# jackBonadies/Guided-Attention

Hardware: AMD Instinct MI355X
Metric: guided images/sec (50-step SD-1.5 512^2) (higher is better)
Workload: dtype f16

## Files before the change

guided-attention_amd/_lib.py:

```python
import ctypes
import os
from pathlib import Path

import torch

_HERE = Path(__file__).resolve().parent
LIB_PATH = Path(os.environ.get("GA_HIP_LIB", _HERE / "libga_hip.so"))

GA_VERSION = 183
GA_F16, GA_BF16, GA_F32 = 0, 1, 2
GA_LINEAR_STREAM = 8
GA_TOK_COOR, GA_TOK_BOX = 0, 1
GA_TERMS = 8
GA_MAX_IMAGES = 64
GA_IMAGE_MAX_TOKENS = 32
DTYPE_CODE = {torch.float16: GA_F16, torch.bfloat16: GA_BF16, torch.float32: GA_F32}


class GaError(RuntimeError):
    pass


class ga_token_t(ctypes.Structure):
    _fields_ = [("token", ctypes.c_int32), ("kind", ctypes.c_int32), ("geom", ctypes.c_double * 4),
# ... 30 lines not shown
    "ga_attn_capture_bwd": [_vp, _vp, _vp, _vp, _vp, _i64, _i64, _vp, _vp, _vp, _i, _i, _i, _i, _i, _f, _i, _vp],
    "ga_attn_capture_bwd_strided": [_vp, _vp, _vp, _vp, _vp, _i64, _i64, _i64, _vp, _vp, _vp, _i, _i, _i, _i, _i, _f, _i,
                                    _vp],
    "ga_attn_scores_max": [_vp, _vp, _i, _i, _i, _i, _i, _f, _i, _vp, _vp],
    "ga_attn_capture_fwd_biased": [_vp, _vp, _vp, _vp, _vp, _vp, _vp, _i, _i, _i, _i, _i, _f, _i, _vp],
    "ga_attn_capture_bwd_biased": [_vp, _vp, _vp, _vp, _vp, _i64, _i64, _vp, _vp, _vp, _vp, _i, _i, _i, _i, _i, _f, _i, _vp],
    "ga_attn_scores_max_grouped": [_vp, _vp, _i, _i, _i, _i, _i, _f, _i, _i, _vp, _vp],
    "ga_attn_capture_fwd_biased_grouped": [_vp, _vp, _vp, _vp, _vp, _vp, _i64, _vp, _vp, _i, _i, _i, _i, _i, _f, _i, _i, _vp],
    "ga_attn_capture_bwd_biased_grouped": [_vp, _vp, _vp, _vp, _vp, _i64, _i64, _i64, _vp, _vp, _i64, _vp, _vp, _vp, _i, _i, _i,
                                           _i, _i, _f, _i, _i, _vp],
    "ga_attn_pww_max_grad": [_vp, _vp, _vp, _vp, _vp, _i, _i, _i, _i, _i, _f, _i, _i, _vp],
    "ga_aggregate_maps": [ctypes.POINTER(_vp), ctypes.POINTER(_i), _i, _i, _i, _vp, _i, _vp],
    "ga_smooth_loss_fwd": [_vp, _i, _i, _i, _i, ctypes.POINTER(ga_token_t), _i, ctypes.POINTER(ga_loss_params_t), _vp,
                           _vp, _vp],
    "ga_smooth_loss_bwd": [_vp, _i, _i, _i, _i, ctypes.POINTER(ga_token_t), _i, ctypes.POINTER(ga_loss_params_t), _vp,
                           _vp, _vp, _f, _i, _vp],
    "ga_aggregate_loss_fwd": [ctypes.POINTER(_vp), ctypes.POINTER(_i), _i, _i, _i, _i, _i, ctypes.POINTER(ga_token_t), _i,
                              ctypes.POINTER(ga_loss_params_t), _vp, _vp, _vp, _vp, _i, _vp],
    "ga_aggregate_loss_fwd_batched": [ctypes.POINTER(_vp), ctypes.POINTER(_i), _i, _i, _i, _i, _i, _i,
                                      ctypes.POINTER(ga_token_t), _i, ctypes.POINTER(ga_loss_params_t), _vp, _vp, _vp, _vp,
                                      _i, _vp],
    "ga_smooth_loss_bwd_batched": [_vp, _i, _i, _i, _i, _i, ctypes.POINTER(ga_token_t), _i, ctypes.POINTER(ga_loss_params_t),
                                   _vp, _vp, _vp, _f, _i, _vp],
    "ga_aggregate_loss_fwd_images": [ctypes.POINTER(_vp), ctypes.POINTER(_i), _i, _i, _i, _i, _vp, _i,
                                     ctypes.POINTER(ga_loss_params_t), _vp, _vp, _vp, _vp, _i, _vp],
    "ga_smooth_loss_bwd_images": [_vp, _i, _i, _i, _vp, _i, ctypes.POINTER(ga_loss_params_t), _vp, _vp, _vp, _f, _i, _vp],
    "ga_gaussian_weights": [_i, _f, ctypes.POINTER(_f)],
    "ga_latent_axpy": [_vp, _vp, _f, _vp, _vp, _i64, _i, _vp],
    "ga_latent_sgd_momentum": [_vp, _vp, _vp, _f, _f, _i, _vp, _i64, _i, _vp],
    "ga_latent_axpby": [_vp, _vp, _f, _f, _vp, _i64, _i, _vp],
    "ga_cfg_ddim_step": [_vp, _vp, _f, _vp, _f, _f, _vp, _vp, _i64, _i, _vp],
    "ga_latent_axpy_batched": [_vp, _vp, _vp, _vp, _vp, _vp, _i, _i64, _i, _vp],
    "ga_latent_axpby_masked": [_vp, _vp, _f, _f, _vp, _vp, _i, _i64, _i, _vp],
    "ga_cfg_ddim_step_masked": [_vp, _vp, _f, _vp, _f, _f, _vp, _vp, _vp, _i, _i64, _i, _vp],
    "ga_self_attn_fwd": [_vp, _vp, _vp, _vp, _vp, _i, _i, _i, _i, _i, _f, _i, _vp],
    "ga_self_attn_bwd": [_vp, _vp, _vp, _vp, _vp, _vp, _vp, _vp, _vp, _vp, _i, _i, _i, _i, _i, _f, _i, _vp],
    "ga_group_norm_fwd": [_vp, _vp, _vp, _vp, _vp, _vp, _vp, _i, _i, _i, _i, _f, _i, _i, _vp],
    "ga_group_norm_bwd": [_vp, _vp, _vp, _vp, _vp, _vp, _vp, _vp, _vp, _i, _i, _i, _i, _i, _i, _vp],
    "ga_geglu_fwd": [_vp, _vp, _i64, _i, _i, _vp],
    "ga_geglu_bwd": [_vp, _vp, _vp, _i64, _i, _i, _vp],
    "ga_bias_residual_add": [_vp, _vp, _vp, _vp, _i64, _i, _i, _vp],
    "ga_cat_channels": [_vp, _vp, _vp, _i64, _i, _i, _i, _vp],
    "ga_cat_channels_gn_blocks": [_i, _i, _i, _i],
    "ga_linear_gn_blocks": [_i, _i, _i, _i, _i],
    "ga_group_norm_one_launch": [_i, _i, _i, _i],
    "ga_cat_group_norm_fwd": [_vp, _vp, _vp, _vp, _vp, _vp, _vp, _i, _i, _i, _i, _i, _f, _i, _i, _vp],
    "ga_cat_channels_gn": [_vp, _vp, _vp, _vp, _i, _i, _i, _i, _i, _i, _vp],
    "ga_conv3x3_packed_elems": [_i, _i],
    "ga_conv3x3_thin_packed_elems": [_i, _i],
    "ga_conv3x3_thin_supported": [_i, _i, _i, _i],
    "ga_conv3x3_thin_pack": [_vp, _vp, _i, _i, _i64, _i64, _i64, _i64, _i, _i, _vp],
    "ga_conv3x3_thin_in": [_vp, _vp, _vp, _vp, _i, _i, _i, _i, _i, _vp],
    "ga_conv3x3_thin_out": [_vp, _vp, _vp, _vp, _i, _i, _i, _i, _i, _vp],
    "ga_conv3x3_pack_weights": [_vp, _vp, _i, _i, _i64, _i64, _i64, _i64, _i, _i, _vp],
    "ga_conv3x3_plan": [_i, _i, _i, _i, _i, _i, ctypes.POINTER(_i), ctypes.POINTER(_i), ctypes.POINTER(_i),
                        ctypes.POINTER(ctypes.c_longlong)],
    "ga_splitk_workspace_floats": [_i64, _i, _i, _i, _i],
    "ga_conv3x3_nhwc": [_vp, _vp, _vp, _vp, _vp, _vp, _vp, _i, _i, _i, _i, _i, _i, _i, _i, _i, _i, _vp],
    "ga_conv3x3_gn_blocks": [_i, _i, _i, _i, _i, _i],
    "ga_conv3x3_nhwc_gn": [_vp, _vp, _vp, _vp, _vp, _vp, _vp, _i, _i, _i, _i, _i, _i, _i, _i, _i, _vp, _vp, _vp, _i],
    "ga_group_norm_apply": [_vp, _vp, _vp, _vp, _vp, _vp, _vp, _i, _i, _i, _i, _i, _f, _i, _i, _vp],
    "ga_group_norm_two_launch": [_i, _i, _i, _i],
    "ga_conv3x3_up2x_nhwc": [_vp, _vp, _vp, _vp, _vp, _vp, _vp, _i, _i, _i, _i, _i, _i, _i, _i, _i, _vp],
    "ga_gemm_nt": [_vp, _vp, _vp, _vp, _vp, _vp, _vp, _i64, _i, _i, _i, _i, _i, _i, _vp],
    "ga_linear_workspace": [_i64, _i, _i, _i, _i, _i, ctypes.POINTER(ctypes.c_longlong), ctypes.POINTER(_i)],
    "ga_linear_fused": [_vp, _i64, _vp, _vp, _i64, ctypes.POINTER(ga_linear_epilogue_t), _vp, _vp, _i64, _i, _i, _i, _i, _i,
                        _i, _i, _vp],
    "ga_add_layer_norm_fwd": [_vp, _vp, _vp, _vp, _vp, _vp, _vp, _i64, _i, _f, _i, _vp],
    "ga_add_layer_norm_bwd": [_vp, _vp, _vp, _vp, _vp, _vp, _i64, _i, _i, _vp],
}

_lib = None


def load():
    global _lib
    if _lib is None:
        if not LIB_PATH.exists():
            raise GaError(f"{LIB_PATH} not found: build it with `make` (or __graft_entry__.build()); "
                          "the guided-attention path has no CPU fallback")
        lib = ctypes.CDLL(str(LIB_PATH))
        lib.ga_version.argtypes, lib.ga_version.restype = [], ctypes.c_int
        built = lib.ga_version()
        if built != GA_VERSION:
            raise GaError(f"{LIB_PATH} is ABI version {built}, this binding is written for {GA_VERSION}: rebuild with `make`")
        for name, argtypes in PROTOTYPES.items():
            try:
                fn = getattr(lib, name)
            except AttributeError:
                raise GaError(f"{LIB_PATH} does not export {name}: rebuild with `make`") from None
            fn.argtypes = argtypes
            fn.restype = (ctypes.c_char_p if name == "ga_strerror" else
                          ctypes.c_longlong if name in ("ga_splitk_workspace_floats", "ga_conv3x3_packed_elems", "ga_conv3x3_thin_packed_elems") else ctypes.c_int)
        _lib = lib
    return _lib


def check(rc, what):
    if rc != 0:
        raise GaError(f"{what} failed: {load().ga_strerror(rc).decode()} ({rc})")


def stream_ptr():
    return ctypes.c_void_p(torch.cuda.current_stream().cuda_stream)


def dtype_code(t):
    try:
        return DTYPE_CODE[t.dtype]
    except KeyError:
        raise GaError(f"unsupported dtype {t.dtype}") from None


def require_cuda(*tensors):
    for t in tensors:
        if t is not None and not t.is_cuda:
            raise GaError("guided-attention kernels run on the GPU only (got a CPU tensor); there is no CPU fallback")
```

guided-attention_amd/csrc/group_norm.hip:

```cpp
#include "attn_common.h"

using namespace ga;

namespace {

constexpr int kThreads = 256;
constexpr int kMaxNPT = 5;
constexpr int kU = 8;

template <typename T, int W>
struct Item {
  T v[W];
};

template <typename T>
__device__ __forceinline__ Item<T, 2> load_pair(const T* p) {
  if constexpr (sizeof(T) == 2) return __builtin_bit_cast(Item<T, 2>, *reinterpret_cast<const unsigned*>(p));
  else return __builtin_bit_cast(Item<T, 2>, *reinterpret_cast<const unsigned long long*>(p));
}

__device__ __forceinline__ float sigmoidf_(float z) { return __builtin_amdgcn_rcpf(1.0f + __expf(-z)); }

template <typename T, int W>
__device__ __forceinline__ void load_chan_bias(const T* __restrict__ cbias, int b, int CP, int cp, float (&cb)[W]) {
#pragma unroll
  for (int j = 0; j < W; ++j) cb[j] = 0.f;
  if (cbias != nullptr) {
    const Item<T, W> it = reinterpret_cast<const Item<T, W>*>(cbias)[(size_t)b * CP + cp];
#pragma unroll
    for (int j = 0; j < W; ++j) cb[j] = Traits<T>::to_f32(it.v[j]);
  }
}

template <int NPT>
__device__ __forceinline__ void fold_to_groups(const float (&s0)[NPT], const float (&s1)[NPT], int CP, int cpg, int G,
                                               float* lds, float* out) {
#pragma unroll
  for (int k = 0; k < NPT; ++k) {
    const int cp = threadIdx.x + k * kThreads;
    if (cp < CP) {
      lds[2 * cp] = s0[k];
      lds[2 * cp + 1] = s1[k];
    }
  }
  __syncthreads();
  for (int g = threadIdx.x; g < G; g += kThreads) {
    float a = 0.f, b = 0.f;
    for (int cp = g * cpg; cp < (g + 1) * cpg; ++cp) {
      a += lds[2 * cp];
      b += lds[2 * cp + 1];
    }
    out[2 * g] = a;
    out[2 * g + 1] = b;
  }
}

template <typename T, int NPT, int W>
__global__ __launch_bounds__(kThreads) void gn_stats_kernel(const T* __restrict__ x, const T* __restrict__ cbias,
                                                            float* __restrict__ partial, int HW, int C, int G, int PB) {
  extern __shared__ __attribute__((aligned(16))) float lds[];
  const int b = blockIdx.y, nb = blockIdx.x, CP = C / W, cpg = (C / G) / W;
  const int p0 = nb * PB, p1 = min(HW, p0 + PB);
  float s0[NPT], s1[NPT];
#pragma unroll
  for (int k = 0; k < NPT; ++k) s0[k] = s1[k] = 0.f;
  const Item<T, W>* xb = reinterpret_cast<const Item<T, W>*>(x) + (size_t)b * HW * CP;
#pragma unroll
  for (int k = 0; k < NPT; ++k) {
    const int cp = threadIdx.x + k * kThreads;
    if (cp >= CP) continue;
    float cb[W];
    load_chan_bias<T, W>(cbias, b, CP, cp, cb);
    for (int p = p0; p < p1; p += kU) {
      Item<T, W> v[kU];
#pragma unroll
      for (int u = 0; u < kU; ++u)
        if (p + u < p1) v[u] = xb[(size_t)(p + u) * CP + cp];
#pragma unroll
      for (int u = 0; u < kU; ++u)
        if (p + u < p1) {
#pragma unroll
          for (int j = 0; j < W; ++j) {
            const float a = Traits<T>::to_f32(v[u].v[j]) + cb[j];
            s0[k] += a;
            s1[k] += a * a;
          }
        }
    }
  }
  fold_to_groups<NPT>(s0, s1, CP, cpg, G, lds, partial + ((size_t)b * gridDim.x + nb) * G * 2);
}

constexpr int kMaxStatsNB = 128;

struct NoHook {
  __device__ __forceinline__ void operator()() const {}
};
template <bool FWD, typename Hook = NoHook>
__device__ __forceinline__ void fold_partials(const float* __restrict__ partial, int b, int NB, int G, float inv_n,
                                              float eps, float2* res, float* keep, Hook after_loads = Hook()) {
  const float2* pp = reinterpret_cast<const float2*>(partial) + (size_t)b * NB * G;
  for (int g0 = 0; g0 < G; g0 += kThreads / 8) {
    const int g = g0 + (threadIdx.x >> 3), part = threadIdx.x & 7;
    float2 v[kMaxStatsNB / 8];
#pragma unroll
    for (int i = 0; i < kMaxStatsNB / 8; ++i) {
      const int nb = part + 8 * i;
      v[i] = pp[(size_t)min(nb, NB - 1) * G + min(g, G - 1)];
    }
    if (g0 == 0) after_loads();
    float sa = 0.f, sc = 0.f;
#pragma unroll
    for (int i = 0; i < kMaxStatsNB / 8; ++i) {
      const bool in = g < G && part + 8 * i < NB;
      sa += in ? v[i].x : 0.f;
      sc += in ? v[i].y : 0.f;
    }
    sa = group_sum<8>(sa);
    sc = group_sum<8>(sc);
    if (part == 0 && g < G) {
      float o0, o1;
      if (FWD) {
        const double mean = (double)sa * inv_n;
        const double var = fmax((double)sc * inv_n - mean * mean, 0.0);
        o0 = (float)mean;
        o1 = rsqrtf((float)var + eps);
      } else {
        o0 = sa * inv_n;
        o1 = sc * inv_n;
      }
      res[g] = float2{o0, o1};
      if (keep != nullptr) {
        keep[((size_t)b * G + g) * 2] = o0;
        keep[((size_t)b * G + g) * 2 + 1] = o1;
      }
    }
  }
  __syncthreads();
}

template <typename T, bool ACT, int NPT, int W>
__global__ __launch_bounds__(kThreads) void gn_apply_kernel(const T* __restrict__ x, const T* __restrict__ cbias,
                                                            const T* __restrict__ gamma,
                                                            const T* __restrict__ beta, T* __restrict__ y,
                                                            const float* __restrict__ partial, int NB, float inv_n,
                                                            float eps, float* __restrict__ stats, int HW, int C, int G,
                                                            int PB) {
  __shared__ float2 res[64];
  const int b = blockIdx.y, CP = C / W, cpg = (C / G) / W;
  fold_partials<true>(partial, b, NB, G, inv_n, eps, res, blockIdx.x == 0 ? stats : nullptr);
  const float* mu_rs = reinterpret_cast<const float*>(res);
  float sc[NPT][W], sh[NPT][W];
#pragma unroll
  for (int k = 0; k < NPT; ++k) {
    const int cp = threadIdx.x + k * kThreads;
    if (cp < CP) {
      const int g = cp / cpg;
      const Item<T, W> ga_ = reinterpret_cast<const Item<T, W>*>(gamma)[cp];
      const Item<T, W> be = reinterpret_cast<const Item<T, W>*>(beta)[cp];
      float cb[W];
      load_chan_bias<T, W>(cbias, b, CP, cp, cb);
#pragma unroll
      for (int j = 0; j < W; ++j) {
        sc[k][j] = Traits<T>::to_f32(ga_.v[j]) * mu_rs[2 * g + 1];
        sh[k][j] = Traits<T>::to_f32(be.v[j]) - (mu_rs[2 * g] - cb[j]) * sc[k][j];
      }
    }
  }
  const int p0 = blockIdx.x * PB, p1 = min(HW, p0 + PB);
  const Item<T, W>* xb = reinterpret_cast<const Item<T, W>*>(x) + (size_t)b * HW * CP;
  Item<T, W>* yb = reinterpret_cast<Item<T, W>*>(y) + (size_t)b * HW * CP;
#pragma unroll
  for (int k = 0; k < NPT; ++k) {
    const int cp = threadIdx.x + k * kThreads;
    if (cp >= CP) continue;
    for (int p = p0; p < p1; p += kU) {
      Item<T, W> v[kU];
#pragma unroll
      for (int u = 0; u < kU; ++u)
        if (p + u < p1) v[u] = xb[(size_t)(p + u) * CP + cp];
#pragma unroll
      for (int u = 0; u < kU; ++u)
        if (p + u < p1) {
          Item<T, W> o;
#pragma unroll
          for (int j = 0; j < W; ++j) {
            float z = Traits<T>::to_f32(v[u].v[j]) * sc[k][j] + sh[k][j];
            if (ACT) z *= sigmoidf_(z);
            o.v[j] = Traits<T>::from_f32(z);
          }
          yb[(size_t)(p + u) * CP + cp] = o;
        }
// ... 740 lines not shown
}

template <typename T>
int small_bwd(const void* x, const void* cb, const void* dy, const void* gamma, const void* beta, const float* stats,
              const void* gres, void* dx, int B, int HW, int C, int G, int act, hipStream_t s) {
  if (small_wide(HW, C, G))
    return act ? small_bwd_launch<T, true, 1024>(x, cb, dy, gamma, beta, stats, gres, dx, B, HW, C, G, s)
               : small_bwd_launch<T, false, 1024>(x, cb, dy, gamma, beta, stats, gres, dx, B, HW, C, G, s);
  return act ? small_bwd_launch<T, true, 256>(x, cb, dy, gamma, beta, stats, gres, dx, B, HW, C, G, s)
             : small_bwd_launch<T, false, 256>(x, cb, dy, gamma, beta, stats, gres, dx, B, HW, C, G, s);
}

bool small_path(int HW, int C, int G, size_t slab_bytes_per_elem) {
  const int Cg = C / G;
  return HW <= 1024 && (Cg & 1) == 0 && Cg <= 2048 && HW * Cg <= kSmallMaxElems &&
         kSmallHeader + slab_bytes_per_elem * (size_t)HW * Cg <= kMaxLdsBytes;
}

inline size_t elem_bytes(int dtype) { return dtype == GA_F32 ? 4 : 2; }

struct Geom {
  int NB, PBs, NBa, PBa, NPT, W;
  size_t lds;
};

int geometry(int B, int HW, int C, int G, Geom& g) {
  if (B < 1 || HW < 1 || C < 1 || G < 1 || G > 64 || C % G != 0) return GA_ERR_SHAPE;
  const int cg = C / G;
  g.W = (cg % 4 == 0) ? 4 : ((cg & 1) ? 1 : 2);
  const int CP = C / g.W;
  g.NPT = (CP + kThreads - 1) / kThreads;
  if (g.NPT > kMaxNPT) return GA_ERR_SHAPE;
  g.PBs = (HW + kMaxStatsNB - 1) / kMaxStatsNB < 8 ? 8 : (HW + kMaxStatsNB - 1) / kMaxStatsNB;
  g.NB = (HW + g.PBs - 1) / g.PBs;
  g.PBa = HW >= 4096 ? 16 : (HW >= 1024 ? 8 : 4);
  g.NBa = (HW + g.PBa - 1) / g.PBa;
  g.lds = sizeof(float) * 2 * CP;
  return GA_OK;
}

template <typename T, bool ACT, int NPT, int W>
int launch_fwd_t(const void* x, const void* cbias, const void* gamma, const void* beta, void* y, float* stats, float* ws,
                 int B, int HW, int C, int G, float eps, const Geom& g, hipStream_t s) {
  const float inv_n = 1.0f / ((float)HW * (float)(C / G));
  hipLaunchKernelGGL((gn_stats_kernel<T, NPT, W>), dim3(g.NB, B), dim3(kThreads), g.lds, s, (const T*)x,
                     (const T*)cbias, ws, HW, C, G, g.PBs);
  hipLaunchKernelGGL((gn_apply_kernel<T, ACT, NPT, W>), dim3(g.NBa, B), dim3(kThreads), 0, s, (const T*)x,
                     (const T*)cbias, (const T*)gamma, (const T*)beta, (T*)y, (const float*)ws, g.NB, inv_n, eps, stats,
                     HW, C, G, g.PBa);
  return check_launch();
}

template <typename T, bool ACT, int NPT, int W>
int launch_bwd_t(const void* x, const void* cbias, const void* dy, const void* gamma, const void* beta,
                 const float* stats, const void* gres, void* dx, float* ws, int B, int HW, int C, int G, const Geom& g,
                 hipStream_t s) {
  const float inv_n = 1.0f / ((float)HW * (float)(C / G));
  hipLaunchKernelGGL((gn_bwd_stats_kernel<T, ACT, NPT, W>), dim3(g.NB, B), dim3(kThreads), g.lds, s, (const T*)x,
                     (const T*)cbias, (const T*)dy, (const T*)gamma, (const T*)beta, stats, ws, HW, C, G, g.PBs);
  hipLaunchKernelGGL((gn_bwd_apply_kernel<T, ACT, NPT, W>), dim3(g.NBa, B), dim3(kThreads), 0, s, (const T*)x,
                     (const T*)cbias, (const T*)dy, (const T*)gamma, (const T*)beta, stats, (const float*)ws, g.NB, inv_n,
                     (const T*)gres, (T*)dx, HW, C, G, g.PBa);
  return check_launch();
}

#define GA_GN_NPT(FN, T, ACT, ...)                                   \
  if (g.W == 1) {                                                    \
    switch (g.NPT) {                                                 \
      case 1: return FN<T, ACT, 1, 1>(__VA_ARGS__);                  \
      case 2: return FN<T, ACT, 2, 1>(__VA_ARGS__);                  \
      default: return FN<T, ACT, 5, 1>(__VA_ARGS__);                 \
    }                                                                \
  }                                                                  \
  if (g.W == 4) {                                                    \
    switch (g.NPT) {                                                 \
      case 1: return FN<T, ACT, 1, 4>(__VA_ARGS__);                  \
      case 2: return FN<T, ACT, 2, 4>(__VA_ARGS__);                  \
      default: return FN<T, ACT, 3, 4>(__VA_ARGS__);                 \
    }                                                                \
  }                                                                  \
  switch (g.NPT) {                                                   \
    case 1: return FN<T, ACT, 1, 2>(__VA_ARGS__);                    \
    case 2: return FN<T, ACT, 2, 2>(__VA_ARGS__);                    \
    case 3: return FN<T, ACT, 3, 2>(__VA_ARGS__);                    \
    case 4: return FN<T, ACT, 4, 2>(__VA_ARGS__);                    \
    default: return FN<T, ACT, 5, 2>(__VA_ARGS__);                   \
  }

inline bool wide_ok(int C, int G, size_t elem) { return elem == 2 && C % 8 == 0 && C / G >= 8 && C <= 8 * kThreads; }

struct WideGeom {
  int PBs, NB, PBa, NBa;
  WideGeom(int HW, int C) {
    const int RP = kThreads / (C / 8);
    const int fill = (HW + kMaxStatsNB - 1) / kMaxStatsNB;
    PBs = fill > 8 * RP ? fill : 8 * RP;
    NB = (HW + PBs - 1) / PBs;
    PBa = 4 * RP;
    NBa = (HW + PBa - 1) / PBa;
  }
};

template <typename T>
int wide_fwd(const void* x, const void* cbias, const void* gamma, const void* beta, void* y, float* stats, float* ws,
             int B, int HW, int C, int G, float eps, int act, hipStream_t s) {
  const WideGeom g(HW, C);
  const float inv_n = 1.0f / ((float)HW * (float)(C / G));
  hipLaunchKernelGGL(gn_wide_stats_kernel<T>, dim3(g.NB, B), dim3(kThreads), 0, s, (const T*)x, (const T*)cbias, ws, HW,
                     C, G, g.PBs);
  if (act)
    hipLaunchKernelGGL((gn_wide_apply_kernel<T, true>), dim3(g.NBa, B), dim3(kThreads), 0, s, (const T*)x,
                       (const T*)cbias, (const T*)gamma, (const T*)beta, (T*)y, (const float*)ws, g.NB, inv_n, eps, stats,
                       HW, C, G, g.PBa);
  else
    hipLaunchKernelGGL((gn_wide_apply_kernel<T, false>), dim3(g.NBa, B), dim3(kThreads), 0, s, (const T*)x,
                       (const T*)cbias, (const T*)gamma, (const T*)beta, (T*)y, (const float*)ws, g.NB, inv_n, eps, stats,
                       HW, C, G, g.PBa);
  return check_launch();
}

template <typename T>
int wide_bwd(const void* x, const void* cbias, const void* dy, const void* gamma, const void* beta, const float* stats,
             const void* gres, void* dx, float* ws, int B, int HW, int C, int G, int act, hipStream_t s) {
  const WideGeom g(HW, C);
  const float inv_n = 1.0f / ((float)HW * (float)(C / G));
  if (act)
    hipLaunchKernelGGL((gn_wide_bwd_stats_kernel<T, true>), dim3(g.NB, B), dim3(kThreads), 0, s, (const T*)x,
                       (const T*)cbias, (const T*)dy, (const T*)gamma, (const T*)beta, stats, ws, HW, C, G, g.PBs);
  else
    hipLaunchKernelGGL((gn_wide_bwd_stats_kernel<T, false>), dim3(g.NB, B), dim3(kThreads), 0, s, (const T*)x,
                       (const T*)cbias, (const T*)dy, (const T*)gamma, (const T*)beta, stats, ws, HW, C, G, g.PBs);
  if (act)
    hipLaunchKernelGGL((gn_wide_bwd_apply_kernel<T, true>), dim3(g.NBa, B), dim3(kThreads), 0, s, (const T*)x,
                       (const T*)cbias, (const T*)dy, (const T*)gamma, (const T*)beta, stats, (const float*)ws, g.NB,
                       inv_n, (const T*)gres, (T*)dx, HW, C, G, g.PBa);
  else
    hipLaunchKernelGGL((gn_wide_bwd_apply_kernel<T, false>), dim3(g.NBa, B), dim3(kThreads), 0, s, (const T*)x,
                       (const T*)cbias, (const T*)dy, (const T*)gamma, (const T*)beta, stats, (const float*)ws, g.NB,
                       inv_n, (const T*)gres, (T*)dx, HW, C, G, g.PBa);
  return check_launch();
}

template <typename T>
int fwd_dtype(const void* x, const void* cbias, const void* gamma, const void* beta, void* y, float* stats, float* ws, int B,
              int HW, int C, int G, float eps, int act, const Geom& g, hipStream_t s) {
  if constexpr (sizeof(T) == 2) {
    if (wide_ok(C, G, sizeof(T))) return wide_fwd<T>(x, cbias, gamma, beta, y, stats, ws, B, HW, C, G, eps, act, s);
  }
  if (act) {
    GA_GN_NPT(launch_fwd_t, T, true, x, cbias, gamma, beta, y, stats, ws, B, HW, C, G, eps, g, s)
  }
  GA_GN_NPT(launch_fwd_t, T, false, x, cbias, gamma, beta, y, stats, ws, B, HW, C, G, eps, g, s)
}

template <typename T>
int bwd_dtype(const void* x, const void* cbias, const void* dy, const void* gamma, const void* beta, const float* stats,
              const void* gres, void* dx, float* ws, int B, int HW, int C, int G, int act, const Geom& g, hipStream_t s) {
  if constexpr (sizeof(T) == 2) {
    if (wide_ok(C, G, sizeof(T))) return wide_bwd<T>(x, cbias, dy, gamma, beta, stats, gres, dx, ws, B, HW, C, G, act, s);
  }
  if (act) {
    GA_GN_NPT(launch_bwd_t, T, true, x, cbias, dy, gamma, beta, stats, gres, dx, ws, B, HW, C, G, g, s)
  }
  GA_GN_NPT(launch_bwd_t, T, false, x, cbias, dy, gamma, beta, stats, gres, dx, ws, B, HW, C, G, g, s)
}

}

extern "C" int ga_group_norm_fwd(const void* x, const void* chan_bias, const void* gamma, const void* beta, void* y,
                                 float* stats, float* workspace, int B, int HW, int C, int G, float eps, int act_silu,
                                 int dtype, ga_stream_t stream) {
  if (!x || !gamma || !beta || !y || !stats || !workspace) return GA_ERR_NULL;
  Geom g;
  int rc = geometry(B, HW, C, G, g);
  if (rc != GA_OK) return rc;
  hipStream_t s = static_cast<hipStream_t>(stream);
  if (small_path(HW, C, G, sizeof(float))) {
    switch (dtype) {
      case GA_F16: return small_fwd<_Float16>(x, chan_bias, gamma, beta, y, stats, B, HW, C, G, eps, act_silu, s);
      case GA_BF16: return small_fwd<bf16_t>(x, chan_bias, gamma, beta, y, stats, B, HW, C, G, eps, act_silu, s);
      case GA_F32: return small_fwd<float>(x, chan_bias, gamma, beta, y, stats, B, HW, C, G, eps, act_silu, s);
      default: return GA_ERR_DTYPE;
    }
  }
  switch (dtype) {
    case GA_F16: return fwd_dtype<_Float16>(x, chan_bias, gamma, beta, y, stats, workspace, B, HW, C, G, eps, act_silu, g, s);
    case GA_BF16: return fwd_dtype<bf16_t>(x, chan_bias, gamma, beta, y, stats, workspace, B, HW, C, G, eps, act_silu, g, s);
    case GA_F32: return fwd_dtype<float>(x, chan_bias, gamma, beta, y, stats, workspace, B, HW, C, G, eps, act_silu, g, s);
    default: return GA_ERR_DTYPE;
  }
}

extern "C" int ga_group_norm_apply(const void* x, const void* chan_bias, const void* gamma, const void* beta, void* y,
                                   float* stats, const float* partials, int blocks, int B, int HW, int C, int G, float eps,
                                   int act_silu, int dtype, ga_stream_t stream) {
  if (!x || !gamma || !beta || !y || !stats || !partials) return GA_ERR_NULL;
  Geom g;
  int rc = geometry(B, HW, C, G, g);
  if (rc != GA_OK) return rc;
  if (blocks < 1 || blocks > kMaxStatsNB) return GA_ERR_SHAPE;
  if (dtype == GA_F32 || !wide_ok(C, G, 2)) return GA_ERR_UNSUPPORTED;
  hipStream_t s = static_cast<hipStream_t>(stream);
  const WideGeom wg(HW, C);
  const float inv_n = 1.0f / ((float)HW * (float)(C / G));
#define GA_GN_APPLY(T, ACT)                                                                                                   \
  hipLaunchKernelGGL((gn_wide_apply_kernel<T, ACT>), dim3(wg.NBa, B), dim3(kThreads), 0, s, (const T*)x, (const T*)chan_bias, \
                     (const T*)gamma, (const T*)beta, (T*)y, partials, blocks, inv_n, eps, stats, HW, C, G, wg.PBa)
  if (dtype == GA_F16) {
    if (act_silu) GA_GN_APPLY(_Float16, true);
    else GA_GN_APPLY(_Float16, false);
  } else if (dtype == GA_BF16) {
    if (act_silu) GA_GN_APPLY(bf16_t, true);
    else GA_GN_APPLY(bf16_t, false);
  } else {
    return GA_ERR_DTYPE;
  }
#undef GA_GN_APPLY
  return check_launch();
}

extern "C" int ga_group_norm_one_launch(int HW, int C, int G, int dtype) {
  if (HW < 1 || C < 1 || G < 1 || G > 64 || C % G != 0 || dtype < GA_F16 || dtype > GA_F32) return 0;
  return small_path(HW, C, G, sizeof(float)) ? 1 : 0;
}

extern "C" int ga_cat_group_norm_fwd(const void* a, const void* b, void* cat, const void* gamma, const void* beta, void* y,
                                     float* stats, int B, int HW, int C1, int C2, int G, float eps, int act_silu, int dtype,
                                     ga_stream_t stream) {
  if (!a || !b || !cat || !gamma || !beta || !y || !stats) return GA_ERR_NULL;
  if (C1 < 2 || C2 < 2 || C1 % 2 != 0 || C2 % 2 != 0) return GA_ERR_SHAPE;
  const int C = C1 + C2;
  Geom g;
  int rc = geometry(B, HW, C, G, g);
  if (rc != GA_OK) return rc;
  if ((C / G) % 2 != 0) return GA_ERR_SHAPE;
  if (!small_path(HW, C, G, sizeof(float))) return GA_ERR_UNSUPPORTED;
  hipStream_t s = static_cast<hipStream_t>(stream);
  const SmallCat sc{b, C1, cat};
  switch (dtype) {
    case GA_F16: return small_fwd<_Float16>(a, nullptr, gamma, beta, y, stats, B, HW, C, G, eps, act_silu, s, sc);
    case GA_BF16: return small_fwd<bf16_t>(a, nullptr, gamma, beta, y, stats, B, HW, C, G, eps, act_silu, s, sc);
    case GA_F32: return small_fwd<float>(a, nullptr, gamma, beta, y, stats, B, HW, C, G, eps, act_silu, s, sc);
    default: return GA_ERR_DTYPE;
  }
}

extern "C" int ga_cat_channels_gn_blocks(int HW, int C, int G, int dtype) {
  if (dtype == GA_F32 || HW < 1 || C < 1 || G < 1 || C % G != 0) return 0;
  if (small_path(HW, C, G, sizeof(float)) || !wide_ok(C, G, 2)) return 0;
  return WideGeom(HW, C).NB;
}

extern "C" int ga_cat_channels_gn(const void* a, const void* b, void* out, float* partials, int B, int HW, int C1, int C2, int G,
                                  int dtype, ga_stream_t stream) {
  if (!a || !b || !out || !partials) return GA_ERR_NULL;
// ... 47 lines not shown
```

guided-attention_amd/csrc/linear.hip:

```cpp
#include "attn_common.h"

using namespace ga;

namespace {

typedef float f32x16 __attribute__((ext_vector_type(16)));
typedef unsigned int u32x4 __attribute__((ext_vector_type(4)));

constexpr int kBK = 64;
constexpr int kThreads = 256;
#define GA_LDS_PTR(p) ((__attribute__((address_space(3))) void*)(p))

template <typename T>
struct Mma32L;
template <>
struct Mma32L<_Float16> {
  __device__ static __forceinline__ f32x16 run(uint4 a, uint4 b, f32x16 c) {
    return __builtin_amdgcn_mfma_f32_32x32x16_f16(__builtin_bit_cast(f16x8, a), __builtin_bit_cast(f16x8, b), c, 0, 0, 0);
  }
};
template <>
struct Mma32L<bf16_t> {
  __device__ static __forceinline__ f32x16 run(uint4 a, uint4 b, f32x16 c) {
    return __builtin_amdgcn_mfma_f32_32x32x16_bf16(__builtin_bit_cast(bf16x8, a), __builtin_bit_cast(bf16x8, b), c, 0, 0, 0);
  }
};

struct LinArgs {
  int M, N, K;
  int ldx, ldy, ld_res, ld_pre;
  int tm, tn, splits, steps, steps_per, n_fastest;
  FastDiv d_tm, d_tn;
  int F;
  int ln_parts;
  float ln_eps, ln_inv_k;
  unsigned x_bytes, w_bytes;
};

struct LinHead {
  int M, ldx;
  unsigned kn;
  int tm;
  unsigned tn_splits;
  unsigned steps;
  unsigned dtm_m, dtn_m;
};

struct LinPtrs {
  const void* bias;
  const void* residual;
  void* preact;
  const float* ln_partials;
  const float* ln_colsum;
  const float* ln_shift;
  float* ln_stats_out;
  float* row_partials_out;
  float* slabs;
  unsigned* tickets;
  float* gn_partials;
  int gn_cg, gn_G, gn_hw, gn_tpi;
};

template <int BM, int BN>
__device__ __forceinline__ void lin_tile(const LinArgs& a, int& mt, int& nt, int& split) {
  const int total = a.tm * a.tn * a.splits, q = total >> 3, r = total & 7;
  const int xcd = blockIdx.x & 7, slot = blockIdx.x >> 3;
  const int logical = (xcd < r ? xcd * (q + 1) : r * (q + 1) + (xcd - r) * q) + slot;
  const bool nf = a.n_fastest != 0;
  const FastDiv d1 = nf ? a.d_tn : a.d_tm, d2 = nf ? a.d_tm : a.d_tn;
  const int t1 = nf ? a.tn : a.tm, t2 = nf ? a.tm : a.tn;
  const int rest = fdiv(logical, d1), i1 = logical - rest * t1;
  split = fdiv(rest, d2);
  const int i2 = rest - split * t2;
  mt = nf ? i2 : i1;
  nt = nf ? i1 : i2;
}

__device__ __forceinline__ void lds_read128(u32x4& dst, unsigned byte_address) {
#if defined(__HIP_DEVICE_COMPILE__)
  asm volatile("ds_read_b128 %0, %1" : "=v"(dst) : "v"(byte_address) : "memory");
#else
  dst = u32x4{byte_address, 0u, 0u, 0u};
#endif
}
__device__ __forceinline__ void opaque(u32x4& v) {
#if defined(__HIP_DEVICE_COMPILE__)
  asm volatile("" : "+v"(v));
#endif
}
template <int N>
__device__ __forceinline__ void wait_vmcnt() {
#if defined(__HIP_DEVICE_COMPILE__)
  asm volatile("s_waitcnt vmcnt(%0)" ::"n"(N) : "memory");
#endif
}
template <int N>
__device__ __forceinline__ void wait_lgkmcnt() {
#if defined(__HIP_DEVICE_COMPILE__)
  asm volatile("s_waitcnt lgkmcnt(%0)" ::"n"(N) : "memory");
#endif
}

#if defined(GA_LIN_STAMPS)
__device__ unsigned long long* g_lin_stamps = nullptr;
struct LinStamps {
  unsigned long long t[10];
  __device__ __forceinline__ void at(int i) {
#if defined(__HIP_DEVICE_COMPILE__)
    __builtin_amdgcn_sched_barrier(0);
    unsigned long long v;
    asm volatile("s_memtime %0\n\ts_waitcnt lgkmcnt(0)" : "=s"(v)::"memory");
    __builtin_amdgcn_sched_barrier(0);
    t[i] = v;
#endif
  }
  __device__ __forceinline__ void real(int i) {
#if defined(__HIP_DEVICE_COMPILE__)
    __builtin_amdgcn_sched_barrier(0);
    unsigned long long v;
    asm volatile("s_memrealtime %0\n\ts_waitcnt lgkmcnt(0)" : "=s"(v)::"memory");
    __builtin_amdgcn_sched_barrier(0);
    t[i] = v;
#endif
  }
  __device__ __forceinline__ void flush() {
    if (threadIdx.x == 0 && g_lin_stamps != nullptr)
      for (int i = 0; i < 10; ++i) g_lin_stamps[(size_t)blockIdx.x * 10 + i] = t[i];
  }
};
#define GA_STAMP(st, i) (st).at(i)
#else
struct LinStamps {};
#define GA_STAMP(st, i) ((void)0)
#endif

// ... 179 lines not shown
      s1 = group_sum<VPR>(s1);
      s2 = group_sum<VPR>(s2);
      if ((v & (VPR - 1)) == 0 && m < a.M)
        *reinterpret_cast<float2*>(p.row_partials_out + ((size_t)m * a.tn + nt) * 2) = float2{s1, s2};
    }
  }
  if constexpr (!GEGLU) {
    if (gn) {
      const int cv = (tid & (VPR - 1)) * 8;
      const int c_abs = n0 + cv, gA = c_abs / p.gn_cg, split = min(8, (gA + 1) * p.gn_cg - c_abs);
      float4 r = {0.f, 0.f, 0.f, 0.f};
#pragma unroll
      for (int q = 0; q < 8; ++q) {
        if (q < split) {
          r.x += gsum[q];
          r.y += gsq[q];
        } else {
          r.z += gsum[q];
          r.w += gsq[q];
        }
      }
      __syncthreads();
      float4* lds4 = reinterpret_cast<float4*>(Cs);
      lds4[tid] = r;
      __syncthreads();
      const int n_end = min(n0 + BN, a.N);
      const int g_first = n0 / p.gn_cg, g_last = (n_end - 1) / p.gn_cg;
      const int g = g_first + tid;
      if (g <= g_last) {
        const int c_lo = max(g * p.gn_cg, n0), c_hi = min((g + 1) * p.gn_cg, n_end);
        float sa = 0.f, sq = 0.f;
        for (int vv = (c_lo - n0) >> 3; vv <= (c_hi - 1 - n0) >> 3; ++vv) {
          const bool first = (n0 + 8 * vv) / p.gn_cg == g;
          for (int pr = 0; pr < kThreads / VPR; ++pr) {
            const float4 e4 = lds4[pr * VPR + vv];
            sa += first ? e4.x : e4.z;
            sq += first ? e4.y : e4.w;
          }
        }
        const int b = m0 / p.gn_hw, t = (m0 - b * p.gn_hw) / BM;
        float2* out = reinterpret_cast<float2*>(p.gn_partials) + ((size_t)b * 2 * p.gn_tpi + 2 * t) * p.gn_G + g;
        const bool starts = g * p.gn_cg >= n0, ends = (g + 1) * p.gn_cg <= n_end;
        if (starts) {
          out[0] = float2{sa, sq};
          if (ends) out[p.gn_G] = float2{0.f, 0.f};
        } else {
          out[p.gn_G] = float2{sa, sq};
        }
      }
    }
  }
}

template <typename T, int BM, int BN, int NSTAGE, bool GEGLU, bool LN>
__global__ __launch_bounds__(kThreads, (BM + BN) * 128 * NSTAGE <= 80 * 1024 ? 2 : 1) void linear_kernel(
    const T* __restrict__ X, const T* __restrict__ W, T* __restrict__ Y, int h_M, int h_ldx, unsigned h_kn, int h_tm,
    unsigned h_tn_splits, unsigned h_steps, unsigned h_dtm_m, unsigned h_dtn_m, LinArgs a_in, LinPtrs p) {
  const LinHead h{h_M, h_ldx, h_kn, h_tm, h_tn_splits, h_steps, h_dtm_m, h_dtn_m};
  LinStamps st;
#if defined(GA_LIN_STAMPS)
  st.real(8);
#endif
  GA_STAMP(st, 0);
  LinArgs a;
  a.M = h.M; a.ldx = h.ldx; a.K = (int)(h.kn & 0xffffu); a.N = (int)(h.kn >> 16);
  a.tm = h.tm; a.tn = (int)(h.tn_splits & 0xffffu); a.splits = (int)(h.tn_splits >> 16);
  a.steps = (int)(h.steps & 0xffffu); a.steps_per = (int)((h.steps >> 16) & 0x7fffu); a.n_fastest = (int)(h.steps >> 31);
  a.d_tm = FastDiv{(unsigned)a.tm, h.dtm_m}; a.d_tn = FastDiv{(unsigned)a.tn, h.dtn_m};
  a.F = GEGLU ? a.N / 2 : 0;
  a.x_bytes = (unsigned)(((a.M - 1) * a.ldx + a.K) * 2); a.w_bytes = (unsigned)(a.N * a.K * 2);
  a.ldy = a_in.ldy; a.ld_res = a_in.ld_res; a.ld_pre = a_in.ld_pre;
  a.ln_parts = a_in.ln_parts; a.ln_eps = a_in.ln_eps; a.ln_inv_k = a_in.ln_inv_k;
  constexpr int WM = BM / 2, WN = BN / 2, IM = WM / 32, JN = WN / 32;
  constexpr int kStage = (BM + BN) * kBK;
  constexpr int IPS = (BM + BN) / 32;
  constexpr int LDC = BN + 8;
  constexpr int kLds = NSTAGE * kStage > BM * LDC ? NSTAGE * kStage : BM * LDC;
  __shared__ __attribute__((aligned(1024))) T lds[kLds];

  const int tid = threadIdx.x, lane = tid & 63, wave = tid >> 6;
  const int wm = wave >> 1, wn = wave & 1, fr = lane & 31, fh = lane >> 5;
  int mt, nt, split;
  lin_tile<BM, BN>(a, mt, nt, split);
  const int m0 = mt * BM;
  const int n0 = GEGLU ? nt * (BN / 2) : nt * BN;
  const int it0 = split * a.steps_per, it1 = min(a.steps, it0 + a.steps_per);
  const int nsteps = it1 - it0;

  const __amdgpu_buffer_rsrc_t xrsrc = __builtin_amdgcn_make_buffer_rsrc(const_cast<T*>(X), 0, a.x_bytes, 0x00020000);
  const __amdgpu_buffer_rsrc_t wrsrc = __builtin_amdgcn_make_buffer_rsrc(const_cast<T*>(W), 0, a.w_bytes, 0x00020000);
  unsigned voff[IPS];
#pragma unroll
  for (int q = 0; q < IPS; ++q) {
    const int row = 8 * (wave + 4 * q) + (lane >> 3);
    const int col = (lane & 7) ^ ((row >> 1) & 7);
    if (row < BM) {
      const int m = min(m0 + row, a.M - 1);
      voff[q] = (unsigned)((m * a.ldx + 8 * col) * (int)sizeof(T));
    } else {
      const int r = row - BM;
      int n;
      if (GEGLU) n = r < BN / 2 ? min(n0 + r, a.F - 1) : a.F + min(n0 + r - BN / 2, a.F - 1);
      else n = min(n0 + r, a.N - 1);
      voff[q] = (unsigned)((n * a.K + 8 * col) * (int)sizeof(T));
    }
  }
  const int wave_u = __builtin_amdgcn_readfirstlane(wave);
  auto issue = [&](int step, int slot) {
    const unsigned koff = (unsigned)((it0 + step) * kBK * (int)sizeof(T));
#pragma unroll
    for (int q = 0; q < IPS; ++q) {
      T* dst = lds + slot * kStage + (wave_u + 4 * q) * 8 * kBK;
      if (8 * (wave_u + 4 * q) < BM)
        __builtin_amdgcn_raw_ptr_buffer_load_lds(xrsrc, GA_LDS_PTR(dst), 16, (int)voff[q], (int)koff, 0, 0);
      else
        __builtin_amdgcn_raw_ptr_buffer_load_lds(wrsrc, GA_LDS_PTR(dst), 16, (int)voff[q], (int)koff, 0, 0);
    }
  };

  unsigned a_adr[IM], a_sw[IM], b_adr[JN], b_sw[JN];
  const unsigned lds0 = (unsigned)(uintptr_t)GA_LDS_PTR(lds);
#pragma unroll
  for (int i = 0; i < IM; ++i) {
    const int row = wm * WM + i * 32 + fr;
    a_adr[i] = lds0 + row * (kBK * (int)sizeof(T));
    a_sw[i] = (unsigned)(((row >> 1) & 7) ^ fh);
  }
#pragma unroll
  for (int j = 0; j < JN; ++j) {
    const int row = BM + wn * WN + j * 32 + fr;
    b_adr[j] = lds0 + row * (kBK * (int)sizeof(T));
    b_sw[j] = (unsigned)(((row >> 1) & 7) ^ fh);
  }

  f32x16 acc[JN][IM];
#pragma unroll
  for (int j = 0; j < JN; ++j)
#pragma unroll
    for (int i = 0; i < IM; ++i)
#pragma unroll
      for (int r = 0; r < 16; ++r) acc[j][i][r] = 0.f;

  constexpr int PRE = NSTAGE - 1;
#pragma unroll
  for (int s = 0; s < PRE; ++s)
    if (s < nsteps) issue(s, s);
  LinPrefetch<T, BM, BN, GEGLU, LN> pre;
  pre.load(a, p, m0, n0);
  float ln_mean[IM], ln_rstd[IM];
  if constexpr (LN) {
    const float2* part[IM];
    float s1[IM], s2[IM];
#pragma unroll
    for (int i = 0; i < IM; ++i) {
      const int m = min(m0 + wm * WM + i * 32 + fr, a.M - 1);
      part[i] = reinterpret_cast<const float2*>(p.ln_partials) + (size_t)m * a.ln_parts;
      s1[i] = s2[i] = 0.f;
    }
    for (int q0 = 0; q0 < a.ln_parts; q0 += 4) {
      float2 v[IM][4];
#pragma unroll
      for (int i = 0; i < IM; ++i)
#pragma unroll
        for (int u = 0; u < 4; ++u) v[i][u] = part[i][min(q0 + u, a.ln_parts - 1)];
#pragma unroll
      for (int i = 0; i < IM; ++i)
#pragma unroll
        for (int u = 0; u < 4; ++u)
          if (q0 + u < a.ln_parts) {
            s1[i] += v[i][u].x;
            s2[i] += v[i][u].y;
          }
    }
#pragma unroll
    for (int i = 0; i < IM; ++i) {
      const float mean = s1[i] * a.ln_inv_k;
      ln_mean[i] = mean;
      ln_rstd[i] = rsqrtf(fmaxf(s2[i] * a.ln_inv_k - mean * mean, 0.f) + a.ln_eps);
    }
  }

  GA_STAMP(st, 1);
  for (int it = 0; it < nsteps; ++it) {
    const int younger = min(nsteps - 1 - it, PRE - 1);
    if (younger >= 3) wait_vmcnt<3 * IPS>();
    else if (younger == 2) wait_vmcnt<2 * IPS>();
    else if (younger == 1) wait_vmcnt<IPS>();
    else wait_vmcnt<0>();
    __builtin_amdgcn_s_barrier();
#if defined(GA_LIN_STAMPS)
    if (it == 0) st.at(2);
#endif
    if (it + PRE < nsteps) issue(it + PRE, (it + PRE) % NSTAGE);
    const unsigned slot_off = (unsigned)((it % NSTAGE) * kStage * (int)sizeof(T));
    u32x4 fa[2][IM], fb[2][JN];
    auto request = [&](int kk, int set) {
#pragma unroll
      for (int i = 0; i < IM; ++i)
        lds_read128(fa[set][i], a_adr[i] + slot_off + 16u * ((2u * kk) ^ a_sw[i]));
#pragma unroll
      for (int j = 0; j < JN; ++j)
        lds_read128(fb[set][j], b_adr[j] + slot_off + 16u * ((2u * kk) ^ b_sw[j]));
    };
    request(0, 0);
#pragma unroll
    for (int kk = 0; kk < kBK / 16; ++kk) {
      if (kk + 1 < kBK / 16) {
        request(kk + 1, (kk + 1) & 1);
        wait_lgkmcnt<IM + JN>();
      } else {
        wait_lgkmcnt<0>();
      }
      __builtin_amdgcn_sched_barrier(0);
#pragma unroll
      for (int j = 0; j < JN; ++j)
#pragma unroll
        for (int i = 0; i < IM; ++i)
          acc[j][i] = Mma32L<T>::run(__builtin_bit_cast(uint4, fb[kk & 1][j]), __builtin_bit_cast(uint4, fa[kk & 1][i]), acc[j][i]);
    }
  }
  static_assert(NSTAGE >= 2 && NSTAGE <= 5, "the counted waits above cover up to four k-steps in flight");
  wait_lgkmcnt<0>();
  __builtin_amdgcn_s_barrier();
  GA_STAMP(st, 3);

  if (a.splits > 1) {
    const int tile = nt * a.tm + mt;
    const __amdgpu_buffer_rsrc_t srsrc =
        __builtin_amdgcn_make_buffer_rsrc(p.slabs, 0, 0x7ffffff0, 0x00020000);
    constexpr int QUADS = JN * IM * 4;
    const unsigned per_slice = (unsigned)(a.tm * a.tn) * (BM * BN * 4u);
    const unsigned tbase = (unsigned)tile * (BM * BN * 4u) + (unsigned)tid * 16u;
#pragma unroll
    for (int j = 0; j < JN; ++j)
#pragma unroll
      for (int i = 0; i < IM; ++i)
#pragma unroll
        for (int qd = 0; qd < 4; ++qd) {
          const int q = (j * IM + i) * 4 + qd;
          const u32x4 v = {__float_as_uint(acc[j][i][4 * qd]), __float_as_uint(acc[j][i][4 * qd + 1]),
                           __float_as_uint(acc[j][i][4 * qd + 2]), __float_as_uint(acc[j][i][4 * qd + 3])};
          __builtin_amdgcn_raw_buffer_store_b128(v, srsrc, tbase + q * (kThreads * 16u), split * per_slice, 16);
        }
    asm volatile("s_waitcnt vmcnt(0)" ::: "memory");
#pragma unroll
    for (int j = 0; j < JN; ++j)
#pragma unroll
      for (int i = 0; i < IM; ++i) keep_live(acc[j][i]);
    __syncthreads();
    int* flag = reinterpret_cast<int*>(lds);
    if (tid == 0) {
      const unsigned old = __hip_atomic_fetch_add(p.tickets + tile, 1u, __ATOMIC_RELAXED, __HIP_MEMORY_SCOPE_AGENT);
      flag[0] = old == (unsigned)a.splits - 1;
      if (old == (unsigned)a.splits - 1) __hip_atomic_store(p.tickets + tile, 0u, __ATOMIC_RELAXED, __HIP_MEMORY_SCOPE_AGENT);
    }
    __syncthreads();
    const int last = flag[0];
    __syncthreads();
    if (!last) return;
#pragma unroll
    for (int j = 0; j < JN; ++j)
#pragma unroll
      for (int i = 0; i < IM; ++i)
#pragma unroll
        for (int r = 0; r < 16; ++r) acc[j][i][r] = 0.f;
    constexpr int SB = QUADS <= 4 ? 4 : (QUADS <= 8 ? 2 : 1);
    for (int s0 = 0; s0 < a.splits; s0 += SB) {
      u32x4 v[SB][QUADS];
#pragma unroll
      for (int sb = 0; sb < SB; ++sb) {
        const unsigned soff = (unsigned)min(s0 + sb, a.splits - 1) * per_slice;
#pragma unroll
        for (int q = 0; q < QUADS; ++q)
          v[sb][q] = __builtin_amdgcn_raw_buffer_load_b128(srsrc, tbase + q * (kThreads * 16u), soff, 16);
      }
#pragma unroll
      for (int sb = 0; sb < SB; ++sb) {
        const bool in = s0 + sb < a.splits;
#pragma unroll
        for (int j = 0; j < JN; ++j)
#pragma unroll
          for (int i = 0; i < IM; ++i)
#pragma unroll
            for (int qd = 0; qd < 4; ++qd)
#pragma unroll
              for (int r = 0; r < 4; ++r)
                acc[j][i][4 * qd + r] += in ? __uint_as_float(v[sb][(j * IM + i) * 4 + qd][r]) : 0.f;
      }
    }
  }

  float ln_m[IM], ln_r[IM];
#pragma unroll
  for (int i = 0; i < IM; ++i) {
    ln_m[i] = LN ? ln_mean[i] : 0.f;
    ln_r[i] = LN ? ln_rstd[i] : 1.f;
  }
  GA_STAMP(st, 4);
  lin_epilogue<T, BM, BN, GEGLU, LN>(acc, lds, Y, a, p, m0, n0, nt, ln_m, ln_r, pre, st);
#if defined(GA_LIN_STAMPS)
  st.at(6);
  asm volatile("s_waitcnt vmcnt(0)" ::: "memory");
  st.at(7);
  st.real(9);
  st.flush();
#endif
}

template <typename T, int BM, int BN, int NSTAGE>
int launch_lin(const T* X, const T* W, T* Y, LinArgs a, const LinPtrs& p, hipStream_t s) {
  const int outc = a.F ? BN / 2 : BN, n_out = a.F ? a.F : a.N;
  a.tm = (a.M + BM - 1) / BM;
  a.tn = (n_out + outc - 1) / outc;
  a.steps = a.K / kBK;
  a.steps_per = (a.steps + a.splits - 1) / a.splits;
  {
    const double xb = (double)a.M * a.K, wb = (double)a.N * a.K;
    const double m_first = wb + xb * (a.tn * a.splits < 8 ? a.tn * a.splits : 8), n_first = xb + wb * (a.tm < 8 ? a.tm : 8);
    a.n_fastest = n_first < m_first ? 1 : 0;
  }
  {
    bool ok = true;
    const unsigned long long wgs = (unsigned long long)a.tm * a.tn * a.splits;
    a.d_tm = make_fastdiv(a.tm, wgs, ok);
    a.d_tn = make_fastdiv(a.tn, wgs, ok);
    if (!ok) return GA_ERR_SHAPE;
  }
  const dim3 grid((unsigned)(a.tm * a.tn * a.splits));
  const bool ln = a.ln_parts > 0;
  if (a.K > 0xffff || a.N > 0xffff || a.tn > 0xffff || a.splits > 0xffff || a.steps > 0xffff || a.steps_per > 0x7fff) return GA_ERR_SHAPE;
  const LinHead h{a.M, a.ldx, (unsigned)a.K | ((unsigned)a.N << 16), a.tm, (unsigned)a.tn | ((unsigned)a.splits << 16),
                  (unsigned)a.steps | ((unsigned)a.steps_per << 16) | ((unsigned)(a.n_fastest != 0) << 31), a.d_tm.m, a.d_tn.m};
#define GA_LIN_LAUNCH(G, L)                                                                                                \
  hipLaunchKernelGGL((linear_kernel<T, BM, BN, NSTAGE, G, L>), grid, dim3(kThreads), 0, s, X, W, Y, h.M, h.ldx, h.kn, h.tm, \
                     h.tn_splits, h.steps, h.dtm_m, h.dtn_m, a, p)
  if (a.F) {
    if (ln) GA_LIN_LAUNCH(true, true);
    else GA_LIN_LAUNCH(true, false);
  } else {
    if (ln) GA_LIN_LAUNCH(false, true);
    else GA_LIN_LAUNCH(false, false);
  }
#undef GA_LIN_LAUNCH
  return check_launch();
}

template <typename T>
int lin_t(const void* X, const void* W, void* Y, const LinArgs& a, const LinPtrs& p, int bm, int bn, int stages, hipStream_t s) {
  const T* x = (const T*)X;
  const T* w = (const T*)W;
  if (bm == 128 && bn == 128) {
    if (stages == 2) return launch_lin<T, 128, 128, 2>(x, w, (T*)Y, a, p, s);
    if (stages == 0 || stages == 3) return launch_lin<T, 128, 128, 3>(x, w, (T*)Y, a, p, s);
  } else if ((bm == 128 && bn == 64) || (bm == 64 && bn == 128)) {
    const bool tall = bm == 128;
    if (stages == 3) return tall ? launch_lin<T, 128, 64, 3>(x, w, (T*)Y, a, p, s) : launch_lin<T, 64, 128, 3>(x, w, (T*)Y, a, p, s);
    if (stages == 0 || stages == 4)
      return tall ? launch_lin<T, 128, 64, 4>(x, w, (T*)Y, a, p, s) : launch_lin<T, 64, 128, 4>(x, w, (T*)Y, a, p, s);
  } else if (bm == 64 && bn == 64) {
    if (stages == 5) return launch_lin<T, 64, 64, 5>(x, w, (T*)Y, a, p, s);
    if (stages == 0 || stages == 4) return launch_lin<T, 64, 64, 4>(x, w, (T*)Y, a, p, s);
  }
  return GA_ERR_SHAPE;
}

constexpr int kSThreads = 512;
constexpr int kSStage = 256 * kBK * 2;
constexpr int kSNst = 4, kSPre = kSNst - 1;
constexpr int kSOutStride = 144;
constexpr int kSPartsMax = 20;
constexpr int kSStageOff = kSNst * kSStage;
constexpr int kSStageBytes = 128 * 16 * (kSPartsMax / 2);
constexpr int kSCstOff = kSStageOff + kSStageBytes;
constexpr int kSStatOff = kSCstOff + 1024;
constexpr int kSLds = kSStatOff + 1024;
static_assert(128 * kSOutStride <= kSStageBytes && kSLds <= 160 * 1024, "LDS map of linear_stream_kernel");

__device__ __forceinline__ void lds_read64(f32x2& dst, unsigned byte_address) {
#if defined(__HIP_DEVICE_COMPILE__)
  asm volatile("ds_read_b64 %0, %1" : "=v"(dst) : "v"(byte_address) : "memory");
#else
  dst = f32x2{(float)byte_address, 0.f};
#endif
}
__device__ __forceinline__ void lds_read128f(f32x4& dst, unsigned byte_address) {
#if defined(__HIP_DEVICE_COMPILE__)
  asm volatile("ds_read_b128 %0, %1" : "=v"(dst) : "v"(byte_address) : "memory");
#else
  dst = f32x4{(float)byte_address, 0.f, 0.f, 0.f};
#endif
}
__device__ __forceinline__ void lds_write64(unsigned byte_address, f32x2 v) {
#if defined(__HIP_DEVICE_COMPILE__)
  asm volatile("ds_write_b64 %0, %1" ::"v"(byte_address), "v"(v) : "memory");
#endif
}

template <typename T>
__device__ __forceinline__ f32x2 pack4(float a, float b, float c, float d) {
  typename Traits<T>::frag f;
  f[0] = Traits<T>::from_f32(a);
  f[1] = Traits<T>::from_f32(b);
  f[2] = Traits<T>::from_f32(c);
  f[3] = Traits<T>::from_f32(d);
  return __builtin_bit_cast(f32x2, f);
}

template <typename T, bool GEGLU>
__global__ __launch_bounds__(kSThreads, 2) void linear_stream_kernel(
    const T* __restrict__ X, const T* __restrict__ W, T* __restrict__ Y, int h_M, int h_ldx, unsigned h_kn, int h_tm,
    unsigned h_tn_splits, unsigned h_steps, unsigned h_dtm_m, unsigned h_dtn_m, LinArgs a_in, LinPtrs p) {
  const int M = h_M, ldx = h_ldx, K = (int)(h_kn & 0xffffu), N = (int)(h_kn >> 16);
  const int tm = h_tm, tn = (int)(h_tn_splits & 0xffffu), G = (int)(h_tn_splits >> 16);
  const int steps = (int)(h_steps & 0xffffu);
// ... 269 lines not shown
  const long long tiles = (long long)a.tm * a.tn;
  if (tiles > 0x7fffffffLL / 256 || a.K > 0xffff || a.N > 0xffff || a.tn > 0xffff || a.steps > 0xffff) return GA_ERR_SHAPE;
  const int G = tiles < cus ? (int)tiles : cus;
  {
    const double xb = (double)a.M * a.K, wb = (double)a.N * a.K;
    const double m_first = wb + xb * (a.tn < 8 ? a.tn : 8), n_first = xb + wb * (a.tm < 8 ? a.tm : 8);
    a.n_fastest = n_first < m_first ? 1 : 0;
  }
  bool ok = true;
  const unsigned long long span = (unsigned long long)tiles + (unsigned long long)G;
  a.d_tm = make_fastdiv(a.tm, span, ok);
  a.d_tn = make_fastdiv(a.tn, span, ok);
  if (!ok) return GA_ERR_SHAPE;
  const LinHead h{a.M, a.ldx, (unsigned)a.K | ((unsigned)a.N << 16), a.tm, (unsigned)a.tn | ((unsigned)G << 16),
                  (unsigned)a.steps | ((unsigned)(a.n_fastest != 0) << 31), a.d_tm.m, a.d_tn.m};
  if (a.F)
    hipLaunchKernelGGL((linear_stream_kernel<T, true>), dim3((unsigned)G), dim3(kSThreads), 0, s, X, W, Y, h.M, h.ldx, h.kn, h.tm,
                       h.tn_splits, h.steps, h.dtm_m, h.dtn_m, a, p);
  else
    hipLaunchKernelGGL((linear_stream_kernel<T, false>), dim3((unsigned)G), dim3(kSThreads), 0, s, X, W, Y, h.M, h.ldx, h.kn, h.tm,
                       h.tn_splits, h.steps, h.dtm_m, h.dtn_m, a, p);
  return check_launch();
}

bool al16(const void* p) { return (reinterpret_cast<uintptr_t>(p) & 15) == 0; }

}

#if defined(GA_LIN_STAMPS)
extern "C" int ga_lin_set_stamps(void* buffer) {
  unsigned long long* p = static_cast<unsigned long long*>(buffer);
  return hipMemcpyToSymbol(HIP_SYMBOL(g_lin_stamps), &p, sizeof(p)) == hipSuccess ? GA_OK : GA_ERR_LAUNCH;
}
#endif

extern "C" int ga_linear_workspace(int64_t M, int N, int bm, int bn, int splits, int geglu, long long* slab_floats, int* tiles) {
  if (!slab_floats || !tiles) return GA_ERR_NULL;
  if (M < 1 || N < 8 || splits < 1 || (bm != 64 && bm != 128) || (bn != 64 && bn != 128)) return GA_ERR_SHAPE;
  const int outc = geglu ? bn / 2 : bn, n_out = geglu ? N / 2 : N;
  const long long tm = (M + bm - 1) / bm, tn = (n_out + outc - 1) / outc;
  *tiles = (int)(tm * tn);
  *slab_floats = splits > 1 ? (long long)splits * tm * tn * bm * bn : 0;
  return GA_OK;
}

extern "C" int ga_linear_gn_blocks(int hw, int N, int groups, int bm, int bn) {
  if (hw < 1 || N < 8 || groups < 1 || N % groups != 0 || (bm != 64 && bm != 128) || (bn != 64 && bn != 128)) return 0;
  const int cg = N / groups;
  if (hw % bm != 0 || cg < 8 || cg > bn || groups > 64) return 0;
  const int blocks = 2 * (hw / bm);
  return blocks <= 128 ? blocks : 0;
}

extern "C" int ga_linear_fused(const void* X, int64_t ldx, const void* W, void* Y, int64_t ldy, const ga_linear_epilogue_t* ep,
                               float* slabs, unsigned* tickets, int64_t M, int K, int N, int bm, int bn, int splits,
                               int stages, int dtype, ga_stream_t stream) {
  if (!X || !W || !Y || !ep) return GA_ERR_NULL;
  if (M < 1 || K < kBK || K % kBK != 0 || N < 8 || N % 8 != 0 || ldx < K || ldx % 8 != 0 || ldy % 8 != 0) return GA_ERR_SHAPE;
  if (splits < 1 || splits > 64 || K / kBK < splits || (splits > 1 && (!slabs || !tickets))) return GA_ERR_SHAPE;
  const int n_out = ep->geglu ? N / 2 : N;
  if (ep->geglu && (N % 16 != 0 || ep->residual)) return GA_ERR_SHAPE;
  if (ldy < n_out || (ep->residual && (ep->ld_res < n_out || ep->ld_res % 8 != 0))) return GA_ERR_SHAPE;
  if (ep->preact && (!ep->geglu || ep->ld_pre < N || ep->ld_pre % 8 != 0)) return GA_ERR_SHAPE;
  if (ep->ln_partials && (ep->ln_parts < 1 || !ep->ln_colsum || !ep->ln_shift)) return GA_ERR_NULL;
  if (!al16(X) || !al16(W) || !al16(Y) || (ep->bias && !al16(ep->bias)) || (ep->residual && !al16(ep->residual)) ||
      (ep->preact && !al16(ep->preact)) || (ep->ln_colsum && !al16(ep->ln_colsum)) || (ep->ln_shift && !al16(ep->ln_shift)))
    return GA_ERR_ALIGN;
  const long long xb = ((long long)(M - 1) * ldx + K) * 2, wb = (long long)N * K * 2;
  if (xb >= (1LL << 31) || wb >= (1LL << 31)) return GA_ERR_SHAPE;
  LinArgs a;
  a.M = (int)M; a.N = N; a.K = K;
  a.ldx = (int)ldx; a.ldy = (int)ldy; a.ld_res = (int)ep->ld_res; a.ld_pre = (int)ep->ld_pre;
  a.splits = splits;
  a.F = ep->geglu ? N / 2 : 0;
  a.ln_parts = ep->ln_partials ? ep->ln_parts : 0;
  a.ln_eps = ep->ln_eps;
  a.ln_inv_k = 1.0f / (float)K;
  a.x_bytes = (unsigned)xb;
  a.w_bytes = (unsigned)wb;
  if (splits > 1) {
    long long need; int tiles;
    if (ga_linear_workspace(M, N, bm, bn, splits, ep->geglu, &need, &tiles) != GA_OK) return GA_ERR_SHAPE;
    if (need * 4 >= (1LL << 31)) return GA_ERR_SHAPE;
  }
  LinPtrs p;
  p.bias = ep->bias; p.residual = ep->residual; p.preact = ep->preact;
  p.ln_partials = ep->ln_partials; p.ln_colsum = ep->ln_colsum; p.ln_shift = ep->ln_shift;
  p.ln_stats_out = ep->ln_stats_out; p.row_partials_out = ep->row_partials_out;
  p.slabs = slabs; p.tickets = tickets;
  p.gn_partials = nullptr; p.gn_cg = p.gn_G = p.gn_hw = p.gn_tpi = 0;
  if (ep->gn_partials) {
    if (ep->geglu || stages == GA_LINEAR_STREAM) return GA_ERR_UNSUPPORTED;
    if (ga_linear_gn_blocks(ep->gn_hw, N, ep->gn_groups, bm, bn) == 0 || M % ep->gn_hw != 0) return GA_ERR_SHAPE;
    p.gn_partials = ep->gn_partials; p.gn_G = ep->gn_groups; p.gn_cg = N / ep->gn_groups; p.gn_hw = ep->gn_hw;
    p.gn_tpi = ep->gn_hw / bm;
  }
  hipStream_t s = static_cast<hipStream_t>(stream);
  if (stages == GA_LINEAR_STREAM) {
    if (bm != 128 || bn != 128 || splits != 1 || !ep->ln_partials || ep->bias || ep->residual || ep->preact || ep->ln_stats_out ||
        ep->row_partials_out || K / kBK < 5 || ep->ln_parts < 2 || ep->ln_parts > kSPartsMax || ldy > 0x7fffffff)
      return GA_ERR_UNSUPPORTED;
    if ((long long)M * ep->ln_parts * 8 >= (1LL << 31)) return GA_ERR_SHAPE;
    switch (dtype) {
      case GA_F16: return launch_stream<_Float16>((const _Float16*)X, (const _Float16*)W, (_Float16*)Y, a, p, s);
      case GA_BF16: return launch_stream<bf16_t>((const bf16_t*)X, (const bf16_t*)W, (bf16_t*)Y, a, p, s);
      default: return GA_ERR_DTYPE;
    }
  }
  switch (dtype) {
    case GA_F16: return lin_t<_Float16>(X, W, Y, a, p, bm, bn, stages, s);
    case GA_BF16: return lin_t<bf16_t>(X, W, Y, a, p, bm, bn, stages, s);
    default: return GA_ERR_DTYPE;
  }
}
```

guided-attention_amd/csrc/thin_conv.hip:

```cpp
#include "ga_common.h"

namespace {
using namespace ga;

constexpr int kSeg = 16;
constexpr int kPatchW = kSeg + 2;
constexpr int kTaps = 9;

template <typename T>
struct Dot2;
template <>
struct Dot2<_Float16> {
  typedef _Float16 v2 __attribute__((ext_vector_type(2)));
  __device__ static __forceinline__ float acc(uint32_t a, uint32_t b, float c) {
    return __builtin_amdgcn_fdot2(__builtin_bit_cast(v2, a), __builtin_bit_cast(v2, b), c, false);
  }
};
template <>
struct Dot2<bf16_t> {
  typedef __bf16 v2 __attribute__((ext_vector_type(2)));
  __device__ static __forceinline__ float acc(uint32_t a, uint32_t b, float c) {
    return __builtin_amdgcn_fdot2_f32_bf16(__builtin_bit_cast(v2, a), __builtin_bit_cast(v2, b), c, false);
  }
};

template <typename T>
__device__ __forceinline__ uint16_t bits_of(T x) {
  return __builtin_bit_cast(uint16_t, x);
}

__global__ void thin_pack_kernel(const uint16_t* __restrict__ w, uint32_t* __restrict__ out, int N, int C, long long so,
                                 long long si, long long sy, long long sx, int flip) {
  const int total = kTaps * (C / 2) * N;
  const int i = blockIdx.x * blockDim.x + threadIdx.x;
  if (i >= total) return;
  int n, q, t;
  if (C == 4) {
    n = i % N;
    q = (i / N) % 2;
    t = i / (2 * N);
  } else {
    n = i % 4;
    q = (i / 4) % (C / 2);
    t = i / (4 * (C / 2));
  }
  const int ty = t / 3, tx = t % 3;
  uint32_t v[2];
#pragma unroll
  for (int e = 0; e < 2; ++e) {
    const int c = 2 * q + e;
    const long long off = flip ? c * so + n * si + (2 - ty) * sy + (2 - tx) * sx : n * so + c * si + ty * sy + tx * sx;
    v[e] = w[off];
  }
// ... 13 lines not shown

  uint4 wv[2 * kTaps];
#pragma unroll
  for (int i = 0; i < 2 * kTaps; ++i) wv[i] = wp[(size_t)i * G + g];
  float bv[4] = {0.f, 0.f, 0.f, 0.f};
  if (bias) {
    const typename Traits<T>::frag bf = load_frag<T>(bias + 4 * g);
#pragma unroll
    for (int j = 0; j < 4; ++j) bv[j] = Traits<T>::to_f32(bf[j]);
  }

  const int pc = tid % kPatchW, pr = (tid / kPatchW) % 3, pci = tid / (3 * kPatchW);
  auto fetch = [&](int sg) -> uint16_t {
    const int seg = sg % segs, row = (sg / segs) % H, b = sg / (segs * H);
    const int yy = row + pr - 1, xx = seg * kSeg + pc - 1;
    if (tid < kInPatch && yy >= 0 && yy < H && xx >= 0 && xx < W) return bits_of(x[(((size_t)b * 4 + pci) * H + yy) * W + xx]);
    return 0;
  };
  uint16_t* pl = reinterpret_cast<uint16_t*>(patch);
  const int first = blockIdx.x * segs_per_wg;
  const int last = min(first + segs_per_wg, total_segs);
  uint16_t nxt = fetch(first);
  for (int sg = first; sg < last; ++sg) {
    const int seg = sg % segs, row = (sg / segs) % H, b = sg / (segs * H);
    if (sg != first) __syncthreads();
    if (tid < kInPatch) pl[(pr * kPatchW + pc) * 4 + pci] = nxt;
    __syncthreads();
    if (sg + 1 < last) nxt = fetch(sg + 1);
    for (int s = slot; s < kSeg; s += PP) {
      float acc[4] = {bv[0], bv[1], bv[2], bv[3]};
#pragma unroll
      for (int t = 0; t < kTaps; ++t) {
        const uint2 xv = patch[(t / 3) * kPatchW + s + (t % 3)];
        const uint4 w0 = wv[2 * t], w1 = wv[2 * t + 1];
        acc[0] = Dot2<T>::acc(xv.x, w0.x, acc[0]);
        acc[1] = Dot2<T>::acc(xv.x, w0.y, acc[1]);
        acc[2] = Dot2<T>::acc(xv.x, w0.z, acc[2]);
        acc[3] = Dot2<T>::acc(xv.x, w0.w, acc[3]);
        acc[0] = Dot2<T>::acc(xv.y, w1.x, acc[0]);
        acc[1] = Dot2<T>::acc(xv.y, w1.y, acc[1]);
        acc[2] = Dot2<T>::acc(xv.y, w1.z, acc[2]);
        acc[3] = Dot2<T>::acc(xv.y, w1.w, acc[3]);
      }
      typename Traits<T>::frag o;
#pragma unroll
      for (int j = 0; j < 4; ++j) o[j] = Traits<T>::from_f32(acc[j]);
      store_frag<T>(y + (((size_t)b * H + row) * W + seg * kSeg + s) * N + 4 * g, o);
    }
  }
}

constexpr int kOutThreads = 256;
constexpr int kOutSlices = 32;

template <typename T, int PAIRS>
__global__ void __launch_bounds__(kOutThreads)
thin_out_kernel(const T* __restrict__ x, const uint32_t* __restrict__ wp, const T* __restrict__ bias, T* __restrict__ y, int H, int W,
                int total_segs, int segs_per_wg) {
  constexpr int C = PAIRS * 64;
  constexpr int kVecPx = C / 8;
  constexpr int kPatchVecs = 3 * kPatchW * kVecPx;
  constexpr int kLoads = (kPatchVecs + kOutThreads - 1) / kOutThreads;
  __shared__ uint4 patch[kPatchVecs];
  const int tid = threadIdx.x;
  const int sl = tid & (kOutSlices - 1), slot = tid >> 5;
  const int segs = W / kSeg;

  uint4 wr[kTaps][PAIRS];
#pragma unroll
  for (int t = 0; t < kTaps; ++t)
#pragma unroll
    for (int q = 0; q < PAIRS; ++q) wr[t][q] = reinterpret_cast<const uint4*>(wp)[t * (C / 2) + sl * PAIRS + q];
  float bv = 0.f;
  if (bias && sl < 4) bv = Traits<T>::to_f32(bias[sl]);

  auto fetch = [&](int sg, uint4 (&val)[kLoads]) {
    const int seg = sg % segs, row = (sg / segs) % H, b = sg / (segs * H);
#pragma unroll
    for (int j = 0; j < kLoads; ++j) {
      const int i = tid + j * kOutThreads;
      const int v = i % kVecPx, c = (i / kVecPx) % kPatchW, r = i / (kVecPx * kPatchW);
      const int yy = row + r - 1, xx = seg * kSeg + c - 1;
      const bool in = i < kPatchVecs && yy >= 0 && yy < H && xx >= 0 && xx < W;
      const size_t pix = in ? ((size_t)b * H + yy) * W + xx : (size_t)b * H * W;
      const uint4 t = reinterpret_cast<const uint4*>(x + pix * C)[in ? v : 0];
      val[j] = in ? t : uint4{0u, 0u, 0u, 0u};
    }
  };
  const int first = blockIdx.x * segs_per_wg;
  const int last = min(first + segs_per_wg, total_segs);
  uint4 val[kLoads];
  fetch(first, val);
  for (int sg = first; sg < last; ++sg) {
    const int seg = sg % segs, row = (sg / segs) % H, b = sg / (segs * H);
    if (sg != first) __syncthreads();
#pragma unroll
    for (int j = 0; j < kLoads; ++j) {
      const int i = tid + j * kOutThreads;
      if (i < kPatchVecs) patch[i] = val[j];
    }
    __syncthreads();
    if (sg + 1 < last) fetch(sg + 1, val);

    const uint32_t* pw = reinterpret_cast<const uint32_t*>(patch);
#pragma unroll
    for (int h = 0; h < kSeg / 8; ++h) {
      const int p = slot + 8 * h;
      float acc[4] = {0.f, 0.f, 0.f, 0.f};
#pragma unroll
      for (int t = 0; t < kTaps; ++t) {
        const uint32_t* xp = pw + ((t / 3) * kPatchW + p + (t % 3)) * (C / 2) + sl * PAIRS;
#pragma unroll
        for (int q = 0; q < PAIRS; ++q) {
          const uint32_t xv = xp[q];
          acc[0] = Dot2<T>::acc(xv, wr[t][q].x, acc[0]);
          acc[1] = Dot2<T>::acc(xv, wr[t][q].y, acc[1]);
          acc[2] = Dot2<T>::acc(xv, wr[t][q].z, acc[2]);
          acc[3] = Dot2<T>::acc(xv, wr[t][q].w, acc[3]);
        }
      }
#pragma unroll
      for (int j = 0; j < 4; ++j) {
        acc[j] = group_sum<16>(acc[j]);
        acc[j] += __shfl_xor(acc[j], 16, 64);
      }
      if (sl < 4) {
        const float v = (sl == 0 ? acc[0] : sl == 1 ? acc[1] : sl == 2 ? acc[2] : acc[3]) + bv;
        y[(((size_t)b * 4 + sl) * H + row) * W + seg * kSeg + p] = Traits<T>::from_f32(v);
      }
    }
  }
}

inline bool aligned16(const void* p) { return (reinterpret_cast<uintptr_t>(p) & 15u) == 0; }

inline void seg_grid(long long total, int& per, unsigned& grid) {
  per = (int)((total + 1023) / 1024);
  grid = (unsigned)((total + per - 1) / per);
}

template <typename T>
int launch_in(const void* x, const void* wp, const void* bias, void* y, int B, int H, int W, int N, hipStream_t s) {
  const int G = N / 4;
  int PP = (256 + G - 1) / G;
  PP = PP < 1 ? 1 : PP > kSeg ? kSeg : PP;
  if (G * PP < kInPatch || G * PP > 1024) return GA_ERR_SHAPE;
  const long long total = (long long)B * H * (W / kSeg);
  int per;
  unsigned grid;
  seg_grid(total, per, grid);
  hipLaunchKernelGGL(thin_in_kernel<T>, dim3(grid), dim3((unsigned)(G * PP)), 0, s, (const T*)x, (const uint4*)wp, (const T*)bias,
                     (T*)y, H, W, N, G, PP, (int)total, per);
  return check_launch();
}

template <typename T>
int launch_out(const void* x, const void* wp, const void* bias, void* y, int B, int H, int W, int C, hipStream_t s) {
  const long long total = (long long)B * H * (W / kSeg);
  const int per = total <= 1024 ? (int)((total + 255) / 256) : (int)((total + 1023) / 1024);
  const unsigned grid = (unsigned)((total + per - 1) / per);
#define GA_THIN_OUT(P)                                                                                                   \
  case P:                                                                                                                \
    hipLaunchKernelGGL((thin_out_kernel<T, P>), dim3(grid), dim3(kOutThreads), 0, s, (const T*)x, (const uint32_t*)wp,    \
                       (const T*)bias, (T*)y, H, W, (int)total, per);                                                    \
    break;
  switch (C / 64) {
    GA_THIN_OUT(1)
    GA_THIN_OUT(2)
    GA_THIN_OUT(3)
    GA_THIN_OUT(4)
    GA_THIN_OUT(5)
    default: return GA_ERR_SHAPE;
  }
#undef GA_THIN_OUT
  return check_launch();
}

}

extern "C" long long ga_conv3x3_thin_packed_elems(int Cout, int Cin) {
  if (Cin == 4 && Cout >= 4) return 36LL * Cout;
  if (Cout == 4 && Cin >= 4) return 36LL * Cin;
  return 0;
}

extern "C" int ga_conv3x3_thin_supported(int H, int W, int Cin, int Cout) {
  if (H < 1 || W < kSeg || W % kSeg != 0) return 0;
  if (Cin == 4) return Cout % 4 == 0 && Cout >= 64 && Cout <= 4096 ? 1 : 0;
  if (Cout == 4) return Cin % 64 == 0 && Cin >= 64 && Cin <= 320 ? 1 : 0;
  return 0;
}

extern "C" int ga_conv3x3_thin_pack(const void* weight, void* packed, int Cout, int Cin, long long so, long long si, long long sy,
                                    long long sx, int transpose_flip, int dtype, ga_stream_t stream) {
  if (!weight || !packed) return GA_ERR_NULL;
  if (dtype != GA_F16 && dtype != GA_BF16) return GA_ERR_DTYPE;
  const int N = transpose_flip ? Cin : Cout, C = transpose_flip ? Cout : Cin;
  if (!((C == 4 && N >= 4 && N % 4 == 0) || (N == 4 && C % 2 == 0 && C >= 4))) return GA_ERR_SHAPE;
  if (!aligned16(packed)) return GA_ERR_ALIGN;
  const int total = kTaps * (C / 2) * N;
  hipLaunchKernelGGL(thin_pack_kernel, dim3((unsigned)((total + 255) / 256)), dim3(256), 0, static_cast<hipStream_t>(stream),
                     (const uint16_t*)weight, (uint32_t*)packed, N, C, so, si, sy, sx, transpose_flip ? 1 : 0);
  return check_launch();
}

extern "C" int ga_conv3x3_thin_in(const void* x, const void* packed, const void* bias, void* y, int B, int H, int W, int Cout,
                                  int dtype, ga_stream_t stream) {
  if (!x || !packed || !y) return GA_ERR_NULL;
  if (B < 1 || !ga_conv3x3_thin_supported(H, W, 4, Cout) || Cout / 4 > 1024) return GA_ERR_SHAPE;
  if ((long long)B * H * (W / kSeg) >= (1LL << 31)) return GA_ERR_SHAPE;
  if (!aligned16(packed) || (reinterpret_cast<uintptr_t>(y) & 7u) || (bias && (reinterpret_cast<uintptr_t>(bias) & 7u)))
    return GA_ERR_ALIGN;
  hipStream_t s = static_cast<hipStream_t>(stream);
  switch (dtype) {
    case GA_F16: return launch_in<_Float16>(x, packed, bias, y, B, H, W, Cout, s);
    case GA_BF16: return launch_in<bf16_t>(x, packed, bias, y, B, H, W, Cout, s);
    default: return GA_ERR_DTYPE;
  }
}

extern "C" int ga_conv3x3_thin_out(const void* x, const void* packed, const void* bias, void* y, int B, int H, int W, int Cin,
                                   int dtype, ga_stream_t stream) {
  if (!x || !packed || !y) return GA_ERR_NULL;
  if (B < 1 || !ga_conv3x3_thin_supported(H, W, Cin, 4)) return GA_ERR_SHAPE;
  if ((long long)B * H * (W / kSeg) >= (1LL << 31)) return GA_ERR_SHAPE;
  if (!aligned16(x) || !aligned16(packed)) return GA_ERR_ALIGN;
  hipStream_t s = static_cast<hipStream_t>(stream);
  switch (dtype) {
    case GA_F16: return launch_out<_Float16>(x, packed, bias, y, B, H, W, Cin, s);
    case GA_BF16: return launch_out<bf16_t>(x, packed, bias, y, B, H, W, Cin, s);
    default: return GA_ERR_DTYPE;
  }
}
```

guided-attention_amd/fused_linear.py:

```python
import weakref

import torch
import torch.nn.functional as F

from . import ops
from ._lib import GaError


def supported(x, in_features, out_features):
    return (x.is_cuda and x.dtype in (torch.float16, torch.bfloat16) and in_features % 64 == 0 and out_features % 16 == 0
            and x.stride(-1) == 1)


def block_folds(x):
    return supported(x, x.shape[-1], x.shape[-1]) and not ops.library_block(x.numel() // x.shape[-1], x.shape[-1])


def _transposed(weight):
    key = (weight.data_ptr(), weight._version, tuple(weight.shape), weight.dtype)
    hit = _wt_cache.get(key)
    if hit is None or hit[0]() is None:
        with torch.no_grad():
            wt = weight.t().contiguous()
        if len(_wt_cache) > 2048:
            for dead in [k for k, (ref, _) in _wt_cache.items() if ref() is None]:
                del _wt_cache[dead]
        owner = weight._base if weight._base is not None else weight
        hit = _wt_cache[key] = (weakref.ref(owner), wt)
    return ops.keep_alive(hit[1])


_wt_cache = {}


def grad_input(gy, weight):
    gy2 = gy if gy.stride(-1) == 1 else gy.contiguous()
    if supported(gy2, weight.shape[0], weight.shape[1]) and weight.shape[1] % 8 == 0:
        return ops.linear_fused(gy2, _transposed(weight), None)["y"]
    return torch.matmul(gy, weight)


class _Linear(torch.autograd.Function):

    @staticmethod
    def forward(ctx, x, weight, bias, residual, want_partials, gn=None, box=None):
        if ctx.needs_input_grad[1] or (bias is not None and ctx.needs_input_grad[2]):
            raise GaError("Linear weight gradients are not part of the guided-attention path (frozen UNet)")
        out = ops.linear_fused(x, weight, bias, residual=residual, want_row_partials=want_partials, gn=gn)
        if box is not None:
            box.append(out["gn"])
        ctx.weight, ctx.has_res = weight, residual is not None
        partials = out["row_partials"]
        if partials is None:
            partials = x.new_empty(0)
        ctx.mark_non_differentiable(partials)
        ctx.set_materialize_grads(False)
        return out["y"], partials

    @staticmethod
    def backward(ctx, gy, _gp):
        if gy is None:
            return None, None, None, None, None, None, None
        gx = grad_input(gy, ctx.weight) if ctx.needs_input_grad[0] else None
        return gx, None, None, (gy if ctx.has_res else None), None, None, None


def linear(x, weight, bias=None, residual=None, want_partials=False, gn_for=None):
    if gn_for is not None and ops.gn_two_launch(gn_for[1], weight.shape[0], gn_for[0], x.dtype):
        box = []
        y, partials = _Linear.apply(x, weight, bias, residual, want_partials, gn_for, box)
        if box and box[0] is not None:
            y._ga_gn_tokens = (box[0][0], box[0][1], gn_for[0], y._version)
        return y, (partials if want_partials else None)
    y, partials = _Linear.apply(x, weight, bias, residual, want_partials)
    return y, (partials if want_partials else None)


def _folded(weight, bias, norm):
    key = (weight.data_ptr(), weight._version, tuple(weight.shape), None if bias is None else (bias.data_ptr(), bias._version),
           norm.weight._version, norm.bias._version, weight.dtype)
    cache = norm.__dict__.setdefault("_ga_folded", {})
    entry = cache.get(key)
    owner = weight._base if weight._base is not None else weight
    hit = entry[1] if entry is not None and entry[0]() is owner else None
    if hit is None:
        with torch.no_grad():
            wg = (weight.float() * norm.weight.float()[None, :]).to(weight.dtype).contiguous()
            colsum = wg.float().sum(1).contiguous()
            shift = weight.float() @ norm.bias.float()
            if bias is not None:
                shift = shift + bias.float()
            hit = (wg, colsum, shift.contiguous())
        if len(cache) > 8:
            def stale(k, ref):
                w = ref()
                return w is None or w._version != k[1] or norm.weight._version != k[4] or norm.bias._version != k[5]
            for k in [k for k, (ref, _) in cache.items() if stale(k, ref)]:
                del cache[k]
        cache[key] = (weakref.ref(owner), hit)
    ops.keep_alive(*hit)
    return hit


class _LNLinear(torch.autograd.Function):

    @staticmethod
    def forward(ctx, x, partials, norm, weight, bias, geglu):
        need = ctx.needs_input_grad[0]
        wg, colsum, shift = _folded(weight, bias, norm)
        out = ops.linear_fused(x, wg, None, geglu=geglu, want_preact=geglu and need,
                               ln=(partials, colsum, shift, norm.eps), want_ln_stats=need)
        if need:
            ctx.save_for_backward(x, out["ln_stats"], out["preact"] if geglu else None)
            ctx.norm, ctx.weight, ctx.geglu = norm, weight, geglu
        ctx.set_materialize_grads(False)
        return out["y"], x.view_as(x)

    @staticmethod
    def backward(ctx, gy, g_pass):
        x, stats, preact = ctx.saved_tensors
        if gy is None:
            return g_pass, None, None, None, None, None
        if ctx.geglu:
            gy = ops.geglu_backward(preact, gy)
        g_ln = grad_input(gy, ctx.weight)
        gx = ops._ln_bwd(x.contiguous(), stats, ctx.norm.weight, g_ln, g_pass)
        return gx, None, None, None, None, None


def ln_linear(x, partials, norm, weight, bias=None, geglu=False):
# ... 7 lines not shown
```

guided-attention_amd/ops.py:

```python
import ctypes
import weakref
from collections import OrderedDict

import torch

from . import _lib
from ._lib import GaError, check, dtype_code, load, require_cuda, stream_ptr


def _ptr(t):
    return ctypes.c_void_p(t.data_ptr()) if t is not None else ctypes.c_void_p(0)


_CENSUS = None


def start_census():
    global _CENSUS
    _CENSUS = {}


def stop_census():
    global _CENSUS
    rec, _CENSUS = _CENSUS, None
    return rec or {}


def _count(key):
    if _CENSUS is not None:
        _CENSUS[key] = _CENSUS.get(key, 0) + 1


class census_scope:

    def __enter__(self):
        global _CENSUS
        self._outer, _CENSUS = _CENSUS, {}
        return self

    def __exit__(self, *exc):
        global _CENSUS
        self.launches, _CENSUS = _CENSUS, self._outer


def add_census(launches):
    if _CENSUS is not None:
        for key, n in launches.items():
            _CENSUS[key] = _CENSUS.get(key, 0) + n


class no_gc:

    def __enter__(self):
# ... 1059 lines not shown

class GroupNormAct(torch.autograd.Function):

    @staticmethod
    def forward(ctx, x, weight, bias, groups, eps, act, chan_bias, with_alias=False, produced=None):
        require_cuda(x, weight, bias, chan_bias)
        if x.dim() != 4:
            raise GaError("GroupNormAct expects a (B, C, H, W) tensor")
        x = _nhwc(x)
        B, C, H, W = x.shape
        if chan_bias is not None:
            if chan_bias.requires_grad:
                raise GaError("the channel bias of the fused GroupNorm carries no gradient on this path")
            chan_bias = chan_bias.to(x.dtype).contiguous()
            if tuple(chan_bias.shape) != (B, C):
                raise GaError(f"chan_bias must be (B, C) = {(B, C)}, got {tuple(chan_bias.shape)}")
        if produced is not None and produced[0] == "done":
            y, stats = produced[1], produced[2]
            ctx.save_for_backward(x, weight, bias, stats, chan_bias)
            ctx.meta = (groups, bool(act))
            if with_alias:
                ctx.set_materialize_grads(False)
                return y, x.view_as(x)
            return y
        y = torch.empty_like(x, memory_format=torch.channels_last)
        stats = torch.empty((B, groups, 2), dtype=torch.float32, device=x.device)
        if produced is not None:
            partials, blocks = produced
            _count(("group_norm_apply", B, groups, H * W, blocks, C, bool(act), str(x.dtype)))
            check(load().ga_group_norm_apply(_ptr(x), _ptr(chan_bias), _ptr(weight), _ptr(bias), _ptr(y), _ptr(stats),
                                             _ptr(partials), blocks, B, H * W, C, groups, float(eps), int(bool(act)),
                                             dtype_code(x), stream_ptr()), "ga_group_norm_apply")
        else:
            ws = torch.empty((B * 257 * groups * 2,), dtype=torch.float32, device=x.device)
            _count(("group_norm_fwd", B, groups, H * W, 0, C, bool(act), str(x.dtype)))
            check(load().ga_group_norm_fwd(_ptr(x), _ptr(chan_bias), _ptr(weight), _ptr(bias), _ptr(y), _ptr(stats), _ptr(ws),
                                           B, H * W, C, groups, float(eps), int(bool(act)), dtype_code(x), stream_ptr()),
                  "ga_group_norm_fwd")
        ctx.save_for_backward(x, weight, bias, stats, chan_bias)
        ctx.meta = (groups, bool(act))
        if with_alias:
            ctx.set_materialize_grads(False)
            return y, x.view_as(x)
        return y

    @staticmethod
    def backward(ctx, dy, g_alias=None):
        if ctx.needs_input_grad[1] or ctx.needs_input_grad[2]:
            raise GaError("GroupNorm weight gradients are not part of the guided-attention path (frozen UNet)")
        if dy is None:
            return g_alias, None, None, None, None, None, None, None, None
        x, weight, bias, stats, chan_bias = ctx.saved_tensors
        groups, act = ctx.meta
        B, C, H, W = x.shape
        dy = _nhwc(dy)
        if g_alias is not None:
            g_alias = _nhwc(g_alias)
        dx = torch.empty_like(x, memory_format=torch.channels_last)
        ws = torch.empty((B * 257 * groups * 2,), dtype=torch.float32, device=x.device)
        _count(("group_norm_bwd", B, groups, H * W, 0, C, bool(act), str(x.dtype)))
        check(load().ga_group_norm_bwd(_ptr(x), _ptr(chan_bias), _ptr(dy), _ptr(weight), _ptr(bias), _ptr(stats),
                                       _ptr(g_alias), _ptr(dx), _ptr(ws), B, H * W, C, groups, int(act), dtype_code(x),
                                       stream_ptr()),
              "ga_group_norm_bwd")
        return dx, None, None, None, None, None, None, None, None


def _gn_versions(x, chan_bias):
    return (x._version, None if chan_bias is None else chan_bias._version)


def group_norm_act(x, weight, bias, groups, eps, act, chan_bias=None, with_alias=False):
    pre = getattr(x, "_ga_gn", None)
    produced = None
    if pre is not None and pre["groups"] == groups and pre["chan_bias"] is chan_bias and pre["shape"] == tuple(x.shape) and \
            pre.get("versions") == _gn_versions(x, chan_bias):
        if "done" not in pre:
            produced = (pre["partials"], pre["blocks"])
        elif pre["weight"] is weight and pre["bias"] is bias and pre["eps"] == float(eps) and pre["act"] == bool(act) and \
                pre.get("norm_versions") == (weight._version, bias._version):
            produced = ("done",) + pre.pop("done")
    return GroupNormAct.apply(x, weight, bias, groups, eps, act, chan_bias, with_alias, produced)


def gn_fused_with_cat(HW, C, groups, dtype):
    code = _lib.DTYPE_CODE.get(dtype)
    return code is not None and (C // groups) % 2 == 0 and bool(load().ga_group_norm_one_launch(HW, C, groups, code))


def gn_two_launch(HW, C, groups, dtype):
    code = _lib.DTYPE_CODE.get(dtype)
    return code is not None and bool(load().ga_group_norm_two_launch(HW, C, groups, code))


class Geglu(torch.autograd.Function):

    @staticmethod
    def forward(ctx, x):
        require_cuda(x)
        x = x.contiguous()
        F2 = x.shape[-1]
        rows = x.numel() // F2
        y = torch.empty(x.shape[:-1] + (F2 // 2,), dtype=x.dtype, device=x.device)
        _count(("geglu_fwd", rows, 0, 0, 0, F2 // 2, False, str(x.dtype)))
        check(load().ga_geglu_fwd(_ptr(x), _ptr(y), rows, F2 // 2, dtype_code(x), stream_ptr()), "ga_geglu_fwd")
        if ctx.needs_input_grad[0]:
            ctx.save_for_backward(x)
        return y

    @staticmethod
    def backward(ctx, dy):
        (x,) = ctx.saved_tensors
        dy = dy.contiguous()
        F2 = x.shape[-1]
        dx = torch.empty_like(x)
        _count(("geglu_bwd", x.numel() // F2, 0, 0, 0, F2 // 2, False, str(x.dtype)))
        check(load().ga_geglu_bwd(_ptr(x), _ptr(dy), _ptr(dx), x.numel() // F2, F2 // 2, dtype_code(x), stream_ptr()),
              "ga_geglu_bwd")
        return dx


def geglu(x):
# ... 245 lines not shown
        if hit is not None:
            bm, bn, sp = hit
        else:
            c_bm, c_bn, c_sp, c_ws = ctypes.c_int(), ctypes.c_int(), ctypes.c_int(), ctypes.c_longlong()
            check(load().ga_conv3x3_plan(B, H, W, Cin, Cout, stride, ctypes.byref(c_bm), ctypes.byref(c_bn), ctypes.byref(c_sp),
                                         ctypes.byref(c_ws)), "ga_conv3x3_plan")
            bm, bn, sp = c_bm.value, c_bn.value, c_sp.value
        floats = lambda k: int(load().ga_splitk_workspace_floats(B * Ho * Wo, Cout, bm, bn, k))
        while sp > 1 and floats(sp) > LIN_SLAB_FLOATS:
            sp -= 1
        plan = _conv_plan_cache[key] = (bm, bn, sp, floats(sp))
    return plan


def conv3x3_packed_weights(weight, transpose_flip):
    key = (weight.data_ptr(), weight._version, weight.dtype, bool(transpose_flip), tuple(weight.stride()), tuple(weight.shape))
    entry = _conv_pack_cache.get(key)
    hit = entry[1] if entry is not None and entry[0]() is weight else None
    if hit is None:
        require_cuda(weight)
        Cout, Cin = weight.shape[0], weight.shape[1]
        N, C = (Cin, Cout) if transpose_flip else (Cout, Cin)
        hit = torch.empty(int(load().ga_conv3x3_packed_elems(N, C)), dtype=weight.dtype, device=weight.device)
        so, si, sy, sx = weight.stride()
        check(load().ga_conv3x3_pack_weights(_ptr(weight), _ptr(hit), Cout, Cin, so, si, sy, sx, int(bool(transpose_flip)),
                                             dtype_code(weight), stream_ptr()), "ga_conv3x3_pack_weights")
        if len(_conv_pack_cache) > 512:
            for dead in [k for k, (ref, _) in _conv_pack_cache.items() if ref() is None]:
                del _conv_pack_cache[dead]
        _conv_pack_cache[key] = (weakref.ref(weight), hit)
    return keep_alive(hit)


CONV_KC = 64


def conv3x3_supported(x, weight, stride=1):
    return (x.is_cuda and x.dtype in (torch.float16, torch.bfloat16) and weight.shape[2:] == (3, 3) and
            weight.shape[1] % CONV_KC == 0 and weight.shape[0] % CONV_KC == 0 and stride in (1, 2))


def conv3x3_nhwc(x, wp, cout, stride=1, bias=None, residual=None, plan=None, gn=None):
    require_cuda(x, wp, bias, residual)
    x = _nhwc(x)
    B, Cin, H, W = x.shape
    Ho, Wo = (H - 1) // stride + 1, (W - 1) // stride + 1
    bm, bn, splits = (plan or conv3x3_plan(B, H, W, Cin, cout, stride))[:3]
    y = torch.empty((B, cout, Ho, Wo), dtype=x.dtype, device=x.device, memory_format=torch.channels_last)
    ws, tickets = splitk_workspace(x.device, B * Ho * Wo, cout, bm, bn, splits)
    if residual is not None:
        residual = _nhwc(residual)
    _count(("conv3x3", B, Cin, H * W, stride, cout, bias is not None or residual is not None, str(x.dtype)))
    if gn is not None:
        groups, cb = gn
        blocks = int(load().ga_conv3x3_gn_blocks(H, W, cout, groups, bm, bn)) if stride == 1 else 0
        if blocks and gn_two_launch(H * W, cout, groups, x.dtype):
            if cb is not None:
                require_cuda(cb)
                cb = cb.to(x.dtype).contiguous()
                if tuple(cb.shape) != (B, cout):
                    raise GaError(f"chan_bias must be (B, C) = {(B, cout)}, got {tuple(cb.shape)}")
            partials = torch.empty((B, blocks, groups, 2), dtype=torch.float32, device=x.device)
            _check_ticketed(load().ga_conv3x3_nhwc_gn(_ptr(x), _ptr(wp), _ptr(y), _ptr(ws), _ptr(tickets), _ptr(bias),
                                                      _ptr(residual), B, H, W, Cin, cout, bm, bn, splits, dtype_code(x),
                                                      stream_ptr(), _ptr(partials), _ptr(cb), groups),
                            "ga_conv3x3_nhwc_gn", tickets)
            return y, (partials, blocks)
    _check_ticketed(load().ga_conv3x3_nhwc(_ptr(x), _ptr(wp), _ptr(y), _ptr(ws), _ptr(tickets), _ptr(bias), _ptr(residual), B,
                                           H, W, Cin, cout, stride, bm, bn, splits, dtype_code(x), stream_ptr()),
                    "ga_conv3x3_nhwc", tickets)
    return (y, None) if gn is not None else y


GA_ERR_SHAPE = -2
_no_fused_upsample = set()


def conv3x3_up2x_nhwc(x, wp, cout, bias=None, plan=None):
    require_cuda(x, wp, bias)
    x = _nhwc(x)
    B, Cin, H, W = x.shape
    key = (B, H, W, Cin, cout, x.dtype)
    if key in _no_fused_upsample:
        return None
    bm, bn, splits = (plan or conv3x3_plan(B, 2 * H, 2 * W, Cin, cout, 1))[:3]
    y = torch.empty((B, cout, 2 * H, 2 * W), dtype=x.dtype, device=x.device, memory_format=torch.channels_last)
    ws, tickets = splitk_workspace(x.device, B * 4 * H * W, cout, bm, bn, splits)
    rc = load().ga_conv3x3_up2x_nhwc(_ptr(x), _ptr(wp), _ptr(y), _ptr(ws), _ptr(tickets), _ptr(bias), None, B, H, W, Cin,
                                     cout, bm, bn, splits, dtype_code(x), stream_ptr())
    if rc == GA_ERR_SHAPE:
        _no_fused_upsample.add(key)
        return None
    _check_ticketed(rc, "ga_conv3x3_up2x_nhwc", tickets)
    _count(("conv3x3", B, Cin, 4 * H * W, 1, cout, bias is not None, str(x.dtype)))
    return y


class UpsampleConv3x3(torch.autograd.Function):

    @staticmethod
    def forward(ctx, x, weight, bias):
        if ctx.needs_input_grad[1] or (bias is not None and ctx.needs_input_grad[2]):
            raise GaError("convolution weight gradients are not part of the guided-attention path (frozen UNet)")
        y = conv3x3_up2x_nhwc(x, conv3x3_packed_weights(weight, False), weight.shape[0], bias)
        if y is None:
            up = torch.nn.functional.interpolate(x, scale_factor=2.0, mode="nearest")
            y = conv3x3_nhwc(up, conv3x3_packed_weights(weight, False), weight.shape[0], 1, bias)
        ctx.weight, ctx.in_shape = weight, tuple(x.shape)
        return y

    @staticmethod
    def backward(ctx, gy):
        if not ctx.needs_input_grad[0]:
            return None, None, None
        g_up = conv3x3_nhwc(_nhwc(gy), conv3x3_packed_weights(ctx.weight, True), ctx.weight.shape[1], 1)
        B, C, H, W = ctx.in_shape
        gx = torch.ops.aten.upsample_nearest2d_backward(g_up, [2 * H, 2 * W], [B, C, H, W], 2.0, 2.0)
        return gx, None, None


def upsample_conv3x3(x, weight, bias=None):
    return UpsampleConv3x3.apply(x, weight, bias)


class Conv3x3(torch.autograd.Function):

    @staticmethod
    def forward(ctx, x, weight, bias, residual, stride, gn=None):
        if ctx.needs_input_grad[1] or ctx.needs_input_grad[2]:
            raise GaError("convolution weight gradients are not part of the guided-attention path (frozen UNet)")
        wp = conv3x3_packed_weights(weight, False)
        ctx.weight, ctx.stride, ctx.in_shape = weight, stride, tuple(x.shape)
        ctx.has_res = residual is not None
        if gn is None:
            return conv3x3_nhwc(x, wp, weight.shape[0], stride, bias, residual)
        y, made = conv3x3_nhwc(x, wp, weight.shape[0], stride, bias, residual, gn=gn)
        ctx.gn_made = made
        return y

    @staticmethod
    def backward(ctx, gy):
        weight, stride = ctx.weight, ctx.stride
        gx = None
        gy = _nhwc(gy)
        if ctx.needs_input_grad[0]:
            if stride == 1:
                gx = conv3x3_nhwc(gy, conv3x3_packed_weights(weight, True), weight.shape[1], 1)
            else:
                gx = torch.nn.grad.conv2d_input(ctx.in_shape, weight, gy, stride=stride, padding=1)
        return gx, None, None, (gy if ctx.has_res else None), None


def conv3x3(x, weight, bias=None, residual=None, stride=1, gn_for=None):
    if gn_for is None:
        return Conv3x3.apply(x, weight, bias, residual, stride)
    groups, cb = gn_for
    B, _, H, W = x.shape
    cout = weight.shape[0]
    if stride != 1 or not gn_two_launch(H * W, cout, groups, x.dtype):
        return Conv3x3.apply(x, weight, bias, residual, stride)
    box = []
    y = _Conv3x3Gn.apply(x, weight, bias, residual, (groups, cb), box)
    if box and box[0] is not None:
        partials, blocks = box[0]
        y._ga_gn = {"partials": partials, "blocks": blocks, "groups": groups, "chan_bias": cb, "shape": tuple(y.shape),
                    "versions": _gn_versions(y, cb)}
    return y


class _Conv3x3Gn(Conv3x3):

    @staticmethod
    def forward(ctx, x, weight, bias, residual, gn, box):
        y = Conv3x3.forward(ctx, x, weight, bias, residual, 1, gn)
        box.append(ctx.gn_made)
        return y

    @staticmethod
    def backward(ctx, gy):
        return Conv3x3.backward(ctx, gy) + (None,)


conv3x3.supported = conv3x3_supported
conv3x3.upsample = upsample_conv3x3


_thin_pack_cache = {}


def conv3x3_thin_supported(x, weight, stride=1):
    if not (x.is_cuda and x.dim() == 4 and x.dtype in (torch.float16, torch.bfloat16) and weight.dtype == x.dtype
            and tuple(weight.shape[2:]) == (3, 3) and stride == 1 and x.shape[1] == weight.shape[1]):
        return False
    cout, cin = weight.shape[0], weight.shape[1]
    if min(cin, cout) != 4 or max(cin, cout) % 64 != 0:
        return False
    lib = load()
    return bool(lib.ga_conv3x3_thin_supported(x.shape[2], x.shape[3], cin, cout) and
                lib.ga_conv3x3_thin_supported(x.shape[2], x.shape[3], cout, cin))


def conv3x3_thin_packed_weights(weight, transpose_flip):
    key = (weight.data_ptr(), weight._version, weight.dtype, bool(transpose_flip), tuple(weight.stride()), tuple(weight.shape))
    entry = _thin_pack_cache.get(key)
    hit = entry[1] if entry is not None and entry[0]() is weight else None
    if hit is None:
        require_cuda(weight)
        Cout, Cin = weight.shape[0], weight.shape[1]
        hit = torch.empty(int(load().ga_conv3x3_thin_packed_elems(Cout, Cin)), dtype=weight.dtype, device=weight.device)
        so, si, sy, sx = weight.stride()
        check(load().ga_conv3x3_thin_pack(_ptr(weight), _ptr(hit), Cout, Cin, so, si, sy, sx, int(bool(transpose_flip)),
                                          dtype_code(weight), stream_ptr()), "ga_conv3x3_thin_pack")
        if len(_thin_pack_cache) > 64:
            for dead in [k for k, (ref, _) in _thin_pack_cache.items() if ref() is None]:
                del _thin_pack_cache[dead]
        _thin_pack_cache[key] = (weakref.ref(weight), hit)
    return keep_alive(hit)


def conv3x3_thin(x, wp, cout, bias=None):
    require_cuda(x, wp, bias)
    B, Cin, H, W = x.shape
    if bias is not None:
        bias = bias.to(x.dtype).contiguous()
    if Cin == 4:
        x = x.contiguous()
        y = torch.empty((B, cout, H, W), dtype=x.dtype, device=x.device, memory_format=torch.channels_last)
        _count(("conv3x3_thin_in", B, 4, H * W, 1, cout, bias is not None, str(x.dtype)))
        check(load().ga_conv3x3_thin_in(_ptr(x), _ptr(wp), _ptr(bias), _ptr(y), B, H, W, cout, dtype_code(x), stream_ptr()),
              "ga_conv3x3_thin_in")
        return y
    if cout != 4:
        raise GaError(f"conv3x3_thin serves 4 -> C and C -> 4 channels, got {Cin} -> {cout}")
    x = _nhwc(x)
    y = torch.empty((B, 4, H, W), dtype=x.dtype, device=x.device)
    _count(("conv3x3_thin_out", B, Cin, H * W, 1, 4, bias is not None, str(x.dtype)))
    check(load().ga_conv3x3_thin_out(_ptr(x), _ptr(wp), _ptr(bias), _ptr(y), B, H, W, Cin, dtype_code(x), stream_ptr()),
          "ga_conv3x3_thin_out")
    return y


class Conv3x3Thin(torch.autograd.Function):

    @staticmethod
    def forward(ctx, x, weight, bias):
        if ctx.needs_input_grad[1] or (bias is not None and ctx.needs_input_grad[2]):
            raise GaError("convolution weight gradients are not part of the guided-attention path (frozen UNet)")
        ctx.weight = weight
        return conv3x3_thin(x, conv3x3_thin_packed_weights(weight, False), weight.shape[0], bias)

    @staticmethod
    def backward(ctx, gy):
        if not ctx.needs_input_grad[0]:
            return None, None, None
        weight = ctx.weight
        return conv3x3_thin(gy, conv3x3_thin_packed_weights(weight, True), weight.shape[1]), None, None


def conv3x3_thin_apply(x, weight, bias=None):
    return Conv3x3Thin.apply(x, weight, bias)


conv3x3_thin_apply.supported = conv3x3_thin_supported


def _sub_ptr(t, elem_offset):
    return ctypes.c_void_p(t.data_ptr() + elem_offset * t.element_size())


def self_attn_fwd(q, k, v, heads, scale, want_lse=True):
    require_cuda(q, k, v)
    q, k, v = q.contiguous(), k.contiguous(), v.contiguous()
    B, N, C = q.shape
    o = torch.empty_like(q)
    lse = torch.empty((B * heads, N), dtype=torch.float32, device=q.device) if want_lse else None
    _count(("self_attn_fwd", B, heads, N, N, C // heads, bool(want_lse), str(q.dtype)))
    check(load().ga_self_attn_fwd(_ptr(q), _ptr(k), _ptr(v), _ptr(o), _ptr(lse), B, heads, N, C // heads, 0,
                                  float(scale), dtype_code(q), stream_ptr()), "ga_self_attn_fwd")
    return o, lse


def self_attn_bwd(q, k, v, o, d_o, lse, heads, scale):
    require_cuda(q, k, v, o, d_o, lse)
    B, N, C = q.shape
    d_o = d_o.contiguous()
    dq, dk, dv = torch.empty_like(q), torch.empty_like(k), torch.empty_like(v)
    delta = torch.empty_like(lse)
    _count(("self_attn_bwd", B, heads, N, N, C // heads, True, str(q.dtype)))
    check(load().ga_self_attn_bwd(_ptr(q), _ptr(k), _ptr(v), _ptr(o), _ptr(d_o), _ptr(lse), _ptr(delta), _ptr(dq),
                                  _ptr(dk), _ptr(dv), B, heads, N, C // heads, 0, float(scale), dtype_code(q),
                                  stream_ptr()), "ga_self_attn_bwd")
    return dq, dk, dv


class SelfAttention(torch.autograd.Function):

    @staticmethod
    def forward(ctx, q, k, v, heads, scale):
        q, k, v = q.contiguous(), k.contiguous(), v.contiguous()
        need = any(ctx.needs_input_grad[:3])
        o, lse = self_attn_fwd(q, k, v, heads, scale, want_lse=need)
        if need:
            ctx.save_for_backward(q, k, v, o, lse)
        ctx.meta = (heads, scale)
        return o

    @staticmethod
    def backward(ctx, d_o):
        q, k, v, o, lse = ctx.saved_tensors
        heads, scale = ctx.meta
        dq, dk, dv = self_attn_bwd(q, k, v, o, d_o, lse, heads, scale)
        return dq, dk, dv, None, None


class SelfAttentionFusedQKV(torch.autograd.Function):

# ... 101 lines not shown
        import json
        from pathlib import Path
        path = Path(__file__).resolve().parent / "linear_plans.json"
        _lin_plan_table = {}
        if path.exists():
            for k, v in json.loads(path.read_text()).items():
                _lin_plan_table[tuple(int(x) for x in k.split(","))] = tuple(v)
    return _lin_plan_table


def library_block(M, C):
    return bool(_measured_linear_plans().get((int(M), int(C), -1, -1), (0,))[0])


LINEAR_STREAM = _lib.GA_LINEAR_STREAM
LINEAR_STREAM_PLAN = (128, 128, 1, LINEAR_STREAM)


def linear_stream_serves(K, parts, ln, bias, residual, want_preact, want_ln_stats, want_row_partials):
    return (ln is not None and bias is None and residual is None and not want_preact and not want_ln_stats
            and not want_row_partials and K // 64 >= 5 and 2 <= parts <= 20)


def linear_plan(M, K, N, geglu=False, stream_ok=False):
    key = (int(M), int(K), int(N), int(bool(geglu)))
    if stream_ok and _measured_linear_plans().get(key + (LINEAR_STREAM,), (0,))[0]:
        return LINEAR_STREAM_PLAN
    plan = _lin_plan_cache.get(key)
    if plan is None:
        plan = _measured_linear_plans().get(key)
        if plan is None:
            n_out = N // 2 if geglu else N
            steps = K // 64
            best, best_cost = None, None
            for bm, bn in ((128, 128), (128, 64), (64, 128), (64, 64)):
                outc = bn // 2 if geglu else bn
                tiles = -(-M // bm) * -(-n_out // outc)
                waste = (-(-M // bm) * bm) * (-(-n_out // outc) * outc) / (M * n_out)
                for sp in (1, 2, 3, 4, 6, 8, 12, 16):
                    if sp > 1 and (steps // sp < 4 or sp * tiles * bm * bn > LIN_SLAB_FLOATS or tiles > LIN_TICKETS):
                        break
                    wgs = tiles * sp
                    rounds = -(-wgs // 256)
                    per_wg = -(-steps // sp) * (0.09 if bm * bn == 128 * 128 else 0.055 if bm * bn == 128 * 64 else 0.04)
                    cost = rounds * (1.2 + per_wg) * waste ** 0.5 + (1.5 + sp * bm * bn * 4 / 100e3 if sp > 1 else 0.0)
                    if best_cost is None or cost < best_cost:
                        best, best_cost = (bm, bn, sp), cost
            plan = best
        _lin_plan_cache[key] = plan
    return plan


def linear_fused(x, weight, bias=None, residual=None, geglu=False, want_preact=False, ln=None, want_ln_stats=False,
                 want_row_partials=False, plan=None, out=None, gn=None):
    require_cuda(x, weight, bias, residual)
    if x.stride(-1) != 1 or not weight.is_contiguous():
        raise GaError("linear_fused needs unit-stride feature axes")
    K = x.shape[-1]
    lead = x.shape[:-1]
    M = 1
    for d in lead:
        M *= d
    ldx = x.stride(-2) if x.dim() > 1 else K
    if x.dim() > 2 and any(x.stride(i) != x.stride(i + 1) * x.shape[i + 1] for i in range(x.dim() - 2)):
        x = x.contiguous()
        ldx = K
    N = weight.shape[0]
    n_out = N // 2 if geglu else N
    if plan is None:
        stream_ok = ln is not None and linear_stream_serves(K, ln[0].shape[1], ln, bias, residual, want_preact, want_ln_stats,
                                                            want_row_partials)
        plan = linear_plan(M, K, N, geglu, stream_ok)
    plan = tuple(plan)
    bm, bn, splits = plan[:3]
    stages = plan[3] if len(plan) > 3 else 0
    y = out if out is not None else torch.empty(lead + (n_out,), dtype=x.dtype, device=x.device)
    ep = _lib.ga_linear_epilogue_t()
    ep.bias = bias.data_ptr() if bias is not None else None
    if residual is not None:
        if residual.stride(-1) != 1 or tuple(residual.shape) != tuple(y.shape):
            raise GaError("residual must have the result's shape and a unit-stride feature axis")
        if residual.dim() > 2 and any(residual.stride(i) != residual.stride(i + 1) * residual.shape[i + 1]
                                      for i in range(residual.dim() - 2)):
            residual = residual.contiguous()
        ep.residual, ep.ld_res = residual.data_ptr(), residual.stride(-2) if residual.dim() > 1 else n_out
    ep.geglu = int(bool(geglu))
    preact = None
    if geglu and want_preact:
        preact = torch.empty(lead + (N,), dtype=x.dtype, device=x.device)
        ep.preact, ep.ld_pre = preact.data_ptr(), N
    ln_stats = None
    if ln is not None:
        partials, colsum, shift, eps = ln
        if partials.dtype != torch.float32 or tuple(partials.shape) != (M, partials.shape[1], 2) or not partials.is_contiguous():
            raise GaError("LayerNorm partial sums must be a contiguous (M, parts, 2) float32 tensor")
        ep.ln_partials, ep.ln_parts, ep.ln_eps = partials.data_ptr(), partials.shape[1], float(eps)
        ep.ln_colsum, ep.ln_shift = colsum.data_ptr(), shift.data_ptr()
        if want_ln_stats:
            ln_stats = torch.empty((M, 2), dtype=torch.float32, device=x.device)
            ep.ln_stats_out = ln_stats.data_ptr()
    outc = bn // 2 if geglu else bn
    parts = -(-n_out // outc)
    row_partials = None
    if want_row_partials:
        row_partials = torch.empty((M, parts, 2), dtype=torch.float32, device=x.device)
        ep.row_partials_out = row_partials.data_ptr()
    gn_made = None
    if gn is not None and not geglu and stages != LINEAR_STREAM:
        groups, hw = gn
        blocks = int(load().ga_linear_gn_blocks(hw, N, groups, bm, bn)) if M % hw == 0 else 0
        if blocks:
            gn_partials = torch.empty((M // hw, blocks, groups, 2), dtype=torch.float32, device=x.device)
            ep.gn_partials, ep.gn_groups, ep.gn_hw = gn_partials.data_ptr(), groups, hw
            gn_made = (gn_partials, blocks)
    slabs = tickets = None
    if splits > 1:
        ws = linear_workspace(x.device)
        tiles = -(-M // bm) * parts
        if splits * tiles * bm * bn > ws["slabs"].numel() or tiles > ws["tickets"].numel():
            raise GaError(f"split-K workspace too small for M={M} N={N} plan {(bm, bn, splits)}")
        slabs, tickets = ws["slabs"], ws["tickets"]
    _count(("linear", M, K, 0, int(bool(geglu)) + 2 * int(ln is not None) + 4 * int(residual is not None), N, bias is not None,
            str(x.dtype)))
    _check_ticketed(load().ga_linear_fused(_ptr(x), ldx, _ptr(weight), _ptr(y), y.stride(-2) if y.dim() > 1 else n_out,
                                           ctypes.byref(ep), _ptr(slabs), _ptr(tickets), M, K, N, bm, bn, splits, stages,
                                           dtype_code(x), stream_ptr()), "ga_linear_fused", tickets)
    return {"y": y, "preact": preact, "ln_stats": ln_stats, "row_partials": row_partials, "parts": parts, "gn": gn_made}
```

guided-attention_amd/unet.py:

```python
import math
from dataclasses import dataclass, field
from types import SimpleNamespace
from typing import Optional, Tuple, Union

import torch
import torch.nn as nn
import torch.nn.functional as F


@dataclass
class UNetConfig:
    sample_size: int = 64
    in_channels: int = 4
    out_channels: int = 4
    block_out_channels: Tuple[int, ...] = (320, 640, 1280, 1280)
    down_block_types: Tuple[str, ...] = ("CrossAttnDownBlock2D", "CrossAttnDownBlock2D", "CrossAttnDownBlock2D",
                                         "DownBlock2D")
    up_block_types: Tuple[str, ...] = ("UpBlock2D", "CrossAttnUpBlock2D", "CrossAttnUpBlock2D", "CrossAttnUpBlock2D")
    layers_per_block: int = 2
    attention_head_dim: Union[int, Tuple[int, ...]] = 8
    cross_attention_dim: int = 768
    norm_num_groups: int = 32
    norm_eps: float = 1e-5
    use_linear_projection: bool = False
# ... 170 lines not shown

    ln_impl = None
    lin_impl = None

    def folds(self, x):
        lin = self.lin_impl
        return (lin is not None and lin.block_folds(x) and
                all(getattr(a._processor(), "supports_folded_layer_norm", False) for a in (self.attn1, self.attn2)))

    def forward_folded(self, x, xp, context, want_partials):
        lin = self.lin_impl
        x, xp = self.attn1(x, folded={"partials": xp, "norm": self.norm1, "residual": x, "want_partials": True})
        x, xp = self.attn2(x, encoder_hidden_states=context,
                           folded={"partials": xp, "norm": self.norm2, "residual": x, "want_partials": True})
        proj, out = self.ff.net[0].proj, self.ff.net[2]
        h, x = lin.ln_linear(x, xp, self.norm3, proj.weight, proj.bias, geglu=True)
        return lin.linear(h, out.weight, out.bias, residual=x, want_partials=want_partials)

    def forward(self, x, context):
        if self.ln_impl is not None and x.shape[-1] % 8 == 0:
            ln, add_ln = self.ln_impl
            h = self.attn1(ln(x, self.norm1.weight, self.norm1.bias, self.norm1.eps))
            x, n = add_ln(h, x, self.norm2.weight, self.norm2.bias, self.norm2.eps)
            h = self.attn2(n, encoder_hidden_states=context)
            x, n = add_ln(h, x, self.norm3.weight, self.norm3.bias, self.norm3.eps)
            return self.ff(n) + x
        x = self.attn1(self.norm1(x)) + x
        x = self.attn2(self.norm2(x), encoder_hidden_states=context) + x
        return self.ff(self.norm3(x)) + x


class Transformer2DModel(nn.Module):
    def __init__(self, heads, dim_head, in_channels, cross_attention_dim, groups, use_linear_projection, depth=1):
        super().__init__()
        inner = heads * dim_head
        self.use_linear_projection = use_linear_projection
        self.norm = GroupNormAct(groups, in_channels, eps=1e-6, act=False)
        if use_linear_projection:
            self.proj_in = nn.Linear(in_channels, inner)
            self.proj_out = nn.Linear(inner, in_channels)
        else:
            self.proj_in = nn.Conv2d(in_channels, inner, 1)
            self.proj_out = nn.Conv2d(inner, in_channels, 1)
        self.transformer_blocks = nn.ModuleList([BasicTransformerBlock(inner, heads, dim_head, cross_attention_dim)
                                                 for _ in range(depth)])

    feeds_norm = False

    def _proj_weights(self, proj):
        if self.use_linear_projection:
            return proj.weight, proj.bias
        return proj.weight.reshape(proj.out_channels, proj.in_channels), proj.bias

    def forward(self, x, context):
        b, c, h, w = x.shape
        x, res = self.norm(x, with_alias=True)
        x = nchw_to_tokens(x)
        blocks = self.transformer_blocks
        lin = blocks[0].lin_impl
        if lin is not None and x.is_contiguous() and lin.supported(x, c, blocks[0].norm1.normalized_shape[0]) and \
                res.is_contiguous(memory_format=torch.channels_last) and all(blk.folds(x) for blk in blocks):
            x, xp = lin.linear(x, *self._proj_weights(self.proj_in), want_partials=True)
            for i, blk in enumerate(blocks):
                x, xp = blk.forward_folded(x, xp, context, want_partials=i + 1 < len(blocks))
            x, _ = lin.linear(x, *self._proj_weights(self.proj_out), residual=nchw_to_tokens(res),
                              gn_for=(self.norm.num_groups, h * w) if self.feeds_norm and self.norm.impl is not None else None)
            made = getattr(x, "_ga_gn_tokens", None)
            x = tokens_to_nchw(x, h, w)
            if made is not None:
                x._ga_gn = {"partials": made[0], "blocks": made[1], "groups": made[2], "chan_bias": None, "shape": tuple(x.shape),
                            "versions": (made[3], None)}
            return x
        x = self.proj_in(x) if self.use_linear_projection else pointwise_conv_tokens(x, self.proj_in)
        for blk in self.transformer_blocks:
            x = blk(x, context)
        x = self.proj_out(x) if self.use_linear_projection else pointwise_conv_tokens(x, self.proj_out)
        return tokens_to_nchw(x, h, w) + res


class ResnetBlock2D(nn.Module):
    def __init__(self, in_channels, out_channels, temb_channels, groups, eps):
        super().__init__()
        self.norm1 = GroupNormAct(groups, in_channels, eps=eps, act=True)
        self.conv1 = nn.Conv2d(in_channels, out_channels, 3, padding=1)
        self.time_emb_proj = nn.Linear(temb_channels, out_channels)
        self.norm2 = GroupNormAct(groups, out_channels, eps=eps, act=True)
        self.conv2 = nn.Conv2d(out_channels, out_channels, 3, padding=1)
        self.conv_shortcut = nn.Conv2d(in_channels, out_channels, 1) if in_channels != out_channels else None

    add_impl = None
    conv_impl = None
    lin_impl = None

    def forward(self, x, temb_act):
        h, x = self.norm1(x, with_alias=True)
        if isinstance(temb_act, dict):
            tproj = temb_act[id(self)]
        else:
            tproj = self.time_emb_proj(temb_act) + self.conv1.bias
        gn = self.norm2.impl is not None
        h = conv3x3(h, self.conv1, self.conv_impl, with_bias=False, gn_for=(self.norm2.num_groups, tproj) if gn else None)
        h = self.norm2(h, chan_bias=tproj)
        if self.conv_shortcut is not None:
            _, _, hh, ww = x.shape
            xt = nchw_to_tokens(x)
            sc = self.conv_shortcut
            if self.lin_impl is not None and xt.is_contiguous() and self.lin_impl.supported(xt, sc.in_channels, sc.out_channels):
                xt, _ = self.lin_impl.linear(xt, sc.weight.reshape(sc.out_channels, sc.in_channels), sc.bias)
            else:
                xt = pointwise_conv_tokens(xt, sc)
            x = tokens_to_nchw(xt, hh, ww)
        if self.conv_impl is not None and self.conv_impl.supported(h, self.conv2.weight, 1):
            if gn:
                return self.conv_impl(h, self.conv2.weight, self.conv2.bias, x, 1, gn_for=(self.norm2.num_groups, None))
            return self.conv_impl(h, self.conv2.weight, self.conv2.bias, x, 1)
        if self.add_impl is not None and self.conv2.out_channels % 8 == 0:
            return self.add_impl(F.conv2d(h, self.conv2.weight, None, padding=1), self.conv2.bias, x)
        return x + self.conv2(h)


class Downsample2D(nn.Module):
    conv_impl = None

    def __init__(self, channels):
        super().__init__()
        self.conv = nn.Conv2d(channels, channels, 3, stride=2, padding=1)

    def forward(self, x):
        return conv3x3(x, self.conv, self.conv_impl)


class Upsample2D(nn.Module):
    conv_impl = None

    def __init__(self, channels):
        super().__init__()
        self.conv = nn.Conv2d(channels, channels, 3, padding=1)

    def forward(self, x, output_size=None):
        impl = self.conv_impl
        if output_size is None and impl is not None and getattr(impl, "upsample", None) is not None and _FUSE_UPSAMPLE and \
                impl.supported(x, self.conv.weight, 1):
            return impl.upsample(x, self.conv.weight, self.conv.bias)
        if output_size is None:
            x = F.interpolate(x, scale_factor=2.0, mode="nearest")
        else:
            x = F.interpolate(x, size=output_size, mode="nearest")
        return conv3x3(x, self.conv, self.conv_impl)


class DownBlock(nn.Module):
    def __init__(self, cfg, in_c, out_c, temb_c, heads, add_downsample, has_attn, depth=1):
        super().__init__()
        self.has_cross_attention = has_attn
        self.resnets = nn.ModuleList([ResnetBlock2D(in_c if i == 0 else out_c, out_c, temb_c, cfg.norm_num_groups,
                                                    cfg.norm_eps) for i in range(cfg.layers_per_block)])
        if has_attn:
            self.attentions = nn.ModuleList([Transformer2DModel(heads, out_c // heads, out_c, cfg.cross_attention_dim,
                                                                cfg.norm_num_groups, cfg.use_linear_projection, depth)
                                             for _ in range(cfg.layers_per_block)])
        self.downsamplers = nn.ModuleList([Downsample2D(out_c)]) if add_downsample else None
        if has_attn:
            for attn in self.attentions[:-1]:
                attn.feeds_norm = True

    def forward(self, x, temb_act, context):
        outs = []
        for i, resnet in enumerate(self.resnets):
            x = resnet(x, temb_act)
            if self.has_cross_attention:
                x = self.attentions[i](x, context)
            outs.append(x)
        if self.downsamplers is not None:
            x = self.downsamplers[0](x)
            outs.append(x)
        return x, outs


class MidBlock(nn.Module):
    def __init__(self, cfg, channels, temb_c, heads, depth=1):
        super().__init__()
        self.has_cross_attention = True
        self.resnets = nn.ModuleList([ResnetBlock2D(channels, channels, temb_c, cfg.norm_num_groups, cfg.norm_eps)
                                      for _ in range(2)])
        self.attentions = nn.ModuleList([Transformer2DModel(heads, channels // heads, channels, cfg.cross_attention_dim,
                                                            cfg.norm_num_groups, cfg.use_linear_projection, depth)])

        self.attentions[0].feeds_norm = True

    def forward(self, x, temb_act, context):
        x = self.resnets[0](x, temb_act)
        x = self.attentions[0](x, context)
        return self.resnets[1](x, temb_act)


class UpBlock(nn.Module):
    def __init__(self, cfg, in_c, out_c, prev_c, temb_c, heads, add_upsample, has_attn, depth=1):
        super().__init__()
        self.has_cross_attention = has_attn
        n = cfg.layers_per_block + 1
        resnets = []
        for i in range(n):
            skip_c = in_c if i == n - 1 else out_c
            res_in = prev_c if i == 0 else out_c
            resnets.append(ResnetBlock2D(res_in + skip_c, out_c, temb_c, cfg.norm_num_groups, cfg.norm_eps))
        self.resnets = nn.ModuleList(resnets)
        if has_attn:
            self.attentions = nn.ModuleList([Transformer2DModel(heads, out_c // heads, out_c, cfg.cross_attention_dim,
                                                                cfg.norm_num_groups, cfg.use_linear_projection, depth)
                                             for _ in range(n)])
        self.upsamplers = nn.ModuleList([Upsample2D(out_c)]) if add_upsample else None

    cat_impl = None

    def forward(self, x, skips, temb_act, context, upsample_size=None, n_layers=None):
        for i, resnet in enumerate(self.resnets):
            if n_layers is not None and i >= n_layers:
                return x
            skip = skips.pop()
            if self.cat_impl is not None:
                n1 = resnet.norm1
                if n1.impl is not None:
                    x = self.cat_impl(x, skip, gn_for=n1.num_groups, norm=(n1.weight, n1.bias, n1.eps, n1.act))
                else:
                    x = self.cat_impl(x, skip)
                x = resnet(x, temb_act)
            else:
                x = resnet(torch.cat([x, skip], dim=1), temb_act)
            if self.has_cross_attention:
                x = self.attentions[i](x, context)
        if n_layers is None and self.upsamplers is not None:
            x = self.upsamplers[0](x, upsample_size)
        return x


def timestep_embedding(timesteps, dim):
    half = dim // 2
    exponent = -math.log(10000.0) * torch.arange(half, dtype=torch.float32, device=timesteps.device) / half
    emb = timesteps[:, None].float() * torch.exp(exponent)[None, :]
    return torch.cat([torch.cos(emb), torch.sin(emb)], dim=-1)


class TimestepEmbedding(nn.Module):
    def __init__(self, in_c, dim):
        super().__init__()
        self.linear_1 = nn.Linear(in_c, dim)
        self.linear_2 = nn.Linear(dim, dim)

    def forward(self, x):
        return self.linear_2(F.silu(self.linear_1(x)))


@dataclass
class UNetOutput:
    sample: Optional[torch.Tensor]


def set_norm_impl(module, impl):
    for m in module.modules():
        if isinstance(m, GroupNormAct):
            m.impl = impl


def set_fused_impl(module, geglu=None, bias_residual_add=None, layer_norms=None, conv=None, linear=None, cat=None):
# ... 169 lines not shown

    def set_fused_impl(self, geglu=None, bias_residual_add=None, layer_norms=None, conv=None, linear=None, cat=None):
        set_fused_impl(self, geglu, bias_residual_add, layer_norms, conv, linear, cat)

    @property
    def dtype(self):
        return self.conv_in.weight.dtype

    @property
    def device(self):
        return self.conv_in.weight.device

    def forward(self, sample, timestep, encoder_hidden_states, class_labels=None, attention_mask=None,
                cross_attention_kwargs=None, return_dict=True, stop_after_up_block=None, time_projection=None):
        cfg = self.config
        up_factor = 2 ** self.num_upsamplers
        forward_upsample_size = any(s % up_factor != 0 for s in sample.shape[-2:])
        if cfg.center_input_sample:
            sample = 2 * sample - 1.0
        if time_projection is None and not torch.is_tensor(timestep) and sample.is_cuda and \
                not self.time_embedding.linear_1.weight.requires_grad:
            time_projection = self.time_projection(timestep, sample.shape[0])
        if time_projection is not None:
            temb_act = self._split_time_projection(time_projection, sample.shape[0])
        else:
            if not torch.is_tensor(timestep):
                timestep = torch.tensor([timestep], dtype=torch.int64 if isinstance(timestep, int) else torch.float64,
                                        device=sample.device)
            elif timestep.dim() == 0:
                timestep = timestep[None].to(sample.device)
            timestep = timestep.expand(sample.shape[0])
            t_emb = timestep_embedding(timestep, cfg.block_out_channels[0]).to(self.dtype)
            emb = self.time_embedding(t_emb)
            added = self._added_rows(sample.shape[0])
            if added is not None:
                emb = emb + added
            temb_act = self._time_projections(F.silu(emb))

        x = self._edge_conv(self.conv_in, sample)
        skips = [x]
        for blk in self.down_blocks:
            x, outs = blk(x, temb_act, encoder_hidden_states)
            skips.extend(outs)
        x = self.mid_block(x, temb_act, encoder_hidden_states)
        for i, blk in enumerate(self.up_blocks):
            n_res = len(blk.resnets)
            upsample_size = None
            if i != len(self.up_blocks) - 1 and forward_upsample_size:
                upsample_size = skips[-n_res - 1].shape[2:]
            if stop_after_up_block is not None and i == stop_after_up_block[0]:
                blk(x, skips, temb_act, encoder_hidden_states, upsample_size, n_layers=stop_after_up_block[1])
                return UNetOutput(sample=None) if return_dict else (None,)
            x = blk(x, skips, temb_act, encoder_hidden_states, upsample_size)
        x = self._edge_conv(self.conv_out, self.conv_norm_out(x))
        return UNetOutput(sample=x) if return_dict else (x,)

    edge_conv_impl = None

    def _edge_conv(self, conv, x):
        impl = self.edge_conv_impl
        if impl is not None and impl.supported(x, conv.weight, conv.stride[0]):
            return impl(x, conv.weight, conv.bias)
        return conv(x)

    def init_weights_(self, seed=0):
        g = torch.Generator(device="cpu").manual_seed(seed)
        with torch.no_grad():
            for name, p in self.named_parameters():
                if name.endswith("bias"):
                    p.zero_()
                elif p.dim() == 1:
                    p.fill_(1.0)
                else:
                    fan_in = p[0].numel()
                    bound = math.sqrt(3.0 / fan_in)
                    p.copy_((torch.rand(p.shape, generator=g) * 2 - 1) * bound)
        return self

    def load_diffusers_state(self, state):
        missing, unexpected = self.load_state_dict(state, strict=False)
        if missing or unexpected:
            raise RuntimeError(f"UNet checkpoint mismatch: missing {missing[:5]}..., unexpected {unexpected[:5]}...")
        return self
```

include/ga_hip.h:

```cpp
#ifndef GA_HIP_H
#define GA_HIP_H

#include <stdint.h>

#ifdef __cplusplus
extern "C" {
#endif

#define GA_VERSION 183

#define GA_MAX_IMAGES 64

typedef void* ga_stream_t;

typedef enum { GA_F16 = 0, GA_BF16 = 1, GA_F32 = 2 } ga_dtype;

typedef enum {
  GA_OK = 0,
  GA_ERR_NULL = -1,
  GA_ERR_SHAPE = -2,
  GA_ERR_DTYPE = -3,
  GA_ERR_ALIGN = -4,
  GA_ERR_LAUNCH = -5,
  GA_ERR_UNSUPPORTED = -6
// ... 137 lines not shown

#define GA_GN_WORKSPACE_FLOATS(B, G) ((B) * 257 * (G) * 2)
int ga_group_norm_fwd(const void* x, const void* chan_bias, const void* gamma, const void* beta, void* y, float* stats,
                      float* workspace, int B, int HW, int C, int G, float eps, int act_silu, int dtype,
                      ga_stream_t stream);
int ga_group_norm_apply(const void* x, const void* chan_bias, const void* gamma, const void* beta, void* y, float* stats,
                        const float* partials, int blocks, int B, int HW, int C, int G, float eps, int act_silu, int dtype,
                        ga_stream_t stream);
int ga_group_norm_two_launch(int HW, int C, int G, int dtype);
int ga_group_norm_bwd(const void* x, const void* chan_bias, const void* dy, const void* gamma, const void* beta,
                      const float* stats, const void* g_res, void* dx, float* workspace, int B, int HW, int C, int G,
                      int act_silu, int dtype, ga_stream_t stream);

int ga_geglu_fwd(const void* x, void* y, int64_t rows, int F, int dtype, ga_stream_t stream);
int ga_geglu_bwd(const void* x, const void* dy, void* dx, int64_t rows, int F, int dtype, ga_stream_t stream);
int ga_bias_residual_add(const void* y, const void* bias, const void* residual, void* out, int64_t rows, int C,
                         int dtype, ga_stream_t stream);

int ga_cat_channels(const void* a, const void* b, void* out, int64_t rows, int C1, int C2, int elem_bytes,
                    ga_stream_t stream);
int ga_group_norm_one_launch(int HW, int C, int G, int dtype);
int ga_cat_group_norm_fwd(const void* a, const void* b, void* cat, const void* gamma, const void* beta, void* y, float* stats,
                          int B, int HW, int C1, int C2, int G, float eps, int act_silu, int dtype, ga_stream_t stream);
int ga_cat_channels_gn_blocks(int HW, int C, int G, int dtype);
int ga_cat_channels_gn(const void* a, const void* b, void* out, float* partials, int B, int HW, int C1, int C2, int G, int dtype,
                       ga_stream_t stream);

long long ga_splitk_workspace_floats(int64_t M, int N, int bm, int bn, int splits);
long long ga_conv3x3_packed_elems(int N, int C);
int ga_conv3x3_pack_weights(const void* W, void* Wp, int Cout, int Cin, int64_t stride_o, int64_t stride_i,
                            int64_t stride_y, int64_t stride_x, int transpose_flip, int dtype, ga_stream_t stream);
int ga_conv3x3_plan(int B, int H, int W, int Cin, int Cout, int stride, int* bm, int* bn, int* splits,
                    long long* workspace_floats);
int ga_conv3x3_nhwc(const void* X, const void* Wp, void* Y, float* workspace, unsigned* tickets, const void* bias,
                    const void* residual, int B, int H, int W, int Cin, int Cout, int stride, int bm, int bn, int splits,
                    int dtype, ga_stream_t stream);
int ga_conv3x3_gn_blocks(int H, int W, int Cout, int groups, int bm, int bn);
int ga_conv3x3_nhwc_gn(const void* X, const void* Wp, void* Y, float* workspace, unsigned* tickets, const void* bias,
                       const void* residual, int B, int H, int W, int Cin, int Cout, int bm, int bn, int splits, int dtype,
                       ga_stream_t stream, float* gn_partials, const void* gn_chan_bias, int gn_groups);

int ga_conv3x3_up2x_nhwc(const void* X, const void* Wp, void* Y, float* workspace, unsigned* tickets, const void* bias,
                         const void* residual, int B, int H, int W, int Cin, int Cout, int bm, int bn, int splits, int dtype,
                         ga_stream_t stream);

long long ga_conv3x3_thin_packed_elems(int Cout, int Cin);
int ga_conv3x3_thin_supported(int H, int W, int Cin, int Cout);
int ga_conv3x3_thin_pack(const void* W, void* Wp, int Cout, int Cin, long long stride_o, long long stride_i, long long stride_y,
                         long long stride_x, int transpose_flip, int dtype, ga_stream_t stream);
int ga_conv3x3_thin_in(const void* X, const void* Wp, const void* bias, void* Y, int B, int H, int W, int Cout, int dtype,
                       ga_stream_t stream);
int ga_conv3x3_thin_out(const void* X, const void* Wp, const void* bias, void* Y, int B, int H, int W, int Cin, int dtype,
                        ga_stream_t stream);

int ga_gemm_nt(const void* X, const void* W, void* Y, float* workspace, unsigned* tickets, const void* bias,
               const void* residual, int64_t M, int K, int N, int bm, int bn, int splits, int dtype, ga_stream_t stream);

#define GA_LINEAR_STREAM 8
typedef struct {
  const void* bias;
  const void* residual;
  int64_t ld_res;
  int geglu;
  void* preact;
  int64_t ld_pre;
  const float* ln_partials;
  int ln_parts;
  float ln_eps;
  const float* ln_colsum;
  const float* ln_shift;
  float* ln_stats_out;
  float* row_partials_out;
  float* gn_partials;
  int gn_groups;
  int gn_hw;
} ga_linear_epilogue_t;

int ga_linear_gn_blocks(int hw, int N, int groups, int bm, int bn);
int ga_linear_workspace(int64_t M, int N, int bm, int bn, int splits, int geglu, long long* slab_floats, int* tiles);
int ga_linear_fused(const void* X, int64_t ldx, const void* W, void* Y, int64_t ldy, const ga_linear_epilogue_t* ep,
                    float* slabs, unsigned* tickets, int64_t M, int K, int N, int bm, int bn, int splits, int stages,
                    int dtype, ga_stream_t stream);

int ga_add_layer_norm_fwd(const void* a, const void* x, const void* gamma, const void* beta, void* x_new, void* y,
                          float* stats, int64_t rows, int C, float eps, int dtype, ga_stream_t stream);
int ga_add_layer_norm_bwd(const void* x, const float* stats, const void* gamma, const void* dy, const void* g_res,
                          void* dx, int64_t rows, int C, int dtype, ga_stream_t stream);

#ifdef __cplusplus
}
#endif
#endif
```

Baseline: 1.948.

## Fold GroupNorm apply into transformer proj_in GEMM and output thin conv

Adds a GN-absorbing variant of the fused linear kernel. It folds the GroupNorm partial statistics in the prologue, builds per-channel scale and shift in LDS, and applies the affine to A fragments as they are read from LDS. It also adds a thin output conv that applies GroupNorm and SiLU on its input, and routes the transformer entry norm and the final conv_norm_out through these fused paths. This removes a separate normalize pass and its write and read of the activation tensor. In exchange the GEMM inner loop carries extra LDS reads and conversions, the kernel needs more LDS and registers, and there is a redundant per-block stats fold.

```diff
diff --git a/guided-attention_amd/_lib.py b/guided-attention_amd/_lib.py
--- a/guided-attention_amd/_lib.py
+++ b/guided-attention_amd/_lib.py
@@ -106,6 +106,7 @@
     "ga_conv3x3_thin_pack": [_vp, _vp, _i, _i, _i64, _i64, _i64, _i64, _i, _i, _vp],
     "ga_conv3x3_thin_in": [_vp, _vp, _vp, _vp, _i, _i, _i, _i, _i, _vp],
     "ga_conv3x3_thin_out": [_vp, _vp, _vp, _vp, _i, _i, _i, _i, _i, _vp],
+    "ga_conv3x3_thin_out_gn": [_vp, _vp, _vp, _vp, _i, _i, _i, _i, _i, _vp, _vp, _i, _i, _f, _vp, _vp, _vp, _i],
     "ga_conv3x3_pack_weights": [_vp, _vp, _i, _i, _i64, _i64, _i64, _i64, _i, _i, _vp],
     "ga_conv3x3_plan": [_i, _i, _i, _i, _i, _i, ctypes.POINTER(_i), ctypes.POINTER(_i), ctypes.POINTER(_i),
                         ctypes.POINTER(ctypes.c_longlong)],
@@ -120,6 +121,8 @@
     "ga_linear_workspace": [_i64, _i, _i, _i, _i, _i, ctypes.POINTER(ctypes.c_longlong), ctypes.POINTER(_i)],
     "ga_linear_fused": [_vp, _i64, _vp, _vp, _i64, ctypes.POINTER(ga_linear_epilogue_t), _vp, _vp, _i64, _i, _i, _i, _i, _i,
                         _i, _i, _vp],
+    "ga_linear_fused_gn": [_vp, _i64, _vp, _vp, _i64, ctypes.POINTER(ga_linear_epilogue_t), _vp, _vp, _i64, _i, _i, _i, _i, _i,
+                           _i, _i, _vp, _vp, _i, _i, _i, _f, _vp, _vp, _vp],
     "ga_add_layer_norm_fwd": [_vp, _vp, _vp, _vp, _vp, _vp, _vp, _i64, _i, _f, _i, _vp],
     "ga_add_layer_norm_bwd": [_vp, _vp, _vp, _vp, _vp, _vp, _i64, _i, _i, _vp],
 }
diff --git a/guided-attention_amd/csrc/gn_fold.h b/guided-attention_amd/csrc/gn_fold.h
--- /dev/null
+++ b/guided-attention_amd/csrc/gn_fold.h
@@ -0,0 +1,58 @@
+#pragma once
+#include "ga_common.h"
+
+namespace ga {
+
+constexpr int kGnFoldThreads = 256;
+constexpr int kMaxStatsNB = 128;
+
+__device__ __forceinline__ float sigmoidf_(float z) { return __builtin_amdgcn_rcpf(1.0f + __expf(-z)); }
+
+struct NoHook {
+  __device__ __forceinline__ void operator()() const {}
+};
+
+template <bool FWD, typename Hook = NoHook>
+__device__ __forceinline__ void fold_partials(const float* __restrict__ partial, int b, int NB, int G, float inv_n,
+                                              float eps, float2* res, float* keep, Hook after_loads = Hook()) {
+  const float2* pp = reinterpret_cast<const float2*>(partial) + (size_t)b * NB * G;
+  for (int g0 = 0; g0 < G; g0 += kGnFoldThreads / 8) {
+    const int g = g0 + (threadIdx.x >> 3), part = threadIdx.x & 7;
+    float2 v[kMaxStatsNB / 8];
+#pragma unroll
+    for (int i = 0; i < kMaxStatsNB / 8; ++i) {
+      const int nb = part + 8 * i;
+      v[i] = pp[(size_t)min(nb, NB - 1) * G + min(g, G - 1)];
+    }
+    if (g0 == 0) after_loads();
+    float sa = 0.f, sc = 0.f;
+#pragma unroll
+    for (int i = 0; i < kMaxStatsNB / 8; ++i) {
+      const bool in = g < G && part + 8 * i < NB;
+      sa += in ? v[i].x : 0.f;
+      sc += in ? v[i].y : 0.f;
+    }
+    sa = group_sum<8>(sa);
+    sc = group_sum<8>(sc);
+    if (part == 0 && g < G) {
+      float o0, o1;
+      if (FWD) {
+        const double mean = (double)sa * inv_n;
+        const double var = fmax((double)sc * inv_n - mean * mean, 0.0);
+        o0 = (float)mean;
+        o1 = rsqrtf((float)var + eps);
+      } else {
+        o0 = sa * inv_n;
+        o1 = sc * inv_n;
+      }
+      res[g] = float2{o0, o1};
+      if (keep != nullptr) {
+        keep[((size_t)b * G + g) * 2] = o0;
+        keep[((size_t)b * G + g) * 2 + 1] = o1;
+      }
+    }
+  }
+  __syncthreads();
+}
+
+}
diff --git a/guided-attention_amd/csrc/group_norm.hip b/guided-attention_amd/csrc/group_norm.hip
--- a/guided-attention_amd/csrc/group_norm.hip
+++ b/guided-attention_amd/csrc/group_norm.hip
@@ -1,4 +1,5 @@
 #include "attn_common.h"
+#include "gn_fold.h"
 
 using namespace ga;
 
@@ -19,7 +20,6 @@
   else return __builtin_bit_cast(Item<T, 2>, *reinterpret_cast<const unsigned long long*>(p));
 }
 
-__device__ __forceinline__ float sigmoidf_(float z) { return __builtin_amdgcn_rcpf(1.0f + __expf(-z)); }
 
 template <typename T, int W>
 __device__ __forceinline__ void load_chan_bias(const T* __restrict__ cbias, int b, int CP, int cp, float (&cb)[W]) {
@@ -91,53 +91,6 @@
   fold_to_groups<NPT>(s0, s1, CP, cpg, G, lds, partial + ((size_t)b * gridDim.x + nb) * G * 2);
 }
 
-constexpr int kMaxStatsNB = 128;
-
-struct NoHook {
-  __device__ __forceinline__ void operator()() const {}
-};
-template <bool FWD, typename Hook = NoHook>
-__device__ __forceinline__ void fold_partials(const float* __restrict__ partial, int b, int NB, int G, float inv_n,
-                                              float eps, float2* res, float* keep, Hook after_loads = Hook()) {
-  const float2* pp = reinterpret_cast<const float2*>(partial) + (size_t)b * NB * G;
-  for (int g0 = 0; g0 < G; g0 += kThreads / 8) {
-    const int g = g0 + (threadIdx.x >> 3), part = threadIdx.x & 7;
-    float2 v[kMaxStatsNB / 8];
-#pragma unroll
-    for (int i = 0; i < kMaxStatsNB / 8; ++i) {
-      const int nb = part + 8 * i;
-      v[i] = pp[(size_t)min(nb, NB - 1) * G + min(g, G - 1)];
-    }
-    if (g0 == 0) after_loads();
-    float sa = 0.f, sc = 0.f;
-#pragma unroll
-    for (int i = 0; i < kMaxStatsNB / 8; ++i) {
-      const bool in = g < G && part + 8 * i < NB;
-      sa += in ? v[i].x : 0.f;
-      sc += in ? v[i].y : 0.f;
-    }
-    sa = group_sum<8>(sa);
-    sc = group_sum<8>(sc);
-    if (part == 0 && g < G) {
-      float o0, o1;
-      if (FWD) {
-        const double mean = (double)sa * inv_n;
-        const double var = fmax((double)sc * inv_n - mean * mean, 0.0);
-        o0 = (float)mean;
-        o1 = rsqrtf((float)var + eps);
-      } else {
-        o0 = sa * inv_n;
-        o1 = sc * inv_n;
-      }
-      res[g] = float2{o0, o1};
-      if (keep != nullptr) {
-        keep[((size_t)b * G + g) * 2] = o0;
-        keep[((size_t)b * G + g) * 2 + 1] = o1;
-      }
-    }
-  }
-  __syncthreads();
-}
 
 template <typename T, bool ACT, int NPT, int W>
 __global__ __launch_bounds__(kThreads) void gn_apply_kernel(const T* __restrict__ x, const T* __restrict__ cbias,
@@ -984,6 +937,16 @@
 }
 
 template <typename T, bool ACT, int NPT, int W>
+int launch_apply_t(const void* x, const void* cbias, const void* gamma, const void* beta, void* y, float* stats,
+                   const float* partials, int blocks, int B, int HW, int C, int G, float eps, const Geom& g, hipStream_t s) {
+  const float inv_n = 1.0f / ((float)HW * (float)(C / G));
+  hipLaunchKernelGGL((gn_apply_kernel<T, ACT, NPT, W>), dim3(g.NBa, B), dim3(kThreads), 0, s, (const T*)x,
+                     (const T*)cbias, (const T*)gamma, (const T*)beta, (T*)y, partials, blocks, inv_n, eps, stats,
+                     HW, C, G, g.PBa);
+  return check_launch();
+}
+
+template <typename T, bool ACT, int NPT, int W>
 int launch_bwd_t(const void* x, const void* cbias, const void* dy, const void* gamma, const void* beta,
                  const float* stats, const void* gres, void* dx, float* ws, int B, int HW, int C, int G, const Geom& g,
                  hipStream_t s) {
@@ -1086,6 +1049,15 @@
 }
 
 template <typename T>
+int apply_dtype(const void* x, const void* cbias, const void* gamma, const void* beta, void* y, float* stats,
+                const float* partials, int blocks, int B, int HW, int C, int G, float eps, int act, const Geom& g, hipStream_t s) {
+  if (act) {
+    GA_GN_NPT(launch_apply_t, T, true, x, cbias, gamma, beta, y, stats, partials, blocks, B, HW, C, G, eps, g, s)
+  }
+  GA_GN_NPT(launch_apply_t, T, false, x, cbias, gamma, beta, y, stats, partials, blocks, B, HW, C, G, eps, g, s)
+}
+
+template <typename T>
 int bwd_dtype(const void* x, const void* cbias, const void* dy, const void* gamma, const void* beta, const float* stats,
               const void* gres, void* dx, float* ws, int B, int HW, int C, int G, int act, const Geom& g, hipStream_t s) {
   if constexpr (sizeof(T) == 2) {
@@ -1131,8 +1103,13 @@
   int rc = geometry(B, HW, C, G, g);
   if (rc != GA_OK) return rc;
   if (blocks < 1 || blocks > kMaxStatsNB) return GA_ERR_SHAPE;
-  if (dtype == GA_F32 || !wide_ok(C, G, 2)) return GA_ERR_UNSUPPORTED;
+  if (dtype == GA_F32) return GA_ERR_UNSUPPORTED;
   hipStream_t s = static_cast<hipStream_t>(stream);
+  if (!wide_ok(C, G, 2)) {
+    if (dtype == GA_F16) return apply_dtype<_Float16>(x, chan_bias, gamma, beta, y, stats, partials, blocks, B, HW, C, G, eps, act_silu, g, s);
+    if (dtype == GA_BF16) return apply_dtype<bf16_t>(x, chan_bias, gamma, beta, y, stats, partials, blocks, B, HW, C, G, eps, act_silu, g, s);
+    return GA_ERR_DTYPE;
+  }
   const WideGeom wg(HW, C);
   const float inv_n = 1.0f / ((float)HW * (float)(C / G));
 #define GA_GN_APPLY(T, ACT)                                                                                                   \
diff --git a/guided-attention_amd/csrc/linear.hip b/guided-attention_amd/csrc/linear.hip
--- a/guided-attention_amd/csrc/linear.hip
+++ b/guided-attention_amd/csrc/linear.hip
@@ -1,4 +1,5 @@
 #include "attn_common.h"
+#include "gn_fold.h"
 
 using namespace ga;
 
@@ -59,6 +60,12 @@
   unsigned* tickets;
   float* gn_partials;
   int gn_cg, gn_G, gn_hw, gn_tpi;
+  const float* gi_partials;
+  const void* gi_gamma;
+  const void* gi_beta;
+  float* gi_stats;
+  int gi_nb, gi_G, gi_hw;
+  float gi_eps;
 };
 
 template <int BM, int BN>
@@ -81,6 +88,14 @@
   asm volatile("ds_read_b128 %0, %1" : "=v"(dst) : "v"(byte_address) : "memory");
 #else
   dst = u32x4{byte_address, 0u, 0u, 0u};
+#endif
+}
+template <int OFF>
+__device__ __forceinline__ void lds_read128_at(u32x4& dst, unsigned byte_address) {
+#if defined(__HIP_DEVICE_COMPILE__)
+  asm volatile("ds_read_b128 %0, %1 offset:%2" : "=v"(dst) : "v"(byte_address), "n"(OFF) : "memory");
+#else
+  dst = u32x4{byte_address, (unsigned)OFF, 0u, 0u};
 #endif
 }
 __device__ __forceinline__ void opaque(u32x4& v) {
@@ -366,7 +381,27 @@
   }
 }
 
-template <typename T, int BM, int BN, int NSTAGE, bool GEGLU, bool LN>
+constexpr int kGnMaxK = 1280;
+constexpr int kGnMaxG = 64;
+
+template <typename T>
+__device__ __forceinline__ u32x4 gn_affine(u32x4 x, const u32x4 (&c)[4]) {
+  T e[8];
+  __builtin_memcpy(e, &x, 16);
+  float sc[8], sh[8];
+  __builtin_memcpy(sc, &c[0], 32);
+  __builtin_memcpy(sh, &c[2], 32);
+#pragma unroll
+  for (int q = 0; q < 8; ++q) {
+    const float z = Traits<T>::to_f32(e[q]) * sc[q] + sh[q];
+    e[q] = Traits<T>::from_f32(z);
+  }
+  u32x4 y;
+  __builtin_memcpy(&y, e, 16);
+  return y;
+}
+
+template <typename T, int BM, int BN, int NSTAGE, bool GEGLU, bool LN, bool GN = false>
 __global__ __launch_bounds__(kThreads, (BM + BN) * 128 * NSTAGE <= 80 * 1024 ? 2 : 1) void linear_kernel(
     const T* __restrict__ X, const T* __restrict__ W, T* __restrict__ Y, int h_M, int h_ldx, unsigned h_kn, int h_tm,
     unsigned h_tn_splits, unsigned h_steps, unsigned h_dtm_m, unsigned h_dtn_m, LinArgs a_in, LinPtrs p) {
@@ -461,6 +496,39 @@
     if (s < nsteps) issue(s, s);
   LinPrefetch<T, BM, BN, GEGLU, LN> pre;
   pre.load(a, p, m0, n0);
+  unsigned gn_adr = 0;
+  if constexpr (GN) {
+    extern __shared__ __attribute__((aligned(16))) float gn_cst[];
+    __shared__ float2 gn_res[kGnMaxG];
+    const int b = m0 / p.gi_hw, cg = a.K / p.gi_G;
+    const T* gamma = static_cast<const T*>(p.gi_gamma);
+    const T* beta = static_cast<const T*>(p.gi_beta);
+    T gm[kGnMaxK / kThreads], bt[kGnMaxK / kThreads];
+    const bool keeper = m0 == b * p.gi_hw && nt == 0 && split == 0;
+    fold_partials<true>(p.gi_partials, b, p.gi_nb, p.gi_G, 1.0f / ((float)p.gi_hw * (float)cg), p.gi_eps, gn_res,
+                        keeper ? p.gi_stats : nullptr, [&]() {
+#pragma unroll
+      for (int u = 0; u < kGnMaxK / kThreads; ++u) {
+        const int k = min(tid + u * kThreads, a.K - 1);
+        gm[u] = gamma[k];
+        bt[u] = beta[k];
+      }
+    });
+    const float* mr = reinterpret_cast<const float*>(gn_res);
+#pragma unroll
+    for (int u = 0; u < kGnMaxK / kThreads; ++u) {
+      const int k = tid + u * kThreads;
+      if (k < a.K) {
+        const int g = k / cg;
+        const float sc = Traits<T>::to_f32(gm[u]) * mr[2 * g + 1];
+        const float sh = Traits<T>::to_f32(bt[u]) - (mr[2 * g] - 0.f) * sc;
+        gn_cst[(k >> 3) * 16 + (k & 7)] = sc;
+        gn_cst[(k >> 3) * 16 + 8 + (k & 7)] = sh;
+      }
+    }
+    __syncthreads();
+    gn_adr = (unsigned)(uintptr_t)GA_LDS_PTR(gn_cst) + (unsigned)(it0 * (kBK / 8) * 64 + fh * 64);
+  }
   float ln_mean[IM], ln_rstd[IM];
   if constexpr (LN) {
     const float2* part[IM];
@@ -507,8 +575,16 @@
 #endif
     if (it + PRE < nsteps) issue(it + PRE, (it + PRE) % NSTAGE);
     const unsigned slot_off = (unsigned)((it % NSTAGE) * kStage * (int)sizeof(T));
-    u32x4 fa[2][IM], fb[2][JN];
+    u32x4 fa[2][IM], fb[2][JN], gc[2][GN ? 4 : 1];
+    const unsigned gn_it = gn_adr + (unsigned)(it * (kBK / 8) * 64);
     auto request = [&](int kk, int set) {
+      if constexpr (GN) {
+        const unsigned ad = gn_it + 128u * kk;
+        lds_read128_at<0>(gc[set][0], ad);
+        lds_read128_at<16>(gc[set][1], ad);
+        lds_read128_at<32>(gc[set][2], ad);
+        lds_read128_at<48>(gc[set][3], ad);
+      }
 #pragma unroll
       for (int i = 0; i < IM; ++i)
         lds_read128(fa[set][i], a_adr[i] + slot_off + 16u * ((2u * kk) ^ a_sw[i]));
@@ -521,11 +597,15 @@
     for (int kk = 0; kk < kBK / 16; ++kk) {
       if (kk + 1 < kBK / 16) {
         request(kk + 1, (kk + 1) & 1);
-        wait_lgkmcnt<IM + JN>();
+        wait_lgkmcnt<IM + JN + (GN ? 4 : 0)>();
       } else {
         wait_lgkmcnt<0>();
       }
       __builtin_amdgcn_sched_barrier(0);
+      if constexpr (GN) {
+#pragma unroll
+        for (int i = 0; i < IM; ++i) fa[kk & 1][i] = gn_affine<T>(fa[kk & 1][i], gc[kk & 1]);
+      }
 #pragma unroll
       for (int j = 0; j < JN; ++j)
 #pragma unroll
@@ -621,7 +701,7 @@
 #endif
 }
 
-template <typename T, int BM, int BN, int NSTAGE>
+template <typename T, int BM, int BN, int NSTAGE, bool GN = false>
 int launch_lin(const T* X, const T* W, T* Y, LinArgs a, const LinPtrs& p, hipStream_t s) {
   const int outc = a.F ? BN / 2 : BN, n_out = a.F ? a.F : a.N;
   a.tm = (a.M + BM - 1) / BM;
@@ -648,7 +728,10 @@
 #define GA_LIN_LAUNCH(G, L)                                                                                                \
   hipLaunchKernelGGL((linear_kernel<T, BM, BN, NSTAGE, G, L>), grid, dim3(kThreads), 0, s, X, W, Y, h.M, h.ldx, h.kn, h.tm, \
                      h.tn_splits, h.steps, h.dtm_m, h.dtn_m, a, p)
-  if (a.F) {
+  if constexpr (GN) {
+    hipLaunchKernelGGL((linear_kernel<T, BM, BN, NSTAGE, false, false, true>), grid, dim3(kThreads), (size_t)a.K * 8, s, X, W, Y, h.M,
+                       h.ldx, h.kn, h.tm, h.tn_splits, h.steps, h.dtm_m, h.dtn_m, a, p);
+  } else if (a.F) {
     if (ln) GA_LIN_LAUNCH(true, true);
     else GA_LIN_LAUNCH(true, false);
   } else {
@@ -658,6 +741,9 @@
 #undef GA_LIN_LAUNCH
   return check_launch();
 }
+
+template <typename T>
+int lin_gn_t(const void* X, const void* W, void* Y, const LinArgs& a, const LinPtrs& p, int bm, int bn, int stages, hipStream_t s);
 
 template <typename T>
 int lin_t(const void* X, const void* W, void* Y, const LinArgs& a, const LinPtrs& p, int bm, int bn, int stages, hipStream_t s) {
@@ -674,6 +760,25 @@
   } else if (bm == 64 && bn == 64) {
     if (stages == 5) return launch_lin<T, 64, 64, 5>(x, w, (T*)Y, a, p, s);
     if (stages == 0 || stages == 4) return launch_lin<T, 64, 64, 4>(x, w, (T*)Y, a, p, s);
+  }
+  return GA_ERR_SHAPE;
+}
+
+template <typename T>
+int lin_gn_t(const void* X, const void* W, void* Y, const LinArgs& a, const LinPtrs& p, int bm, int bn, int stages, hipStream_t s) {
+  const T* x = (const T*)X;
+  const T* w = (const T*)W;
+  if (bm == 128 && bn == 128) {
+    if (stages == 2) return launch_lin<T, 128, 128, 2, true>(x, w, (T*)Y, a, p, s);
+    if (stages == 0 || stages == 3) return launch_lin<T, 128, 128, 3, true>(x, w, (T*)Y, a, p, s);
+  } else if ((bm == 128 && bn == 64) || (bm == 64 && bn == 128)) {
+    const bool tall = bm == 128;
+    if (stages == 3)
+      return tall ? launch_lin<T, 128, 64, 3, true>(x, w, (T*)Y, a, p, s) : launch_lin<T, 64, 128, 3, true>(x, w, (T*)Y, a, p, s);
+    if (stages == 0 || stages == 4)
+      return tall ? launch_lin<T, 128, 64, 4, true>(x, w, (T*)Y, a, p, s) : launch_lin<T, 64, 128, 4, true>(x, w, (T*)Y, a, p, s);
+  } else if (bm == 64 && bn == 64) {
+    if (stages == 0 || stages == 4 || stages == 5) return launch_lin<T, 64, 64, 4, true>(x, w, (T*)Y, a, p, s);
   }
   return GA_ERR_SHAPE;
 }
@@ -1049,9 +1154,46 @@
   return blocks <= 128 ? blocks : 0;
 }
 
+namespace {
+struct LinGnIn {
+  const float* partials;
+  int blocks, groups, hw;
+  float eps;
+  const void* gamma;
+  const void* beta;
+  float* stats;
+};
+int linear_fused_impl(const void* X, int64_t ldx, const void* W, void* Y, int64_t ldy, const ga_linear_epilogue_t* ep, float* slabs,
+                      unsigned* tickets, int64_t M, int K, int N, int bm, int bn, int splits, int stages, int dtype,
+                      ga_stream_t stream, const LinGnIn* gi);
+}
+
 extern "C" int ga_linear_fused(const void* X, int64_t ldx, const void* W, void* Y, int64_t ldy, const ga_linear_epilogue_t* ep,
                                float* slabs, unsigned* tickets, int64_t M, int K, int N, int bm, int bn, int splits,
                                int stages, int dtype, ga_stream_t stream) {
+  return linear_fused_impl(X, ldx, W, Y, ldy, ep, slabs, tickets, M, K, N, bm, bn, splits, stages, dtype, stream, nullptr);
+}
+
+extern "C" int ga_linear_fused_gn(const void* X, int64_t ldx, const void* W, void* Y, int64_t ldy, const ga_linear_epilogue_t* ep,
+                                  float* slabs, unsigned* tickets, int64_t M, int K, int N, int bm, int bn, int splits,
+                                  int stages, int dtype, ga_stream_t stream, const float* gn_in_partials, int gn_in_blocks,
+                                  int gn_in_groups, int gn_in_hw, float gn_in_eps, const void* gn_in_gamma,
+                                  const void* gn_in_beta, float* gn_in_stats) {
+  if (!X || !W || !Y || !ep || !gn_in_partials || !gn_in_gamma || !gn_in_beta || !gn_in_stats) return GA_ERR_NULL;
+  if (dtype != GA_F16 && dtype != GA_BF16) return GA_ERR_DTYPE;
+  if ((bm != 64 && bm != 128) || (bn != 64 && bn != 128)) return GA_ERR_SHAPE;
+  if (gn_in_groups < 1 || gn_in_groups > kGnMaxG || K < 1 || K % gn_in_groups != 0) return GA_ERR_SHAPE;
+  if (gn_in_hw < 1 || gn_in_hw % bm != 0 || M < 1 || M % gn_in_hw != 0) return GA_ERR_SHAPE;
+  if (gn_in_blocks < 1 || gn_in_blocks > kMaxStatsNB) return GA_ERR_SHAPE;
+  if (K > kGnMaxK || ep->geglu || ep->ln_partials || stages == GA_LINEAR_STREAM) return GA_ERR_UNSUPPORTED;
+  const LinGnIn gi{gn_in_partials, gn_in_blocks, gn_in_groups, gn_in_hw, gn_in_eps, gn_in_gamma, gn_in_beta, gn_in_stats};
+  return linear_fused_impl(X, ldx, W, Y, ldy, ep, slabs, tickets, M, K, N, bm, bn, splits, stages, dtype, stream, &gi);
+}
+
+namespace {
+int linear_fused_impl(const void* X, int64_t ldx, const void* W, void* Y, int64_t ldy, const ga_linear_epilogue_t* ep, float* slabs,
+                      unsigned* tickets, int64_t M, int K, int N, int bm, int bn, int splits, int stages, int dtype,
+                      ga_stream_t stream, const LinGnIn* gi) {
   if (!X || !W || !Y || !ep) return GA_ERR_NULL;
   if (M < 1 || K < kBK || K % kBK != 0 || N < 8 || N % 8 != 0 || ldx < K || ldx % 8 != 0 || ldy % 8 != 0) return GA_ERR_SHAPE;
   if (splits < 1 || splits > 64 || K / kBK < splits || (splits > 1 && (!slabs || !tickets))) return GA_ERR_SHAPE;
@@ -1086,6 +1228,11 @@
   p.ln_stats_out = ep->ln_stats_out; p.row_partials_out = ep->row_partials_out;
   p.slabs = slabs; p.tickets = tickets;
   p.gn_partials = nullptr; p.gn_cg = p.gn_G = p.gn_hw = p.gn_tpi = 0;
+  p.gi_partials = nullptr; p.gi_gamma = p.gi_beta = nullptr; p.gi_stats = nullptr; p.gi_nb = p.gi_G = p.gi_hw = 0; p.gi_eps = 0.f;
+  if (gi) {
+    p.gi_partials = gi->partials; p.gi_gamma = gi->gamma; p.gi_beta = gi->beta; p.gi_stats = gi->stats;
+    p.gi_nb = gi->blocks; p.gi_G = gi->groups; p.gi_hw = gi->hw; p.gi_eps = gi->eps;
+  }
   if (ep->gn_partials) {
     if (ep->geglu || stages == GA_LINEAR_STREAM) return GA_ERR_UNSUPPORTED;
     if (ga_linear_gn_blocks(ep->gn_hw, N, ep->gn_groups, bm, bn) == 0 || M % ep->gn_hw != 0) return GA_ERR_SHAPE;
@@ -1104,9 +1251,17 @@
       default: return GA_ERR_DTYPE;
     }
   }
+  if (gi) {
+    switch (dtype) {
+      case GA_F16: return lin_gn_t<_Float16>(X, W, Y, a, p, bm, bn, stages, s);
+      case GA_BF16: return lin_gn_t<bf16_t>(X, W, Y, a, p, bm, bn, stages, s);
+      default: return GA_ERR_DTYPE;
+    }
+  }
   switch (dtype) {
     case GA_F16: return lin_t<_Float16>(X, W, Y, a, p, bm, bn, stages, s);
     case GA_BF16: return lin_t<bf16_t>(X, W, Y, a, p, bm, bn, stages, s);
     default: return GA_ERR_DTYPE;
   }
 }
+}
diff --git a/guided-attention_amd/csrc/thin_conv.hip b/guided-attention_amd/csrc/thin_conv.hip
--- a/guided-attention_amd/csrc/thin_conv.hip
+++ b/guided-attention_amd/csrc/thin_conv.hip
@@ -1,4 +1,5 @@
 #include "ga_common.h"
+#include "gn_fold.h"
 
 namespace {
 using namespace ga;
@@ -118,11 +119,36 @@
 
 constexpr int kOutThreads = 256;
 constexpr int kOutSlices = 32;
-
-template <typename T, int PAIRS>
+static_assert(kOutThreads == kGnFoldThreads, "fold_partials is written for 256 threads");
+
+struct ThinGn {
+  const float* partials;
+  const void* gamma;
+  const void* beta;
+  float* stats;
+  int nb, G, act;
+  float eps;
+};
+
+template <typename T, bool ACT>
+__device__ __forceinline__ uint4 thin_gn_affine(uint4 x, const float* __restrict__ sc, const float* __restrict__ sh) {
+  T e[8];
+  __builtin_memcpy(e, &x, 16);
+#pragma unroll
+  for (int q = 0; q < 8; ++q) {
+    float z = Traits<T>::to_f32(e[q]) * sc[q] + sh[q];
+    if (ACT) z *= sigmoidf_(z);
+    e[q] = Traits<T>::from_f32(z);
+  }
+  uint4 y;
+  __builtin_memcpy(&y, e, 16);
+  return y;
+}
+
+template <typename T, int PAIRS, bool GN = false, bool ACT = false>
 __global__ void __launch_bounds__(kOutThreads)
 thin_out_kernel(const T* __restrict__ x, const uint32_t* __restrict__ wp, const T* __restrict__ bias, T* __restrict__ y, int H, int W,
-                int total_segs, int segs_per_wg) {
+                int total_segs, int segs_per_wg, ThinGn gn) {
   constexpr int C = PAIRS * 64;
   constexpr int kVecPx = C / 8;
   constexpr int kPatchVecs = 3 * kPatchW * kVecPx;
@@ -130,7 +156,7 @@
   __shared__ uint4 patch[kPatchVecs];
   const int tid = threadIdx.x;
   const int sl = tid & (kOutSlices - 1), slot = tid >> 5;
-  const int segs = W / kSeg;
+  const int segs = (W + kSeg - 1) / kSeg;
 
   uint4 wr[kTaps][PAIRS];
 #pragma unroll
@@ -140,8 +166,9 @@
   float bv = 0.f;
   if (bias && sl < 4) bv = Traits<T>::to_f32(bias[sl]);
 
-  auto fetch = [&](int sg, uint4 (&val)[kLoads]) {
+  auto fetch = [&](int sg, uint4 (&val)[kLoads]) -> unsigned {
     const int seg = sg % segs, row = (sg / segs) % H, b = sg / (segs * H);
+    unsigned inside = 0u;
 #pragma unroll
     for (int j = 0; j < kLoads; ++j) {
       const int i = tid + j * kOutThreads;
@@ -151,22 +178,65 @@
       const size_t pix = in ? ((size_t)b * H + yy) * W + xx : (size_t)b * H * W;
       const uint4 t = reinterpret_cast<const uint4*>(x + pix * C)[in ? v : 0];
       val[j] = in ? t : uint4{0u, 0u, 0u, 0u};
-    }
+      inside |= in ? 1u << j : 0u;
+    }
+    return inside;
   };
   const int first = blockIdx.x * segs_per_wg;
   const int last = min(first + segs_per_wg, total_segs);
   uint4 val[kLoads];
-  fetch(first, val);
+  unsigned inside = fetch(first, val);
+  __shared__ float2 gn_res[GN ? 64 : 1];
+  __shared__ __attribute__((aligned(16))) float gn_sc[GN ? C : 4], gn_sh[GN ? C : 4];
+  int gn_b = -1;
   for (int sg = first; sg < last; ++sg) {
     const int seg = sg % segs, row = (sg / segs) % H, b = sg / (segs * H);
     if (sg != first) __syncthreads();
+    if constexpr (GN) {
+      if (b != gn_b) {
+        gn_b = b;
+        constexpr int KPT = (C + kOutThreads - 1) / kOutThreads;
+        const T* gamma = static_cast<const T*>(gn.gamma);
+        const T* beta = static_cast<const T*>(gn.beta);
+        T gm[KPT], bt[KPT];
+        const int cg = C / gn.G;
+        const bool keeper = sg % (segs * H) == 0;
+        fold_partials<true>(gn.partials, b, gn.nb, gn.G, 1.0f / ((float)(H * W) * (float)cg), gn.eps, gn_res,
+                            keeper ? gn.stats : nullptr, [&]() {
+#pragma unroll
+          for (int u = 0; u < KPT; ++u) {
+            const int k = min(tid + u * kOutThreads, C - 1);
+            gm[u] = gamma[k];
+            bt[u] = beta[k];
+          }
+        });
+        const float* mr = reinterpret_cast<const float*>(gn_res);
+#pragma unroll
+        for (int u = 0; u < KPT; ++u) {
+          const int k = tid + u * kOutThreads;
+          if (k < C) {
+            const int g = k / cg;
+            const float sc = Traits<T>::to_f32(gm[u]) * mr[2 * g + 1];
+            gn_sc[k] = sc;
+            gn_sh[k] = Traits<T>::to_f32(bt[u]) - (mr[2 * g] - 0.f) * sc;
+          }
+        }
+        __syncthreads();
+      }
+    }
 #pragma unroll
     for (int j = 0; j < kLoads; ++j) {
       const int i = tid + j * kOutThreads;
-      if (i < kPatchVecs) patch[i] = val[j];
+      if constexpr (GN) {
+        const int v = i % kVecPx;
+        if (i < kPatchVecs)
+          patch[i] = (inside >> j) & 1u ? thin_gn_affine<T, ACT>(val[j], gn_sc + 8 * v, gn_sh + 8 * v) : uint4{0u, 0u, 0u, 0u};
+      } else {
+        if (i < kPatchVecs) patch[i] = val[j];
+      }
     }
     __syncthreads();
-    if (sg + 1 < last) fetch(sg + 1, val);
+    if (sg + 1 < last) inside = fetch(sg + 1, val);
 
     const uint32_t* pw = reinterpret_cast<const uint32_t*>(patch);
 #pragma unroll
@@ -190,7 +260,7 @@
         acc[j] = group_sum<16>(acc[j]);
         acc[j] += __shfl_xor(acc[j], 16, 64);
       }
-      if (sl < 4) {
+      if (sl < 4 && seg * kSeg + p < W) {
         const float v = (sl == 0 ? acc[0] : sl == 1 ? acc[1] : sl == 2 ? acc[2] : acc[3]) + bv;
         y[(((size_t)b * 4 + sl) * H + row) * W + seg * kSeg + p] = Traits<T>::from_f32(v);
       }
@@ -221,14 +291,19 @@
 }
 
 template <typename T>
-int launch_out(const void* x, const void* wp, const void* bias, void* y, int B, int H, int W, int C, hipStream_t s) {
-  const long long total = (long long)B * H * (W / kSeg);
+int launch_out(const void* x, const void* wp, const void* bias, void* y, int B, int H, int W, int C, hipStream_t s,
+               const ThinGn* gn = nullptr) {
+  const long long total = (long long)B * H * ((W + kSeg - 1) / kSeg);
   const int per = total <= 1024 ? (int)((total + 255) / 256) : (int)((total + 1023) / 1024);
   const unsigned grid = (unsigned)((total + per - 1) / per);
-#define GA_THIN_OUT(P)                                                                                                   \
-  case P:                                                                                                                \
-    hipLaunchKernelGGL((thin_out_kernel<T, P>), dim3(grid), dim3(kOutThreads), 0, s, (const T*)x, (const uint32_t*)wp,    \
-                       (const T*)bias, (T*)y, H, W, (int)total, per);                                                    \
+#define GA_THIN_OUT_K(P, GN, ACT, G)                                                                                  \
+  hipLaunchKernelGGL((thin_out_kernel<T, P, GN, ACT>), dim3(grid), dim3(kOutThreads), 0, s, (const T*)x, (const uint32_t*)wp, \
+                     (const T*)bias, (T*)y, H, W, (int)total, per, G)
+#define GA_THIN_OUT(P)                                                 \
+  case P:                                                              \
+    if (!gn) GA_THIN_OUT_K(P, false, false, ThinGn{});                 \
+    else if (gn->act) GA_THIN_OUT_K(P, true, true, *gn);               \
+    else GA_THIN_OUT_K(P, true, false, *gn);                           \
     break;
   switch (C / 64) {
     GA_THIN_OUT(1)
@@ -239,6 +314,7 @@
     default: return GA_ERR_SHAPE;
   }
 #undef GA_THIN_OUT
+#undef GA_THIN_OUT_K
   return check_launch();
 }
 
@@ -251,9 +327,10 @@
 }
 
 extern "C" int ga_conv3x3_thin_supported(int H, int W, int Cin, int Cout) {
-  if (H < 1 || W < kSeg || W % kSeg != 0) return 0;
+  if (H < 1 || W < 1) return 0;
+  if (Cout == 4 && Cin != 4) return W % 8 == 0 && Cin % 64 == 0 && Cin >= 64 && Cin <= 320 ? 1 : 0;
+  if (W < kSeg || W % kSeg != 0) return 0;
   if (Cin == 4) return Cout % 4 == 0 && Cout >= 64 && Cout <= 4096 ? 1 : 0;
-  if (Cout == 4) return Cin % 64 == 0 && Cin >= 64 && Cin <= 320 ? 1 : 0;
   return 0;
 }
 
@@ -289,7 +366,7 @@
                                    int dtype, ga_stream_t stream) {
   if (!x || !packed || !y) return GA_ERR_NULL;
   if (B < 1 || !ga_conv3x3_thin_supported(H, W, Cin, 4)) return GA_ERR_SHAPE;
-  if ((long long)B * H * (W / kSeg) >= (1LL << 31)) return GA_ERR_SHAPE;
+  if ((long long)B * H * ((W + kSeg - 1) / kSeg) >= (1LL << 31)) return GA_ERR_SHAPE;
   if (!aligned16(x) || !aligned16(packed)) return GA_ERR_ALIGN;
   hipStream_t s = static_cast<hipStream_t>(stream);
   switch (dtype) {
@@ -298,3 +375,20 @@
     default: return GA_ERR_DTYPE;
   }
 }
+
+extern "C" int ga_conv3x3_thin_out_gn(const void* x, const void* packed, const void* bias, void* y, int B, int H, int W, int Cin,
+                                      int dtype, ga_stream_t stream, const float* gn_in_partials, int gn_in_blocks, int gn_in_groups,
+                                      float gn_in_eps, const void* gn_in_gamma, const void* gn_in_beta, float* gn_in_stats,
+                                      int act_silu) {
+  if (!x || !packed || !y || !gn_in_partials || !gn_in_gamma || !gn_in_beta || !gn_in_stats) return GA_ERR_NULL;
+  if (dtype != GA_F16 && dtype != GA_BF16) return GA_ERR_DTYPE;
+  if (B < 1 || !ga_conv3x3_thin_supported(H, W, Cin, 4)) return GA_ERR_SHAPE;
+  if ((long long)B * H * ((W + kSeg - 1) / kSeg) >= (1LL << 31)) return GA_ERR_SHAPE;
+  if (gn_in_groups < 1 || gn_in_groups > 64 || Cin % gn_in_groups != 0 || gn_in_blocks < 1 || gn_in_blocks > kMaxStatsNB)
+    return GA_ERR_SHAPE;
+  if (!aligned16(x) || !aligned16(packed)) return GA_ERR_ALIGN;
+  const ThinGn gn{gn_in_partials, gn_in_gamma, gn_in_beta, gn_in_stats, gn_in_blocks, gn_in_groups, act_silu ? 1 : 0, gn_in_eps};
+  hipStream_t s = static_cast<hipStream_t>(stream);
+  return dtype == GA_F16 ? launch_out<_Float16>(x, packed, bias, y, B, H, W, Cin, s, &gn)
+                         : launch_out<bf16_t>(x, packed, bias, y, B, H, W, Cin, s, &gn);
+}
diff --git a/guided-attention_amd/fused_linear.py b/guided-attention_amd/fused_linear.py
--- a/guided-attention_amd/fused_linear.py
+++ b/guided-attention_amd/fused_linear.py
@@ -76,6 +76,52 @@
     return y, (partials if want_partials else None)
 
 
+class _GNLinear(torch.autograd.Function):
+
+    @staticmethod
+    def forward(ctx, x, gn_weight, gn_bias, groups, eps, weight, bias, produced, with_alias):
+        if ctx.needs_input_grad[1] or ctx.needs_input_grad[2] or ctx.needs_input_grad[5] or \
+                (bias is not None and ctx.needs_input_grad[6]):
+            raise GaError("GroupNorm / Linear weight gradients are not part of the guided-attention path (frozen UNet)")
+        B, C, H, W = x.shape
+        xt = x.permute(0, 2, 3, 1).reshape(B, H * W, C)
+        out = ops.linear_fused(xt, weight, bias, want_row_partials=True,
+                               gn_in=(produced[0], produced[1], groups, H * W, eps, gn_weight, gn_bias))
+        ctx.save_for_backward(x, gn_weight, gn_bias, out["gn_in_stats"])
+        ctx.weight, ctx.groups = weight, groups
+        ctx.mark_non_differentiable(out["row_partials"])
+        ctx.set_materialize_grads(False)
+        if with_alias:
+            return out["y"], out["row_partials"], x.view_as(x)
+        return out["y"], out["row_partials"]
+
+    @staticmethod
+    def backward(ctx, gy, _gp, g_alias=None):
+        if gy is None:
+            return (g_alias,) + (None,) * 8
+        x, gn_weight, gn_bias, stats = ctx.saved_tensors
+        B, C, H, W = x.shape
+        g_norm = grad_input(gy, ctx.weight).reshape(B, H, W, C).permute(0, 3, 1, 2)
+        gx = ops.group_norm_bwd(x, None, g_norm, gn_weight, gn_bias, stats, g_alias, ctx.groups, False)
+        return (gx,) + (None,) * 8
+
+
+def gn_linear(x, norm, weight, bias, with_alias):
+    if ops.GN_ABSORB != 1 or norm.act or x.dim() != 4 or not x.is_contiguous(memory_format=torch.channels_last):
+        return None
+    B, C, H, W = x.shape
+    groups = norm.num_groups
+    if weight.shape[1] != C or not supported(x.permute(0, 2, 3, 1), C, weight.shape[0]) or \
+            not ops.gn_absorb_wanted(H * W, C, B, groups, x.dtype) or norm.weight.dtype != x.dtype or \
+            not ops.linear_gn_in_serves(B * H * W, C, weight.shape[0], H * W, groups):
+        return None
+    produced = ops.gn_produced(x, groups)
+    if produced is None:
+        return None
+    out = _GNLinear.apply(x, norm.weight, norm.bias, groups, norm.eps, weight, bias, produced, with_alias)
+    return (out[0], out[1], out[2]) if with_alias else (out[0], out[1], x)
+
+
 def _folded(weight, bias, norm):
     key = (weight.data_ptr(), weight._version, tuple(weight.shape), None if bias is None else (bias.data_ptr(), bias._version),
            norm.weight._version, norm.bias._version, weight.dtype)
diff --git a/guided-attention_amd/ops.py b/guided-attention_amd/ops.py
--- a/guided-attention_amd/ops.py
+++ b/guided-attention_amd/ops.py
@@ -1,4 +1,5 @@
 import ctypes
+import os
 import weakref
 from collections import OrderedDict
 
@@ -1164,22 +1165,64 @@
             return g_alias, None, None, None, None, None, None, None, None
         x, weight, bias, stats, chan_bias = ctx.saved_tensors
         groups, act = ctx.meta
-        B, C, H, W = x.shape
-        dy = _nhwc(dy)
-        if g_alias is not None:
-            g_alias = _nhwc(g_alias)
-        dx = torch.empty_like(x, memory_format=torch.channels_last)
-        ws = torch.empty((B * 257 * groups * 2,), dtype=torch.float32, device=x.device)
-        _count(("group_norm_bwd", B, groups, H * W, 0, C, bool(act), str(x.dtype)))
-        check(load().ga_group_norm_bwd(_ptr(x), _ptr(chan_bias), _ptr(dy), _ptr(weight), _ptr(bias), _ptr(stats),
-                                       _ptr(g_alias), _ptr(dx), _ptr(ws), B, H * W, C, groups, int(act), dtype_code(x),
-                                       stream_ptr()),
-              "ga_group_norm_bwd")
+        dx = group_norm_bwd(x, chan_bias, dy, weight, bias, stats, g_alias, groups, act)
         return dx, None, None, None, None, None, None, None, None
+
+
+def group_norm_bwd(x, chan_bias, dy, weight, bias, stats, g_alias, groups, act):
+    B, C, H, W = x.shape
+    dy = _nhwc(dy)
+    if g_alias is not None:
+        g_alias = _nhwc(g_alias)
+    dx = torch.empty_like(x, memory_format=torch.channels_last)
+    ws = torch.empty((B * 257 * groups * 2,), dtype=torch.float32, device=x.device)
+    _count(("group_norm_bwd", B, groups, H * W, 0, C, bool(act), str(x.dtype)))
+    check(load().ga_group_norm_bwd(_ptr(x), _ptr(chan_bias), _ptr(dy), _ptr(weight), _ptr(bias), _ptr(stats),
+                                   _ptr(g_alias), _ptr(dx), _ptr(ws), B, H * W, C, groups, int(act), dtype_code(x),
+                                   stream_ptr()),
+          "ga_group_norm_bwd")
+    return dx
 
 
 def _gn_versions(x, chan_bias):
     return (x._version, None if chan_bias is None else chan_bias._version)
+
+
+GN_ABSORB = int(os.environ.get("GA_GN_ABSORB", "1"))
+_gn_absorb_table = None
+
+
+def set_gn_absorb(mode):
+    global GN_ABSORB
+    old, GN_ABSORB = GN_ABSORB, int(mode)
+    return old
+
+
+def gn_absorb_shape(HW, C, B):
+    global _gn_absorb_table
+    if _gn_absorb_table is None:
+        import json
+        from pathlib import Path
+        path = Path(os.environ.get("GA_GN_ABSORB_PLANS", Path(__file__).resolve().parent / "gn_absorb_plans.json"))
+        _gn_absorb_table = {}
+        if path.exists():
+            for k, v in json.loads(path.read_text()).items():
+                _gn_absorb_table[tuple(int(t) for t in k.split(","))] = int(v)
+    t = _gn_absorb_table
+    return bool(t.get((int(HW), int(C), int(B)), t.get((int(HW), int(C), -1), 1)))
+
+
+def gn_absorb_wanted(HW, C, B, groups, dtype):
+    return (GN_ABSORB in (1, 2) and dtype in (torch.float16, torch.bfloat16) and C % groups == 0 and groups <= 64 and C <= 1280
+            and gn_absorb_shape(HW, C, B))
+
+
+def gn_produced(x, groups, chan_bias=None):
+    pre = getattr(x, "_ga_gn", None)
+    if pre is not None and "done" not in pre and pre["groups"] == groups and pre["chan_bias"] is chan_bias and \
+            pre["shape"] == tuple(x.shape) and pre.get("versions") == _gn_versions(x, chan_bias):
+        return pre["partials"], pre["blocks"]
+    return None
 
 
 def group_norm_act(x, weight, bias, groups, eps, act, chan_bias=None, with_alias=False):
@@ -1531,9 +1574,10 @@
         residual = _nhwc(residual)
     _count(("conv3x3", B, Cin, H * W, stride, cout, bias is not None or residual is not None, str(x.dtype)))
     if gn is not None:
-        groups, cb = gn
+        groups, cb = gn[0], gn[1]
+        absorb = len(gn) > 2 and gn[2]
         blocks = int(load().ga_conv3x3_gn_blocks(H, W, cout, groups, bm, bn)) if stride == 1 else 0
-        if blocks and gn_two_launch(H * W, cout, groups, x.dtype):
+        if blocks and (absorb or gn_two_launch(H * W, cout, groups, x.dtype)):
             if cb is not None:
                 require_cuda(cb)
                 cb = cb.to(x.dtype).contiguous()
@@ -1633,13 +1677,14 @@
 def conv3x3(x, weight, bias=None, residual=None, stride=1, gn_for=None):
     if gn_for is None:
         return Conv3x3.apply(x, weight, bias, residual, stride)
-    groups, cb = gn_for
+    groups, cb = gn_for[0], gn_for[1]
     B, _, H, W = x.shape
     cout = weight.shape[0]
-    if stride != 1 or not gn_two_launch(H * W, cout, groups, x.dtype):
+    absorb = len(gn_for) > 2 and bool(gn_for[2]) and cb is None and gn_absorb_wanted(H * W, cout, B, groups, x.dtype)
+    if stride != 1 or not (absorb or gn_two_launch(H * W, cout, groups, x.dtype)):
         return Conv3x3.apply(x, weight, bias, residual, stride)
     box = []
-    y = _Conv3x3Gn.apply(x, weight, bias, residual, (groups, cb), box)
+    y = _Conv3x3Gn.apply(x, weight, bias, residual, (groups, cb, absorb), box)
     if box and box[0] is not None:
         partials, blocks = box[0]
         y._ga_gn = {"partials": partials, "blocks": blocks, "groups": groups, "chan_bias": cb, "shape": tuple(y.shape),
@@ -1719,6 +1764,58 @@
     return y
 
 
+def conv3x3_thin_out_gn(x, wp, bias, partials, blocks, gamma, beta, groups, eps, act):
+    require_cuda(x, wp, bias, partials, gamma, beta)
+    B, Cin, H, W = x.shape
+    if bias is not None:
+        bias = bias.to(x.dtype).contiguous()
+    x = _nhwc(x)
+    y = torch.empty((B, 4, H, W), dtype=x.dtype, device=x.device)
+    stats = torch.empty((B, groups, 2), dtype=torch.float32, device=x.device)
+    _count(("conv3x3_thin_out", B, Cin, H * W, 1, 4, bias is not None, str(x.dtype)))
+    check(load().ga_conv3x3_thin_out_gn(_ptr(x), _ptr(wp), _ptr(bias), _ptr(y), B, H, W, Cin, dtype_code(x), stream_ptr(),
+                                        _ptr(partials), blocks, groups, float(eps), _ptr(gamma), _ptr(beta), _ptr(stats),
+                                        int(bool(act))), "ga_conv3x3_thin_out_gn")
+    return y, stats
+
+
+class GroupNormConv3x3Thin(torch.autograd.Function):
+
+    @staticmethod
+    def forward(ctx, x, gn_weight, gn_bias, groups, eps, act, weight, bias, produced):
+        if ctx.needs_input_grad[1] or ctx.needs_input_grad[2] or ctx.needs_input_grad[6] or \
+                (bias is not None and ctx.needs_input_grad[7]):
+            raise GaError("GroupNorm / convolution weight gradients are not part of the guided-attention path (frozen UNet)")
+        x = _nhwc(x)
+        y, stats = conv3x3_thin_out_gn(x, conv3x3_thin_packed_weights(weight, False), bias, produced[0], produced[1], gn_weight,
+                                       gn_bias, groups, eps, act)
+        ctx.save_for_backward(x, gn_weight, gn_bias, stats)
+        ctx.weight, ctx.meta = weight, (groups, bool(act))
+        return y
+
+    @staticmethod
+    def backward(ctx, gy):
+        if not ctx.needs_input_grad[0]:
+            return (None,) * 9
+        x, gn_weight, gn_bias, stats = ctx.saved_tensors
+        groups, act = ctx.meta
+        weight = ctx.weight
+        g_norm = conv3x3_thin(gy, conv3x3_thin_packed_weights(weight, True), weight.shape[1])
+        return (group_norm_bwd(x, None, g_norm, gn_weight, gn_bias, stats, None, groups, act),) + (None,) * 8
+
+
+def group_norm_conv3x3_thin(x, norm_weight, norm_bias, groups, eps, act, weight, bias=None):
+    if GN_ABSORB != 1 or not conv3x3_thin_supported(x, weight):
+        return None
+    B, C, H, W = x.shape
+    if weight.shape[0] != 4 or not gn_absorb_wanted(H * W, C, B, groups, x.dtype):
+        return None
+    produced = gn_produced(x, groups)
+    if produced is None:
+        return None
+    return GroupNormConv3x3Thin.apply(x, norm_weight, norm_bias, groups, eps, act, weight, bias, produced)
+
+
 class Conv3x3Thin(torch.autograd.Function):
 
     @staticmethod
@@ -1741,6 +1838,7 @@
 
 
 conv3x3_thin_apply.supported = conv3x3_thin_supported
+conv3x3_thin_apply.with_group_norm = group_norm_conv3x3_thin
 
 
 def _sub_ptr(t, elem_offset):
@@ -1948,7 +2046,7 @@
 
 
 def linear_fused(x, weight, bias=None, residual=None, geglu=False, want_preact=False, ln=None, want_ln_stats=False,
-                 want_row_partials=False, plan=None, out=None, gn=None):
+                 want_row_partials=False, plan=None, out=None, gn=None, gn_in=None):
     require_cuda(x, weight, bias, residual)
     if x.stride(-1) != 1 or not weight.is_contiguous():
         raise GaError("linear_fused needs unit-stride feature axes")
@@ -2018,7 +2116,28 @@
         slabs, tickets = ws["slabs"], ws["tickets"]
     _count(("linear", M, K, 0, int(bool(geglu)) + 2 * int(ln is not None) + 4 * int(residual is not None), N, bias is not None,
             str(x.dtype)))
-    _check_ticketed(load().ga_linear_fused(_ptr(x), ldx, _ptr(weight), _ptr(y), y.stride(-2) if y.dim() > 1 else n_out,
-                                           ctypes.byref(ep), _ptr(slabs), _ptr(tickets), M, K, N, bm, bn, splits, stages,
-                                           dtype_code(x), stream_ptr()), "ga_linear_fused", tickets)
-    return {"y": y, "preact": preact, "ln_stats": ln_stats, "row_partials": row_partials, "parts": parts, "gn": gn_made}
+    gn_in_stats = None
+    if gn_in is not None:
+        g_partials, g_blocks, g_groups, g_hw, g_eps, g_gamma, g_beta = gn_in
+        require_cuda(g_partials, g_gamma, g_beta)
+        if g_gamma.dtype != x.dtype or g_beta.dtype != x.dtype or not g_gamma.is_contiguous() or not g_beta.is_contiguous():
+            raise GaError("the absorbed GroupNorm's weight and bias must be contiguous tensors of the activation type")
+        gn_in_stats = torch.empty((M // g_hw, g_groups, 2), dtype=torch.float32, device=x.device)
+        _check_ticketed(load().ga_linear_fused_gn(_ptr(x), ldx, _ptr(weight), _ptr(y), y.stride(-2) if y.dim() > 1 else n_out,
+                                                  ctypes.byref(ep), _ptr(slabs), _ptr(tickets), M, K, N, bm, bn, splits, stages,
+                                                  dtype_code(x), stream_ptr(), _ptr(g_partials), g_blocks, g_groups, g_hw,
+                                                  float(g_eps), _ptr(g_gamma), _ptr(g_beta), _ptr(gn_in_stats)),
+                        "ga_linear_fused_gn", tickets)
+    else:
+        _check_ticketed(load().ga_linear_fused(_ptr(x), ldx, _ptr(weight), _ptr(y), y.stride(-2) if y.dim() > 1 else n_out,
+                                               ctypes.byref(ep), _ptr(slabs), _ptr(tickets), M, K, N, bm, bn, splits, stages,
+                                               dtype_code(x), stream_ptr()), "ga_linear_fused", tickets)
+    return {"y": y, "preact": preact, "ln_stats": ln_stats, "row_partials": row_partials, "parts": parts, "gn": gn_made,
+            "gn_in_stats": gn_in_stats}
+
+
+def linear_gn_in_serves(M, K, N, hw, groups, plan=None):
+    plan = tuple(plan) if plan is not None else linear_plan(M, K, N)
+    stages = plan[3] if len(plan) > 3 else 0
+    return (stages != LINEAR_STREAM and hw % plan[0] == 0 and M % hw == 0 and K <= 1280 and K % 64 == 0 and groups <= 64
+            and K % groups == 0)
diff --git a/guided-attention_amd/unet.py b/guided-attention_amd/unet.py
--- a/guided-attention_amd/unet.py
+++ b/guided-attention_amd/unet.py
@@ -246,15 +246,34 @@
             return proj.weight, proj.bias
         return proj.weight.reshape(proj.out_channels, proj.in_channels), proj.bias
 
+    def _absorbed_entry(self, x):
+        blocks = self.transformer_blocks
+        lin = blocks[0].lin_impl
+        if lin is None or self.norm.impl is None or not hasattr(lin, "gn_linear") or not x.is_cuda:
+            return None
+        xt = nchw_to_tokens(x)
+        c = x.shape[1]
+        if not (xt.is_contiguous() and lin.supported(xt, c, blocks[0].norm1.normalized_shape[0]) and
+                all(blk.folds(xt) for blk in blocks)):
+            return None
+        alias = _GN_ALIAS and x.requires_grad and torch.is_grad_enabled()
+        return lin.gn_linear(x, self.norm, *self._proj_weights(self.proj_in), with_alias=alias)
+
     def forward(self, x, context):
         b, c, h, w = x.shape
-        x, res = self.norm(x, with_alias=True)
-        x = nchw_to_tokens(x)
         blocks = self.transformer_blocks
         lin = blocks[0].lin_impl
-        if lin is not None and x.is_contiguous() and lin.supported(x, c, blocks[0].norm1.normalized_shape[0]) and \
-                res.is_contiguous(memory_format=torch.channels_last) and all(blk.folds(x) for blk in blocks):
-            x, xp = lin.linear(x, *self._proj_weights(self.proj_in), want_partials=True)
+        entry = self._absorbed_entry(x)
+        if entry is None:
+            x, res = self.norm(x, with_alias=True)
+            x = nchw_to_tokens(x)
+        if entry is not None or (
+                lin is not None and x.is_contiguous() and lin.supported(x, c, blocks[0].norm1.normalized_shape[0]) and
+                res.is_contiguous(memory_format=torch.channels_last) and all(blk.folds(x) for blk in blocks)):
+            if entry is not None:
+                x, xp, res = entry
+            else:
+                x, xp = lin.linear(x, *self._proj_weights(self.proj_in), want_partials=True)
             for i, blk in enumerate(blocks):
                 x, xp = blk.forward_folded(x, xp, context, want_partials=i + 1 < len(blocks))
             x, _ = lin.linear(x, *self._proj_weights(self.proj_out), residual=nchw_to_tokens(res),
@@ -282,6 +301,7 @@
         self.conv2 = nn.Conv2d(out_channels, out_channels, 3, padding=1)
         self.conv_shortcut = nn.Conv2d(in_channels, out_channels, 1) if in_channels != out_channels else None
 
+    feeds_transformer = False
     add_impl = None
     conv_impl = None
     lin_impl = None
@@ -306,7 +326,8 @@
             x = tokens_to_nchw(xt, hh, ww)
         if self.conv_impl is not None and self.conv_impl.supported(h, self.conv2.weight, 1):
             if gn:
-                return self.conv_impl(h, self.conv2.weight, self.conv2.bias, x, 1, gn_for=(self.norm2.num_groups, None))
+                return self.conv_impl(h, self.conv2.weight, self.conv2.bias, x, 1,
+                                      gn_for=(self.norm2.num_groups, None, self.feeds_transformer))
             return self.conv_impl(h, self.conv2.weight, self.conv2.bias, x, 1)
         if self.add_impl is not None and self.conv2.out_channels % 8 == 0:
             return self.add_impl(F.conv2d(h, self.conv2.weight, None, padding=1), self.conv2.bias, x)
@@ -357,6 +378,8 @@
         if has_attn:
             for attn in self.attentions[:-1]:
                 attn.feeds_norm = True
+            for resnet in self.resnets:
+                resnet.feeds_transformer = True
 
     def forward(self, x, temb_act, context):
         outs = []
@@ -381,6 +404,7 @@
                                                             cfg.norm_num_groups, cfg.use_linear_projection, depth)])
 
         self.attentions[0].feeds_norm = True
+        self.resnets[0].feeds_transformer = True
 
     def forward(self, x, temb_act, context):
         x = self.resnets[0](x, temb_act)
@@ -404,6 +428,9 @@
                                                                 cfg.norm_num_groups, cfg.use_linear_projection, depth)
                                              for _ in range(n)])
         self.upsamplers = nn.ModuleList([Upsample2D(out_c)]) if add_upsample else None
+        if has_attn:
+            for resnet in self.resnets:
+                resnet.feeds_transformer = True
 
     cat_impl = None
 
@@ -679,10 +706,19 @@
                 blk(x, skips, temb_act, encoder_hidden_states, upsample_size, n_layers=stop_after_up_block[1])
                 return UNetOutput(sample=None) if return_dict else (None,)
             x = blk(x, skips, temb_act, encoder_hidden_states, upsample_size)
-        x = self._edge_conv(self.conv_out, self.conv_norm_out(x))
+        x = self._out_conv(x)
         return UNetOutput(sample=x) if return_dict else (x,)
 
     edge_conv_impl = None
+
+    def _out_conv(self, x):
+        impl, norm, conv = self.edge_conv_impl, self.conv_norm_out, self.conv_out
+        fused = getattr(impl, "with_group_norm", None) if impl is not None and norm.impl is not None else None
+        if fused is not None and x.is_cuda and conv.stride[0] == 1:
+            y = fused(x, norm.weight, norm.bias, norm.num_groups, norm.eps, norm.act, conv.weight, conv.bias)
+            if y is not None:
+                return y
+        return self._edge_conv(conv, norm(x))
 
     def _edge_conv(self, conv, x):
         impl = self.edge_conv_impl
diff --git a/include/ga_hip.h b/include/ga_hip.h
--- a/include/ga_hip.h
+++ b/include/ga_hip.h
@@ -213,6 +213,9 @@
                        ga_stream_t stream);
 int ga_conv3x3_thin_out(const void* X, const void* Wp, const void* bias, void* Y, int B, int H, int W, int Cin, int dtype,
                         ga_stream_t stream);
+int ga_conv3x3_thin_out_gn(const void* X, const void* Wp, const void* bias, void* Y, int B, int H, int W, int Cin, int dtype,
+                           ga_stream_t stream, const float* gn_in_partials, int gn_in_blocks, int gn_in_groups, float gn_in_eps,
+                           const void* gn_in_gamma, const void* gn_in_beta, float* gn_in_stats, int act_silu);
 
 int ga_gemm_nt(const void* X, const void* W, void* Y, float* workspace, unsigned* tickets, const void* bias,
                const void* residual, int64_t M, int K, int N, int bm, int bn, int splits, int dtype, ga_stream_t stream);
@@ -243,6 +246,11 @@
                     float* slabs, unsigned* tickets, int64_t M, int K, int N, int bm, int bn, int splits, int stages,
                     int dtype, ga_stream_t stream);
 
+int ga_linear_fused_gn(const void* X, int64_t ldx, const void* W, void* Y, int64_t ldy, const ga_linear_epilogue_t* ep,
+                       float* slabs, unsigned* tickets, int64_t M, int K, int N, int bm, int bn, int splits, int stages,
+                       int dtype, ga_stream_t stream, const float* gn_in_partials, int gn_in_blocks, int gn_in_groups,
+                       int gn_in_hw, float gn_in_eps, const void* gn_in_gamma, const void* gn_in_beta, float* gn_in_stats);
+
 int ga_add_layer_norm_fwd(const void* a, const void* x, const void* gamma, const void* beta, void* x_new, void* y,
                           float* stats, int64_t rows, int C, float eps, int dtype, ga_stream_t stream);
 int ga_add_layer_norm_bwd(const void* x, const float* stats, const void* gamma, const void* dy, const void* g_res,
```

Measured after the change: 1.963 (median of 6 runs). About the same (+0.8%).
